# GaodeRender/triangle-splatting

Measured on AMD Instinct MI355X. Metric: fwd+bwd Mpixels/sec @ 1M triangles, 1920x1080; achieved HBM GB/s, higher is better.
Workload: dtype f32

## Files before the change

triangle-splatting_amd/csrc/api.hip:

```cpp
#pragma GCC visibility push(default)
#include "../../include/ts2d.h"
#ifdef TS2D_LAB
#include "ts2d_lab.h"
#endif
#pragma GCC visibility pop
#include "ts2d_api.h"
#include <atomic>
#include <chrono>
#include <cstdarg>
#include <cstdio>
#include <cstring>
#include <mutex>
#include <string>
#include <vector>

namespace
{
thread_local std::string g_err;

struct ProfRow { std::string name; double ms = 0; int64_t launches = 0; };
struct ProfPending { int row; hipEvent_t a, b; };
std::mutex g_prof_mu;
bool g_prof_on = false;
std::string g_prof_only;
std::vector<ProfRow> g_prof_rows;
std::vector<ProfPending> g_prof_pending;
std::vector<hipEvent_t> g_prof_free;

void prof_drain()
{
    for (auto &p : g_prof_pending)
    {
        float ms = 0;
        if (hipEventSynchronize(p.b) == hipSuccess && hipEventElapsedTime(&ms, p.a, p.b) == hipSuccess)
        {
            g_prof_rows[p.row].ms += ms;
            g_prof_rows[p.row].launches += 1;
        }
        g_prof_free.push_back(p.a);
        g_prof_free.push_back(p.b);
    }
    g_prof_pending.clear();
}

#ifdef TS2D_LAB
bool g_lab_all_quadrants = false;
#endif

int validate(const ts2d_camera *cam, const ts2d_geometry *geom, uint32_t flags)
{
    if (!cam || !geom) return ts_fail(TS2D_ERR_INVALID, "null camera/geometry");
    if (cam->width <= 0 || cam->height <= 0) return ts_fail(TS2D_ERR_INVALID, "image size must be positive");
    if (cam->width > 65535 * TS_TILE || cam->height > 65535 * TS_TILE) return ts_fail(TS2D_ERR_INVALID, "image too large");
    if (geom->P < 0) return ts_fail(TS2D_ERR_INVALID, "P must be >= 0");
    if (geom->P > (int)TS_ID_MASK) return ts_fail(TS2D_ERR_CAPACITY, "more than 2^28 - 1 triangles: the instance values keep four bits for the quadrant mask");
    if (geom->C > TS2D_MAX_CHANNELS)
        return ts_fail(TS2D_ERR_INVALID, "feature's num_channels can't be larger than MAX_CHANNELS");
    if (geom->C < 1) return ts_fail(TS2D_ERR_INVALID, "need at least one colour channel");
    if (geom->gamma < 0.0f) return ts_fail(TS2D_ERR_INVALID, "gamma must be larger than 0");
    if (flags & TS2D_FLAG_USE_SHS)
    {
        if (geom->C != 3) return ts_fail(TS2D_ERR_INVALID, "SH mode renders 3 channels");
        if (geom->sh_degree < 0 || geom->sh_degree > 3) return ts_fail(TS2D_ERR_INVALID, "sh_degree must be in 0..3");
        if ((geom->sh_degree + 1) * (geom->sh_degree + 1) > geom->M)
            return ts_fail(TS2D_ERR_INVALID, "shs holds fewer coefficients than sh_degree needs");
        if (geom->P > 0 && !geom->shs) return ts_fail(TS2D_ERR_INVALID, "shs is null");
    }
    else if (geom->P > 0 && !geom->feature) return ts_fail(TS2D_ERR_INVALID, "feature is null");
    if (geom->P > 0 && (!geom->vertex || !geom->opacity)) return ts_fail(TS2D_ERR_INVALID, "vertex/opacity is null");
    if (!cam->viewmatrix || !cam->projmatrix || !cam->campos || !geom->background)
        return ts_fail(TS2D_ERR_INVALID, "camera matrices / background are null");
    return TS2D_OK;
}

PreprocessArgs make_pre(const ts2d_camera *cam, const ts2d_geometry *geom, uint32_t flags)
{
    PreprocessArgs a;
    a.W = cam->width; a.H = cam->height; a.P = geom->P; a.D = geom->sh_degree; a.M = geom->M; a.C = geom->C;
    a.grid_x = (cam->width + TS_TILE - 1) / TS_TILE; a.grid_y = (cam->height + TS_TILE - 1) / TS_TILE;
    a.rich_info = flags & TS2D_FLAG_RICH_INFO; a.use_shs = flags & TS2D_FLAG_USE_SHS;
    a.back_culling = flags & TS2D_FLAG_BACK_CULLING;
    a.tan_fovx = cam->tan_fovx; a.tan_fovy = cam->tan_fovy;
    a.viewmatrix = cam->viewmatrix; a.projmatrix = cam->projmatrix; a.campos = cam->campos;
    a.vertex = geom->vertex; a.shs = geom->shs; a.feature = geom->feature; a.opacity = geom->opacity;
    return a;
}

RenderArgs make_render(const ts2d_camera *cam, const ts2d_geometry *geom, uint32_t flags)
{
    RenderArgs r;
    r.W = cam->width; r.H = cam->height; r.C = geom->C;
    r.grid_x = (cam->width + TS_TILE - 1) / TS_TILE; r.grid_y = (cam->height + TS_TILE - 1) / TS_TILE;
    r.gamma = geom->gamma; r.background_depth = geom->background_depth;
    r.background_depth_dev = geom->background_depth_dev;
    r.background = geom->background;
    r.rich_info = flags & TS2D_FLAG_RICH_INFO;
    return r;
}

inline void cpu_relax()
{
#if defined(__x86_64__) || defined(__i386__)
    __builtin_ia32_pause();
#elif defined(__aarch64__)
    asm volatile("yield" ::: "memory");
#endif
}

struct CapacityHint { int dev, variant, W, H; unsigned long long key; double per_triangle; unsigned long long stamp; };
thread_local unsigned long long t_hint_key = 0;
std::atomic<unsigned long long> g_speculative_overflows{0};
std::mutex g_hint_mu;
std::vector<CapacityHint> g_hints;
unsigned long long g_hint_clock = 0;

void record_instance_count(int variant, int W, int H, int P, unsigned long long n)
{
    int dev = 0;
    if (P <= 0 || hipGetDevice(&dev) != hipSuccess) return;
    const double per = (double)n / (double)P;
    std::lock_guard<std::mutex> lk(g_hint_mu);
    CapacityHint *slot = nullptr;
    for (auto &h : g_hints)
        if (h.dev == dev && h.variant == variant && h.W == W && h.H == H && h.key == t_hint_key) slot = &h;
    if (!slot)
    {
        if (g_hints.size() < 32) { g_hints.push_back({dev, variant, W, H, t_hint_key, 0.0, 0}); slot = &g_hints.back(); }
        else
        {
            slot = &g_hints[0];
            for (auto &h : g_hints)
                if (h.stamp < slot->stamp) slot = &h;
            *slot = {dev, variant, W, H, t_hint_key, 0.0, 0};
        }
    }
    slot->per_triangle = per > 0.97 * slot->per_triangle ? per : 0.97 * slot->per_triangle;
    slot->stamp = ++g_hint_clock;
}

int read_instance_count(const ts2d_camera *cam, const ts2d_geometry *geom, uint32_t flags, const ts2d_state *state, const EarlyCount *early,
                        hipStream_t s, int64_t *num_rendered)
{
    if (int rc = wait_instance_count(geom->P, state, early, s, num_rendered)) return rc;
    record_instance_count((flags & TS2D_FLAG_3D) ? 3 : 2, cam->width, cam->height, geom->P, (unsigned long long)*num_rendered);
    return TS2D_OK;
}

int forward_bin_impl(const ts2d_camera *cam, const ts2d_geometry *geom, uint32_t flags, int32_t *radii, const ts2d_state *state, hipStream_t s,
                     const EarlyCount *early)
{
    const int P = geom->P;
    GeometryStateView g;
    ts_carve_geometry((char *)state->geometry, P, g);
    const PreprocessArgs a = make_pre(cam, geom, flags);
    {
        ProfScope ps("preprocess_fwd", s);
        if (flags & TS2D_FLAG_3D) ts_launch_preprocess3d_fwd(a, radii, g, s);
        else ts_launch_preprocess_fwd(a, radii, g, s);
    }
    TS_CHECK(flags, s, "preprocess_fwd");
    return ts_order_triangles(flags, g, P, early, s);
}

int forward_render_impl(const ts2d_camera *cam, const ts2d_geometry *geom, uint32_t flags, int64_t N, bool count_on_device,
                        const ts2d_state *state, const ts2d_forward_out *out, hipStream_t s)
{
    const bool rich = flags & TS2D_FLAG_RICH_INFO;
    const int P = geom->P, W = cam->width, H = cam->height;
    GeometryStateView g{};
    BinningStateView b{};
    ImageStateView im{};
    if (P > 0) ts_carve_geometry((char *)state->geometry, P, g);
    if (N > 0)
    {
        ts_carve_binning((char *)state->binning, ts_binning_capacity(state->binning_bytes, W, H), W, H, b);
        if (!count_on_device) ts_binning_set_count(b, N);
    }
    ts_carve_image((char *)state->image, W, H, im);
    const RenderArgs r = make_render(cam, geom, flags);
    const int ntiles = r.grid_x * r.grid_y;
    const unsigned long long *n_dev = count_on_device ? ts_instance_count_dev(g, P) : nullptr;

    QuadMaskArgs quad{(flags & TS2D_FLAG_3D) ? 3 : 2, fmaxf(0.0f, 2.0f * geom->gamma), cam->tan_fovx, cam->tan_fovy, W, H, 1.0f / (float)W, 1.0f / (float)H};
#ifdef TS2D_LAB
    if (g_lab_all_quadrants) quad.variant = 0;
#endif
    if (int rc = ts_order_instances(flags, P, r.grid_x, ntiles, g, b, im, rich ? out->contrib_sum : nullptr, rich ? out->contrib_max : nullptr, N, n_dev,
                                    quad, s))
        return rc;
    {
        ProfScope ps("render_fwd", s);
        if (flags & TS2D_FLAG_3D)
            ts_launch_render3d_fwd_group(r, cam->tan_fovx, cam->tan_fovy, g, b, im, out->out_feature, out->depth, out->normal,
                                         out->contrib_sum, out->contrib_max, s);
        else
            ts_launch_render_fwd_group(r, g, b, im, out->out_feature, out->depth, out->normal, out->contrib_sum, out->contrib_max, s);
    }
    TS_CHECK(flags, s, "render_fwd");
    return TS2D_OK;
}

int check_forward_args(const ts2d_camera *cam, const ts2d_geometry *geom, uint32_t flags, int64_t N, const ts2d_state *state,
                       const ts2d_forward_out *out)
{
    if (int rc = validate(cam, geom, flags)) return rc;
    if (!state || !out || !out->out_feature) return ts_fail(TS2D_ERR_INVALID, "null state/output");
    const bool rich = flags & TS2D_FLAG_RICH_INFO;
    if (rich && (!out->depth || !out->normal || (geom->P > 0 && (!out->contrib_sum || !out->contrib_max))))
        return ts_fail(TS2D_ERR_INVALID, "rich_info outputs are null");
    const int P = geom->P, W = cam->width, H = cam->height;
    if (N < 0) return ts_fail(TS2D_ERR_INVALID, "num_rendered < 0");
    if (N > 0x7fffffffll) return ts_fail(TS2D_ERR_CAPACITY, "the instance list addresses at most 2^31 - 1 instances");
    if (!state->image || state->image_bytes < ts2d_image_state_bytes(W, H)) return ts_fail(TS2D_ERR_CAPACITY, "image state buffer too small");
    if (N > 0 && (!state->binning || ts_binning_capacity(state->binning_bytes, W, H) < N))
        return ts_fail(TS2D_ERR_CAPACITY, "binning state buffer too small");
    if (P > 0 && (!state->geometry || state->geometry_bytes < ts2d_geometry_state_bytes(P)))
        return ts_fail(TS2D_ERR_CAPACITY, "geometry state buffer too small");
    return TS2D_OK;
}
}

int ts_fail(int code, const char *fmt, ...)
{
    char buf[512];
    va_list ap;
    va_start(ap, fmt);
    vsnprintf(buf, sizeof(buf), fmt, ap);
    va_end(ap);
    g_err = buf;
    return code;
}

ProfScope::ProfScope(const char *name, hipStream_t stream) : s(stream)
{
    if (!g_prof_on) return;
    std::lock_guard<std::mutex> lk(g_prof_mu);
    if (!g_prof_only.empty() && g_prof_only != name) return;
    for (size_t i = 0; i < g_prof_rows.size(); i++)
        if (g_prof_rows[i].name == name) row = (int)i;
    if (row < 0) { g_prof_rows.push_back({name, 0, 0}); row = (int)g_prof_rows.size() - 1; }
    auto get = [&]() { hipEvent_t e; if (!g_prof_free.empty()) { e = g_prof_free.back(); g_prof_free.pop_back(); } else (void)hipEventCreate(&e); return e; };
    a = get(); b = get();
    (void)hipEventRecord(a, s);
}
ProfScope::~ProfScope()
{
    if (row < 0) return;
    (void)hipEventRecord(b, s);
    std::lock_guard<std::mutex> lk(g_prof_mu);
    g_prof_pending.push_back({row, a, b});
}

bool acquire_early_count(EarlyCount &e)
{
    constexpr int SLOTS = 64, MAXDEV = 16;
    static unsigned long long *ring = [] {
        void *p = nullptr;
        return hipHostMalloc(&p, (size_t)MAXDEV * SLOTS * sizeof(unsigned long long), hipHostMallocPortable | hipHostMallocMapped | hipHostMallocCoherent) == hipSuccess
                   ? (unsigned long long *)p : nullptr;
    }();
    static hipEvent_t events[MAXDEV][SLOTS] = {};
    static std::atomic<unsigned> next{0};
    static std::mutex mu;
    int dev = 0;
    if (!ring || hipGetDevice(&dev) != hipSuccess || dev < 0 || dev >= MAXDEV) return false;
    const unsigned i = next.fetch_add(1) % SLOTS;
    {
        std::lock_guard<std::mutex> lk(mu);
#ifndef TS2D_COUNT_EVENT_FLAGS
#define TS2D_COUNT_EVENT_FLAGS (hipEventDisableTiming | hipEventBlockingSync)
#endif
        if (!events[dev][i] && hipEventCreateWithFlags(&events[dev][i], TS2D_COUNT_EVENT_FLAGS) != hipSuccess) return false;
    }
    e.host = ring + (size_t)dev * SLOTS + i;
    e.ev = events[dev][i];
    __atomic_store_n(e.host, ~0ull, __ATOMIC_RELEASE);
    return true;
}

int wait_instance_count(int P, const ts2d_state *state, const EarlyCount *early, hipStream_t s, int64_t *num_rendered)
{
    unsigned long long n = ~0ull;
    if (early)
    {
        const auto t0 = std::chrono::steady_clock::now();
        for (unsigned spin = 0;; spin++)
        {
            n = __atomic_load_n(early->host, __ATOMIC_ACQUIRE);
            if (n != ~0ull) break;
            cpu_relax();
            if ((spin & 63u) == 63u && std::chrono::steady_clock::now() - t0 > std::chrono::microseconds(250)) break;
        }
        if (n == ~0ull)
        {
            const hipError_t q = hipEventSynchronize(early->ev);
            if (q != hipSuccess) return ts_fail(TS2D_ERR_HIP, "waiting for the instance count: %s", hipGetErrorString(q));
            n = __atomic_load_n(early->host, __ATOMIC_ACQUIRE);
            if (n == ~0ull) return ts_fail(TS2D_ERR_HIP, "the instance count was not published");
        }
    }
    else
    {
        GeometryStateView g;
        ts_carve_geometry((char *)state->geometry, P, g);
        TS_HIP(hipMemcpyAsync(&n, ts_instance_count_dev(g, P), sizeof(n), hipMemcpyDeviceToHost, s));
        TS_HIP(hipStreamSynchronize(s));
    }
    if (n > 0x7fffffffull)
        return ts_fail(TS2D_ERR_CAPACITY, "%llu tile instances exceed the 2^31 - 1 the instance list can address", n);
    *num_rendered = (int64_t)n;
    return TS2D_OK;
}

int ts_order_triangles(uint32_t flags, const GeometryStateView &g, int P, const EarlyCount *early, hipStream_t s)
{
    {
        ProfScope ps("depth_census", s);
        ts_sort_by_depth_begin(g, P, early ? early->host : nullptr, s);
    }
    if (early) TS_HIP(hipEventRecord(early->ev, s));
    { ProfScope ps("depth_sort", s); ts_sort_by_depth_finish(g, P, s); }
    TS_CHECK(flags, s, "depth_sort");
    { ProfScope ps("scan", s); ts_scan_offsets(g, P, s); }
    TS_CHECK(flags, s, "scan");
    return TS2D_OK;
}

int ts_order_instances(uint32_t flags, int P, int grid_x, int ntiles, const GeometryStateView &g, const BinningStateView &b, const ImageStateView &im,
                       float *contrib_sum, float *contrib_max, int64_t N, const unsigned long long *n_dev, const QuadMaskArgs &quad, hipStream_t s)
{
    if (P > 0)
    {
        { ProfScope ps("emit_keys", s); ts_launch_emit_keys(P, grid_x, ntiles, g, b, im, contrib_sum, contrib_max, n_dev ? N : -1, im.status, quad, s); }
        TS_CHECK(flags, s, "emit_keys");
    }
    else ts_launch_zero_words((uint32_t *)im.ranges, 2 * (size_t)ntiles, s);
    if (N > 0)
    {
        { ProfScope ps("tile_sort", s); ts_sort_pairs(b, N, n_dev, ntiles, s); }
        TS_CHECK(flags, s, "tile_sort");
        { ProfScope ps("tile_ranges", s); ts_launch_tile_ranges(N, n_dev, b, im, s); }
        TS_CHECK(flags, s, "tile_ranges");
    }
    return TS2D_OK;
}

extern "C" {

const char *ts2d_version(void) { return "ts2d 0.1 (gfx950)"; }
const char *ts2d_last_error(void) { return g_err.c_str(); }

size_t ts2d_geometry_state_bytes(int32_t P)
{
    GeometryStateView v;
    return ts_carve_geometry(nullptr, P, v);
}
size_t ts2d_binning_state_bytes(int64_t N, int32_t W, int32_t H)
{
    BinningStateView v;
    return ts_carve_binning(nullptr, N, W, H, v);
}
size_t ts2d_image_state_bytes(int32_t W, int32_t H)
{
    ImageStateView v;
    return ts_carve_image(nullptr, W, H, v);
}
size_t ts2d_backward_scratch_bytes(int32_t P) { return (size_t)(P > 0 ? P : 0) * TS_GRAD_FLOATS * sizeof(float) + TS_ALIGN; }
int64_t ts2d_binning_capacity(size_t bytes, int32_t W, int32_t H)
{
    const int64_t c = ts_binning_capacity(bytes, W, H);
    return c < 0 ? 0 : c;
}
int64_t ts2d_instance_capacity_hint(int32_t P, int32_t W, int32_t H, uint32_t flags)
{
    int dev = 0;
    if (P <= 0 || hipGetDevice(&dev) != hipSuccess) return 0;
    const int variant = (flags & TS2D_FLAG_3D) ? 3 : 2;
    std::lock_guard<std::mutex> lk(g_hint_mu);
    for (auto &h : g_hints)
        if (h.dev == dev && h.variant == variant && h.W == W && h.H == H && h.key == t_hint_key)
        {
            h.stamp = ++g_hint_clock;
            const double want = 1.25 * h.per_triangle * (double)P + 4096.0;
            if (want >= 2147483647.0) return 0x7fffffffll;
            int64_t w = (int64_t)want, step = 1;
            while ((step << 4) <= w) step <<= 1;
            w = (w + step - 1) / step * step;
            return w > 0x7fffffffll ? 0x7fffffffll : w;
        }
    return 0;
}

int ts2d_forward_bin(const ts2d_camera *cam, const ts2d_geometry *geom, uint32_t flags, int32_t *radii,
                     const ts2d_state *state, int64_t *num_rendered, void *stream)
{
    if (int rc = validate(cam, geom, flags)) return rc;
    if (!state || !num_rendered) return ts_fail(TS2D_ERR_INVALID, "null state/num_rendered");
    hipStream_t s = (hipStream_t)stream;
    *num_rendered = 0;
    const int P = geom->P;
    if (P == 0) return TS2D_OK;
    if (!radii) return ts_fail(TS2D_ERR_INVALID, "radii is null");
    if (!state->geometry || state->geometry_bytes < ts2d_geometry_state_bytes(P))
        return ts_fail(TS2D_ERR_CAPACITY, "geometry state buffer too small: %zu < %zu", state->geometry_bytes,
                    ts2d_geometry_state_bytes(P));
    EarlyCount early;
    const bool have_early = acquire_early_count(early);
    if (int rc = forward_bin_impl(cam, geom, flags, radii, state, s, have_early ? &early : nullptr)) return rc;
    return read_instance_count(cam, geom, flags, state, have_early ? &early : nullptr, s, num_rendered);
}

int ts2d_forward_render(const ts2d_camera *cam, const ts2d_geometry *geom, uint32_t flags, int64_t N,
                        const ts2d_state *state, const ts2d_forward_out *out, void *stream)
{
    if (int rc = check_forward_args(cam, geom, flags, N, state, out)) return rc;
    return forward_render_impl(cam, geom, flags, N, false, state, out, (hipStream_t)stream);
}

int ts2d_forward(const ts2d_camera *cam, const ts2d_geometry *geom, uint32_t flags, int32_t *radii, const ts2d_state *state,
                 int64_t instance_capacity, const ts2d_forward_out *out, void *stream)
{
    if (int rc = check_forward_args(cam, geom, flags, instance_capacity, state, out)) return rc;
    hipStream_t s = (hipStream_t)stream;
    if (geom->P == 0) return forward_render_impl(cam, geom, flags, 0, false, state, out, s);
    if (!radii) return ts_fail(TS2D_ERR_INVALID, "radii is null");
    if (instance_capacity <= 0) return ts_fail(TS2D_ERR_INVALID, "instance_capacity must be positive");
    if (int rc = forward_bin_impl(cam, geom, flags, radii, state, s, nullptr)) return rc;
    return forward_render_impl(cam, geom, flags, instance_capacity, true, state, out, s);
}

int ts2d_forward_speculative(const ts2d_camera *cam, const ts2d_geometry *geom, uint32_t flags, int32_t *radii, const ts2d_state *state,
                             const ts2d_forward_out *out, int64_t *num_rendered, void *stream)
{
    if (!num_rendered) return ts_fail(TS2D_ERR_INVALID, "null num_rendered");
    *num_rendered = 0;
    if (int rc = check_forward_args(cam, geom, flags, 0, state, out)) return rc;
    hipStream_t s = (hipStream_t)stream;
    const int P = geom->P, W = cam->width, H = cam->height;
    if (P == 0) return forward_render_impl(cam, geom, flags, 0, false, state, out, s);
    if (!radii) return ts_fail(TS2D_ERR_INVALID, "radii is null");
    int64_t cap = state->binning ? ts_binning_capacity(state->binning_bytes, W, H) : 0;
    if (state->binning && cap <= 0) return ts_fail(TS2D_ERR_CAPACITY, "binning state buffer too small for any instance (pass NULL to size it from num_rendered)");
    EarlyCount early;
    const bool have_early = acquire_early_count(early);
    if (int rc = forward_bin_impl(cam, geom, flags, radii, state, s, have_early ? &early : nullptr)) return rc;
    if (cap > 0)
    {
        if (int rc = forward_render_impl(cam, geom, flags, cap, true, state, out, s)) return rc;
    }
    if (int rc = read_instance_count(cam, geom, flags, state, have_early ? &early : nullptr, s, num_rendered)) return rc;
    if (cap > 0 && *num_rendered > cap) g_speculative_overflows.fetch_add(1, std::memory_order_relaxed);
    return TS2D_OK;
}

void ts2d_set_capacity_hint_key(uint64_t key) { t_hint_key = key; }
uint64_t ts2d_speculative_overflow_count(void) { return g_speculative_overflows.load(std::memory_order_relaxed); }

int ts2d_forward_status(const ts2d_state *state, int32_t P, int32_t width, int32_t height, int32_t *overflowed, int64_t *num_rendered,
                        void *stream)
{
    if (!state || !state->image || !overflowed || !num_rendered) return ts_fail(TS2D_ERR_INVALID, "null pointer");
    hipStream_t s = (hipStream_t)stream;
    *overflowed = 0;
    *num_rendered = 0;
    if (P <= 0) return TS2D_OK;
    if (!state->geometry) return ts_fail(TS2D_ERR_INVALID, "null geometry state");
    GeometryStateView g{};
    ImageStateView im{};
    ts_carve_geometry((char *)state->geometry, P, g);
    ts_carve_image((char *)state->image, width, height, im);
    unsigned long long n = 0;
    TS_HIP(hipMemcpyAsync(overflowed, im.status, sizeof(int32_t), hipMemcpyDeviceToHost, s));
    TS_HIP(hipMemcpyAsync(&n, ts_instance_count_dev(g, P), sizeof(n), hipMemcpyDeviceToHost, s));
    TS_HIP(hipStreamSynchronize(s));
    *num_rendered = (int64_t)n;
    return TS2D_OK;
}

int ts2d_backward(const ts2d_camera *cam, const ts2d_geometry *geom, uint32_t flags, int64_t N, const int32_t *radii,
                  const ts2d_state *state, const ts2d_loss_grads *loss, void *scratch, size_t scratch_bytes,
                  const ts2d_backward_out *out, void *stream)
{
    return ts2d_backward_ranged(cam, geom, flags, N, radii, state, loss, scratch, scratch_bytes, out, 1, nullptr, stream);
}

int32_t ts2d_backward_range_rows(int32_t P, int32_t num_ranges)
{
    if (P <= 0 || num_ranges < 1) return 0;
    return ((P + num_ranges - 1) / num_ranges + 63) & ~63;
}

int ts2d_backward_ranged(const ts2d_camera *cam, const ts2d_geometry *geom, uint32_t flags, int64_t N, const int32_t *radii,
                         const ts2d_state *state, const ts2d_loss_grads *loss, void *scratch, size_t scratch_bytes,
                         const ts2d_backward_out *out, int32_t num_ranges, void *const *range_done_events, void *stream)
// ... 16 lines not shown
    if (!scratch || scratch_bytes < ts2d_backward_scratch_bytes(P)) return ts_fail(TS2D_ERR_CAPACITY, "backward scratch too small");
    if (!state->geometry || state->geometry_bytes < ts2d_geometry_state_bytes(P) || !state->image ||
        state->image_bytes < ts2d_image_state_bytes(W, H) ||
        (N > 0 && (!state->binning || ts_binning_capacity(state->binning_bytes, W, H) < N)))
        return ts_fail(TS2D_ERR_CAPACITY, "state buffers too small");
    GeometryStateView g{};
    BinningStateView b{};
    ImageStateView im{};
    ts_carve_geometry((char *)state->geometry, P, g);
    if (N > 0) ts_carve_binning((char *)state->binning, ts_binning_capacity(state->binning_bytes, W, H), W, H, b);
    ts_carve_image((char *)state->image, W, H, im);
    RenderArgs r = make_render(cam, geom, flags);
    if (colour_only) r.rich_info = false;
    float *grad_rec = (float *)ts_align_up((size_t)scratch);

    {
        ProfScope ps("zero_grad_records", s);
        ts_launch_zero_words((uint32_t *)grad_rec, (size_t)TS_GRAD_FLOATS * (size_t)P, s);
    }
    if (N > 0)
    {
        ProfScope ps("render_bwd", s);
        if (flags & TS2D_FLAG_3D)
            ts_launch_render3d_bwd_group(r, cam->tan_fovx, cam->tan_fovy, g, b, im, loss->dL_dout_feature, loss->dL_dout_depth,
                                         loss->dL_dout_normal, grad_rec, s);
        else
            ts_launch_render_bwd_group(r, g, b, im, loss->dL_dout_feature, loss->dL_dout_depth, loss->dL_dout_normal, grad_rec, s);
    }
    TS_CHECK(flags, s, "render_bwd");
    {
        ProfScope ps("preprocess_bwd", s);
        const PreprocessArgs a = make_pre(cam, geom, flags);
        const int per = ((P + num_ranges - 1) / num_ranges + 63) & ~63;
        for (int k = 0; k < num_ranges; k++)
        {
            const int first = k * per, count = first < P ? (P - first < per ? P - first : per) : 0;
            if (count > 0)
            {
                PreprocessArgs ak = a;
                ak.P = count;
                ak.vertex += 9 * (size_t)first;
                if (ak.shs) ak.shs += (size_t)first * a.M * 3;
                if (ak.feature) ak.feature += (size_t)first * a.C;
                ak.opacity += first;
                GeometryStateView gk = g;
                gk.clamped += first;
                if (gk.rec) gk.rec += 4 * (size_t)first;
                float *dshs = (factored || !out->dL_dshs) ? nullptr : out->dL_dshs + (size_t)first * a.M * 3;
                float *dfeat = out->dL_dfeature ? out->dL_dfeature + (size_t)first * a.C : nullptr;
                if (flags & TS2D_FLAG_3D)
                    ts_launch_preprocess3d_bwd(ak, radii + first, gk, grad_rec + TS_GRAD_FLOATS * (size_t)first, out->dL_dvertex + 9 * (size_t)first,
                                               out->dL_dcenter2D + 2 * (size_t)first, dshs, dfeat, out->dL_dopacity + first, s);
                else
                    ts_launch_preprocess_bwd(ak, radii + first, gk, grad_rec + TS_GRAD_FLOATS * (size_t)first, out->dL_dvertex + 9 * (size_t)first,
                                             out->dL_dcenter2D + 2 * (size_t)first, dshs, dfeat, out->dL_dopacity + first, s);
            }
            if (range_done_events && range_done_events[k]) TS_HIP(hipEventRecord((hipEvent_t)range_done_events[k], s));
        }
    }
    TS_CHECK(flags, s, "preprocess_bwd");
    return TS2D_OK;
}

int ts2d_sh_grad_expand(int32_t P, int32_t sh_degree, int32_t M, int32_t num_views, const float *vertex, const float *campos,
                        const float *dL_dcolor, float *dL_dshs, void *stream)
{
    if (P < 0 || num_views < 0) return ts_fail(TS2D_ERR_INVALID, "P / num_views must be >= 0");
    if (sh_degree < 0 || sh_degree > 3) return ts_fail(TS2D_ERR_INVALID, "sh_degree must be in 0..3");
    if ((sh_degree + 1) * (sh_degree + 1) > M) return ts_fail(TS2D_ERR_INVALID, "shs holds fewer coefficients than sh_degree needs");
    if (P == 0) return TS2D_OK;
    if (!vertex || !dL_dshs || (num_views > 0 && (!campos || !dL_dcolor))) return ts_fail(TS2D_ERR_INVALID, "null pointer");
    hipStream_t s = (hipStream_t)stream;
    { ProfScope ps("sh_grad_expand", s); ts_launch_sh_grad_expand(P, sh_degree, M, num_views, vertex, campos, dL_dcolor, dL_dshs, s); }
    TS_CHECK(0u, s, "sh_grad_expand");
    return TS2D_OK;
}

#ifdef TS2D_LAB
int ts2d_debug_read_state(const ts2d_state *state, int32_t P, int64_t N, int32_t W, int32_t H, int32_t field, void *dst,
                          size_t dst_bytes, void *stream)
{
    if (!state || !dst) return ts_fail(TS2D_ERR_INVALID, "null state/dst");
    hipStream_t s = (hipStream_t)stream;
    GeometryStateView g{};
    BinningStateView b{};
    ImageStateView im{};
    if (P > 0 && state->geometry) ts_carve_geometry((char *)state->geometry, P, g);
    if (N > 0 && state->binning) ts_carve_binning((char *)state->binning, ts_binning_capacity(state->binning_bytes, W, H), W, H, b);
    if (state->image) ts_carve_image((char *)state->image, W, H, im);
    const int gx = (W + TS_TILE - 1) / TS_TILE, gy = (H + TS_TILE - 1) / TS_TILE;
    const void *src = nullptr;
    size_t bytes = 0;
    std::vector<float> recs;
    auto need_recs = [&]() -> int {
        recs.resize((size_t)P * TS_REC_FLOATS);
        if (P == 0) return TS2D_OK;
        TS_HIP(hipMemcpyAsync(recs.data(), g.rec, recs.size() * sizeof(float), hipMemcpyDeviceToHost, s));
        TS_HIP(hipStreamSynchronize(s));
        return TS2D_OK;
    };
    auto from_recs = [&](std::initializer_list<int> cols, bool area) -> int {
        if (int rc = need_recs()) return rc;
        const size_t n = area ? 1 : cols.size();
        if (dst_bytes < (size_t)P * n * sizeof(float)) return ts_fail(TS2D_ERR_CAPACITY, "dst too small");
        float *o = (float *)dst;
        for (int i = 0; i < P; i++)
        {
            const float *r = &recs[(size_t)i * TS_REC_FLOATS];
            if (area) o[i] = (r[2] - r[0]) * (r[5] - r[1]) - (r[3] - r[1]) * (r[4] - r[0]);
            else { size_t c = 0; for (int col : cols) o[(size_t)i * n + c++] = r[col]; }
        }
        return TS2D_OK;
    };
    switch (field)
    {
    case 0: return from_recs({0, 1, 2, 3, 4, 5}, false);
    case 1: return from_recs({}, true);
    case 2: return from_recs({10, 11, 12}, false);
    case 3: return from_recs({13, 14, 15}, false);
    case 5: return from_recs({7, 8, 9}, false);
    case 4: src = g.depth; bytes = (size_t)P * 4; break;
    case 6: src = g.clamped; bytes = (size_t)P; break;
    case 7: src = g.offsets; bytes = (size_t)P * 4; break;
    case 8: src = g.tiles_touched; bytes = (size_t)P * 4; break;
    case 9:
    {
        std::vector<uint2> rc((size_t)P);
        if (dst_bytes < (size_t)P * 16) return ts_fail(TS2D_ERR_CAPACITY, "dst too small");
        if (P > 0)
        {
            TS_HIP(hipMemcpyAsync(rc.data(), g.rect, (size_t)P * sizeof(uint2), hipMemcpyDeviceToHost, s));
            TS_HIP(hipStreamSynchronize(s));
        }
        uint32_t *o = (uint32_t *)dst;
        for (int i = 0; i < P; i++)
        {
            o[4 * i] = rc[i].x & 0xffffu; o[4 * i + 1] = rc[i].x >> 16;
            o[4 * i + 2] = rc[i].y & 0xffffu; o[4 * i + 3] = rc[i].y >> 16;
        }
        return TS2D_OK;
    }
    case 10:
    {
        if (dst_bytes < (size_t)N * 8) return ts_fail(TS2D_ERR_CAPACITY, "dst too small");
        std::vector<uint32_t> tile((size_t)N), vals((size_t)N), depth((size_t)P);
        if (N > 0)
        {
            TS_HIP(hipMemcpyAsync(tile.data(), b.tile, (size_t)N * 4, hipMemcpyDeviceToHost, s));
            TS_HIP(hipMemcpyAsync(vals.data(), b.vals, (size_t)N * 4, hipMemcpyDeviceToHost, s));
            TS_HIP(hipMemcpyAsync(depth.data(), g.depth, (size_t)P * 4, hipMemcpyDeviceToHost, s));
            TS_HIP(hipStreamSynchronize(s));
        }
        uint64_t *o = (uint64_t *)dst;
        for (int64_t i = 0; i < N; i++) o[i] = ((uint64_t)tile[i] << 32) | depth[vals[i] & TS_ID_MASK];
        return TS2D_OK;
    }
    case 11: src = b.vals; bytes = (size_t)N * 4; break;
    case 12: src = im.ranges; bytes = (size_t)gx * gy * 8; break;
    case 13: src = im.n_contrib; bytes = (size_t)W * H * 4; break;
    case 14: src = im.final_T; bytes = (size_t)W * H * 4; break;
    case 15: src = b.k[(b.passes & 1) ^ 1]; bytes = (size_t)N * 4; break;
    case 16: src = b.v[(b.passes & 1) ^ 1]; bytes = (size_t)N * 4; break;
    case 17:
    {
        uint32_t top_const = 0;
        if (P > 0)
        {
            TS_HIP(hipMemcpyAsync(&top_const, g.top_const, 4, hipMemcpyDeviceToHost, s));
            TS_HIP(hipStreamSynchronize(s));
        }
        src = top_const ? g.sv[0] : g.sv[1];
        bytes = (size_t)P * 4;
        break;
    }
    case 18: src = g.rec; bytes = (size_t)P * TS_REC_FLOATS * 4; break;
    default: return ts_fail(TS2D_ERR_INVALID, "unknown field %d", field);
    }
    if (dst_bytes < bytes) return ts_fail(TS2D_ERR_CAPACITY, "dst too small");
    if (bytes)
    {
        TS_HIP(hipMemcpyAsync(dst, src, bytes, hipMemcpyDeviceToHost, s));
        TS_HIP(hipStreamSynchronize(s));
    }
    return TS2D_OK;
}

void ts2d_lab_force_ticket_passes(int on) { ts_force_ticket_passes(on != 0); }
void ts2d_lab_force_all_quadrants(int on) { g_lab_all_quadrants = on != 0; }
void ts2d_lab_force_depth_pass4(int on) { ts_force_depth_pass4(on != 0); }
void ts2d_lab_depth_split(int mode, int bucket_cap) { ts_lab_depth_split(mode, bucket_cap); }
#endif

void ts2d_profile_enable(int on)
{
    std::lock_guard<std::mutex> lk(g_prof_mu);
    g_prof_on = on != 0;
}
void ts2d_profile_only(const char *name)
{
    std::lock_guard<std::mutex> lk(g_prof_mu);
    g_prof_only = name ? name : "";
}
void ts2d_profile_reset(void)
{
    std::lock_guard<std::mutex> lk(g_prof_mu);
    prof_drain();
    g_prof_rows.clear();
}
int ts2d_profile_read(int32_t index, char *name, size_t name_bytes, double *total_ms, int64_t *launches)
{
    std::lock_guard<std::mutex> lk(g_prof_mu);
    prof_drain();
    if (index < 0 || (size_t)index >= g_prof_rows.size()) return TS2D_ERR_INVALID;
    const ProfRow &r = g_prof_rows[index];
    if (name && name_bytes) { strncpy(name, r.name.c_str(), name_bytes - 1); name[name_bytes - 1] = 0; }
    if (total_ms) *total_ms = r.ms;
    if (launches) *launches = r.launches;
    return TS2D_OK;
}
}
```

triangle-splatting_amd/csrc/binning.hip:

```cpp
#include "ts2d_common.h"
#include "ts2d_wave.h"
#include "ts2d_support.h"

namespace
{
constexpr int NB = TS_RS_BINS;

__device__ __forceinline__ unsigned long long ballot64(bool p) { return __builtin_amdgcn_ballot_w64(p); }

__device__ __forceinline__ uint32_t wave_inclusive_scan(uint32_t v, int lane)
{
    int x = (int)v;
    x += __builtin_amdgcn_update_dpp(0, x, 0x111, 0xF, 0xF, true);
    x += __builtin_amdgcn_update_dpp(0, x, 0x112, 0xF, 0xF, true);
    x += __builtin_amdgcn_update_dpp(0, x, 0x114, 0xF, 0xF, true);
    x += __builtin_amdgcn_update_dpp(0, x, 0x118, 0xF, 0xF, true);
    x += __builtin_amdgcn_update_dpp(0, x, 0x142, 0xA, 0xF, true);
    x += __builtin_amdgcn_update_dpp(0, x, 0x143, 0xC, 0xF, true);
    return (uint32_t)x;
}
__device__ __forceinline__ unsigned long long wave_sum64(unsigned long long v)
{
    for (int o = 32; o > 0; o >>= 1) v += __shfl_xor(v, o);
    return v;
// ... 492 lines not shown
#pragma unroll
        for (int j = 0; j < KB; j++)
        {
            const int p = t + 256 * j;
            if ((j & 3) == 0) dpack[j >> 2] = 0u;
            if (p < count)
            {
                const uint32_t k = stage_k[p], d = (k >> shift) & mask;
                dpack[j >> 2] |= d << (8 * (j & 3));
                kout[(int64_t)gdelta[d] + p] = k;
            }
        }
        __syncthreads();
#pragma unroll
        for (int b = 0; b < KB; b++)
            if (64 * b + lane < mine) stage_k[rk[b]] = val[b];
        __syncthreads();
#pragma unroll
        for (int j = 0; j < KB; j++)
        {
            const int p = t + 256 * j;
            if (p < count) vout[(int64_t)gdelta[(dpack[j >> 2] >> (8 * (j & 3))) & 0xFFu] + p] = stage_k[p];
        }
        return;
    }
#pragma unroll
    for (int b = 0; b < KB; b++)
        if (64 * b + lane < mine)
        {
            const uint32_t p = wcnt[wave][(key[b] >> shift) & mask] + rk[b];
            stage_k[p] = key[b];
            stage_v[p] = val[b];
        }
    __syncthreads();
    for (int p = t; p < count; p += 256)
    {
        const uint32_t k = stage_k[p];
        const int64_t dst = (int64_t)gdelta[(k >> shift) & mask] + p;
        kout[dst] = k;
        vout[dst] = stage_v[p];
    }
    if (CENSUS && chunk == 0) publish_census(census, r.chunks, t);
}
template <bool IDENTITY_VALUES, int CH, bool DIRECT, bool CENSUS = false>
__global__ void __launch_bounds__(256) rs_scatter_kernel(const uint32_t *__restrict__ kin, const uint32_t *__restrict__ vin,
                                                          uint32_t *__restrict__ kout, uint32_t *__restrict__ vout, int64_t n,
                                                          const unsigned long long *n_dev, int shift, int nbits, RadixScratchView r, const uint32_t *skip_flag,
                                                          const uint32_t *__restrict__ acc, uint32_t *__restrict__ acc_clear, DepthCensus census = DepthCensus{})
{
    rs_scatter_body<IDENTITY_VALUES, CH, DIRECT, CENSUS, false>(kin, vin, kout, vout, n, n_dev, shift, nbits, r, skip_flag, acc, acc_clear, census);
}
template <int CH>
__global__ void __launch_bounds__(256, 5) rs_scatter_two_phase_kernel(const uint32_t *__restrict__ kin, const uint32_t *__restrict__ vin,
                                                                       uint32_t *__restrict__ kout, uint32_t *__restrict__ vout, int64_t n,
                                                                       const unsigned long long *n_dev, int shift, int nbits, RadixScratchView r,
                                                                       const uint32_t *skip_flag, const uint32_t *__restrict__ acc, uint32_t *__restrict__ acc_clear)
{
    rs_scatter_body<false, CH, true, false, true>(kin, vin, kout, vout, n, n_dev, shift, nbits, r, skip_flag, acc, acc_clear, DepthCensus{});
}

#define TS_WITH_CHUNK(chunk, ...)                                    \
    switch (chunk)                                                   \
    {                                                                \
    case TS_RS_CHUNK_SMALL: { constexpr int CH = TS_RS_CHUNK_SMALL; __VA_ARGS__; } break; \
    case TS_RS_CHUNK_MID: { constexpr int CH = TS_RS_CHUNK_MID; __VA_ARGS__; } break;     \
    default: { constexpr int CH = TS_RS_CHUNK; __VA_ARGS__; } break; \
    }
void radix_hist(const uint32_t *kin, int64_t n, const unsigned long long *n_dev, int shift, int nbits, const RadixScratchView &r, hipStream_t s,
                const DepthCensus *census = nullptr, const uint32_t *skip_flag = nullptr)
{
    const dim3 grid((unsigned)r.chunks);
    const uint32_t mask = (1u << nbits) - 1u;
    TS_WITH_CHUNK(r.chunk,
                  if (census) hipLaunchKernelGGL((rs_hist_kernel<true, CH>), grid, dim3(256), 0, s, kin, n, n_dev, shift, mask, r, *census, skip_flag);
                  else hipLaunchKernelGGL((rs_hist_kernel<false, CH>), grid, dim3(256), 0, s, kin, n, n_dev, shift, mask, r, DepthCensus{}, skip_flag))
}
template <int CH>
void radix_scatter_ch(const uint32_t *kin, const uint32_t *vin, uint32_t *kout, uint32_t *vout, int64_t n, const unsigned long long *n_dev, int shift,
                      int nbits, const RadixScratchView &r, hipStream_t s, const uint32_t *skip_flag, const uint32_t *acc, uint32_t *acc_clear)
{
    const dim3 grid((unsigned)r.chunks);
#define TS_SCATTER(ID, D) hipLaunchKernelGGL((rs_scatter_kernel<ID, CH, D>), grid, dim3(256), 0, s, kin, vin, kout, vout, n, n_dev, shift, nbits, r, skip_flag, acc, acc_clear)
    if (acc && vin)
    {
        if constexpr (CH == TS_RS_CHUNK)
            hipLaunchKernelGGL((rs_scatter_two_phase_kernel<CH>), grid, dim3(256), 0, s, kin, vin, kout, vout, n, n_dev, shift, nbits, r, skip_flag, acc, acc_clear);
        else TS_SCATTER(false, true);
    }
    else if (acc) TS_SCATTER(true, true);
    else if (vin) TS_SCATTER(false, false);
    else TS_SCATTER(true, false);
#undef TS_SCATTER
}
void radix_scatter(const uint32_t *kin, const uint32_t *vin, uint32_t *kout, uint32_t *vout, int64_t n, const unsigned long long *n_dev, int shift,
                   int nbits, const RadixScratchView &r, hipStream_t s, const uint32_t *skip_flag = nullptr, const uint32_t *acc = nullptr,
                   uint32_t *acc_clear = nullptr)
{
    TS_WITH_CHUNK(r.chunk, radix_scatter_ch<CH>(kin, vin, kout, vout, n, n_dev, shift, nbits, r, s, skip_flag, acc, acc_clear))
}
void radix_pass(const uint32_t *kin, const uint32_t *vin, uint32_t *kout, uint32_t *vout, int64_t n, const unsigned long long *n_dev, int shift,
                int nbits, const RadixScratchView &r, hipStream_t s, const uint32_t *skip_flag = nullptr)
{
    radix_hist(kin, n, n_dev, shift, nbits, r, s, nullptr, skip_flag);
    radix_scatter(kin, vin, kout, vout, n, n_dev, shift, nbits, r, s, skip_flag);
}
bool g_force_tickets = false;
bool g_force_pass4 = false;
bool radix_direct_ok(const RadixScratchView &r) { return !g_force_tickets && r.slabs <= TS_DIRECT_MAX_SLABS; }
void radix_pass_direct(const uint32_t *kin, const uint32_t *vin, uint32_t *kout, uint32_t *vout, int64_t n, const unsigned long long *n_dev, int shift,
                       int nbits, const RadixScratchView &r, int which, hipStream_t s, const uint32_t *skip_flag = nullptr)
{
    const dim3 grid((unsigned)r.chunks);
    const uint32_t mask = (1u << nbits) - 1u;
    TS_WITH_CHUNK(r.chunk, hipLaunchKernelGGL((rs_hist_direct_kernel<CH>), grid, dim3(256), 0, s, kin, n, n_dev, shift, mask, r, r.slabacc[which], skip_flag))
    radix_scatter(kin, vin, kout, vout, n, n_dev, shift, nbits, r, s, skip_flag, r.slabacc[which], r.slabacc[which ^ 1]);
}

constexpr int SB = 1024;

__global__ void __launch_bounds__(256) gather_blocksum_kernel(int P, GeometryStateView g, bool two_level)
{
    __shared__ unsigned long long wsum[4];
    const int t = threadIdx.x, lane = t & 63, wave = t >> 6;
    const int i0 = blockIdx.x * SB + 4 * t;
    const uint32_t *ids = sorted_ids(g);
    uint32_t v[4];
    unsigned long long sum = 0;
#pragma unroll
    for (int k = 0; k < 4; k++)
    {
        v[k] = (i0 + k < P) ? g.tiles_touched[ids[i0 + k]] : 0u;
        sum += v[k];
    }
    if (i0 + 3 < P) *(uint4 *)(g.tiles_sorted + i0) = make_uint4(v[0], v[1], v[2], v[3]);
    else
        for (int k = 0; k < 4; k++)
            if (i0 + k < P) g.tiles_sorted[i0 + k] = v[k];
    for (int o = 32; o > 0; o >>= 1) sum += __shfl_xor(sum, o);
    if (lane == 0) wsum[wave] = sum;
    __syncthreads();
    if (t == 0)
    {
        const unsigned long long total = wsum[0] + wsum[1] + wsum[2] + wsum[3];
        g.blocksum[blockIdx.x] = total;
        if (two_level && total) __hip_atomic_fetch_add((unsigned long long *)g.supersum + (blockIdx.x >> 6), total, __ATOMIC_RELAXED, __HIP_MEMORY_SCOPE_AGENT);
    }
}

constexpr uint32_t SMALL = 32;

#ifndef TS_EMIT_WAVES
#define TS_EMIT_WAVES 6
#endif
#if TS_EMIT_WAVES > 0
__global__ void __launch_bounds__(256, TS_EMIT_WAVES) scan_emit_kernel(
#else
__global__ void __launch_bounds__(256) scan_emit_kernel(
#endif
int P, int grid_x, int ntiles, GeometryStateView g, BinningStateView b, uint2 *ranges,
                                                         float *contrib_sum, float *contrib_max, long long capacity, int32_t *status, bool two_level,
                                                         QuadMaskArgs qmask)
{
    __shared__ uint32_t wtot[4];
    __shared__ unsigned long long wpart[4];
    const int t = threadIdx.x, lane = t & 63, wave = t >> 6;
    const int i = blockIdx.x * 256 + t;
    for (int k = i; k < ntiles; k += gridDim.x * 256) ranges[k] = make_uint2(0u, 0u);
    if (b.rs.tickets)
    {
        for (int k = i; k < b.rs.slabs + TS_RS_TICKET_EXTRA; k += gridDim.x * 256) b.rs.tickets[k] = 0u;
        for (int k = i; k < b.rs.slabs * NB; k += gridDim.x * 256) b.rs.slabacc[0][k] = 0u;
    }
    if (contrib_sum && i < P)
    {
        contrib_sum[i] = 0.0f;
        contrib_max[i] = 0.0f;
    }
    const bool valid = i < P;
    uint32_t tiles = valid ? g.tiles_sorted[i] : 0u;
    const uint32_t id_ahead = valid ? sorted_ids(g)[i] : 0u;
    const int sblock = blockIdx.x >> 2, quarter = blockIdx.x & 3;
    unsigned long long part = 0;
    if (two_level)
    {
        for (int k = t; k < (sblock >> 6); k += 256) part += g.supersum[k];
        if (t < (sblock & 63)) part += g.blocksum[(sblock & ~63) + t];
    }
    else
        for (int k = t; k < sblock; k += 256) part += g.blocksum[k];
    for (int q = 0; q < quarter; q++)
    {
        const int j = (sblock * 4 + q) * 256 + t;
        part += (j < P) ? g.tiles_sorted[j] : 0u;
    }
    if (capacity >= 0)
    {
        const unsigned long long live = g.blocksum[(P + SB - 1) / SB];
        const bool over = live > (unsigned long long)capacity;
        if (i == 0 && status) *status = over ? 1 : 0;
        if (over) tiles = 0u;
    }
    else if (i == 0 && status) *status = 0;
    const uint32_t inc = wave_inclusive_scan(tiles, lane);
    for (int o = 32; o > 0; o >>= 1) part += __shfl_xor(part, o);
    if (lane == 63) wtot[wave] = inc;
    if (lane == 0) wpart[wave] = part;
    __syncthreads();
    uint32_t before = 0;
    for (int w = 0; w < wave; w++) before += wtot[w];
    const unsigned long long qbase = wpart[0] + wpart[1] + wpart[2] + wpart[3];
    const uint32_t incl = (uint32_t)(qbase + before + inc);
    if (valid) g.offsets[i] = incl;
    const uint32_t id = tiles > 0 ? id_ahead : 0u;
    const uint32_t off = incl - tiles;
    uint2 rect = {0u, 0u};
    float4 rec0 = make_float4(0, 0, 0, 0), rec1 = rec0, rec2 = rec0;
    if (tiles > 0)
    {
        rect = g.rect[id];
        const float4 *rp = g.rec + 4 * (size_t)id;
        rec0 = rp[0];
        rec1 = rp[1];
        if (qmask.variant == 3) rec2 = rp[2];
    }
    const uint32_t minx = rect.x & 0xffffu, miny = rect.x >> 16, maxx = rect.y & 0xffffu, maxy = rect.y >> 16;
    uint32_t *tile_out = b.k[0], *val_out = b.v[0];
    constexpr bool qm = true;
    const float quad_g2 = qmask.g2;
    auto setup_from = [&](const float4 &r0, const float4 &r1, const float4 &r2, uint32_t tminx, uint32_t tminy, uint32_t tmaxx, uint32_t tmaxy) {
        if (qmask.variant == 0) return quad_setup_all();
        if (qmask.variant == 3)
        {
            const float E = quad_g2 == 2.0f ? support_scale<true>(1.0f, quad_g2) : support_scale<false>(1.0f, quad_g2);
            return quad_setup_3d(r0, r1, r2, E, qmask.tan_fovx, qmask.tan_fovy, qmask.W, qmask.H, qmask.inv_W, qmask.inv_H, (float)(tminx * TS_TILE) - 1.0f,
                                 (float)(tminy * TS_TILE) - 1.0f, (float)(tmaxx * TS_TILE), (float)(tmaxy * TS_TILE));
        }
        const float E = quad_g2 == 2.0f ? support_scale<true>(r1.z, quad_g2) : support_scale<false>(r1.z, quad_g2);
        return quad_setup(r0.x, r0.y, r0.z, r0.w, r1.x, r1.y, E);
    };
    auto setup_of = [&](uint32_t tri, uint32_t tminx, uint32_t tminy, uint32_t tmaxx, uint32_t tmaxy) {
        const float4 *rp = g.rec + 4 * (size_t)tri;
        return setup_from(rp[0], rp[1], qmask.variant == 3 ? rp[2] : make_float4(0, 0, 0, 0), tminx, tminy, tmaxx, tmaxy);
    };
    QuadSetup qs{};
    constexpr uint32_t STAGE = 2048;
    __shared__ uint32_t stage_t[STAGE];
    __shared__ __attribute__((aligned(16))) float4 region_b[256 * 4];
    uint32_t *const stage_v = (uint32_t *)region_b;
    const uint32_t run0 = (uint32_t)qbase, run = wtot[0] + wtot[1] + wtot[2] + wtot[3];
    const bool staged = run <= STAGE;
    const bool qstage = qm && staged;
    const uint32_t rw = maxx - minx, rh = maxy - miny;
    if (qm && tiles > 0)
    {
        qs = setup_from(rec0, rec1, rec2, minx, miny, maxx, maxy);
        if (qstage)
        {
            const QuadAffine qa = quad_anchor(qs, id, minx, miny, rw, rh);
            region_b[4 * t] = qa.a; region_b[4 * t + 1] = qa.b; region_b[4 * t + 2] = qa.c; region_b[4 * t + 3] = qa.d;
        }
    }
    if (tiles > 0 && tiles <= SMALL)
    {
        uint32_t o = off;
        if (staged)
        {
            o -= run0;
            for (uint32_t y = miny; y < maxy; y++)
                for (uint32_t x = minx; x < maxx; x++)
                {
                    stage_t[o] = qstage ? ((x - minx) | ((y - miny) << 12) | ((uint32_t)t << 24)) : y * grid_x + x;
                    if (!qstage) stage_v[o] = id;
                    o++;
                }
        }
        else
            for (uint32_t y = miny; y < maxy; y++)
                for (uint32_t x = minx; x < maxx; x++)
                {
                    tile_out[o] = y * grid_x + x;
                    val_out[o] = qm ? id | (quadrant_mask(qs, (float)(x * TS_TILE), (float)(y * TS_TILE)) << TS_ID_BITS) : id;
                    o++;
                }
    }
    unsigned long long big = ballot64(tiles > SMALL);
    while (big)
    {
        const int j = __builtin_ctzll(big);
        big &= big - 1;
        const uint32_t t_minx = __shfl(minx, j), t_miny = __shfl(miny, j), t_maxx = __shfl(maxx, j), t_maxy = __shfl(maxy, j);
        const uint32_t t_tiles = __shfl(tiles, j), t_off = __shfl(off, j), t_id = __shfl(id, j);
        const uint32_t w = t_maxx - t_minx;
        QuadSetup tq{};
        if (qm && !staged) tq = setup_of(t_id, t_minx, t_miny, t_maxx, t_maxy);
        for (uint32_t k = lane; k < t_tiles; k += 64)
        {
            const uint32_t y = t_miny + k / w, x = t_minx + k % w;
            if (staged)
            {
                stage_t[t_off - run0 + k] = qstage ? ((k % w) | ((k / w) << 12) | ((uint32_t)(wave * 64 + j) << 24)) : y * grid_x + x;
                if (!qstage) stage_v[t_off - run0 + k] = t_id;
            }
            else
            {
                tile_out[t_off + k] = y * grid_x + x;
                val_out[t_off + k] = qm ? t_id | (quadrant_mask(tq, (float)(x * TS_TILE), (float)(y * TS_TILE)) << TS_ID_BITS) : t_id;
            }
        }
    }
    if (staged)
    {
        __syncthreads();
        for (uint32_t k = t; k < run; k += 256)
        {
            uint32_t tl = stage_t[k], v;
            if (qstage)
            {
                const uint32_t dx = tl & 0xfffu, dy = (tl >> 12) & 0xfffu, slot = tl >> 24;
                QuadAffine qa;
                qa.a = region_b[4 * slot]; qa.b = region_b[4 * slot + 1]; qa.c = region_b[4 * slot + 2]; qa.d = region_b[4 * slot + 3];
                const uint32_t org = __float_as_uint(qa.d.z), x = (org & 0xffffu) + dx, y = (org >> 16) + dy;
                v = __float_as_uint(qa.d.y) | (quadrant_mask_affine(qa, dx, dy, x, y) << TS_ID_BITS);
                tl = y * grid_x + x;
            }
            else v = stage_v[k];
            tile_out[run0 + k] = tl;
            val_out[run0 + k] = v;
        }
    }
}

__global__ void __launch_bounds__(256) tile_ranges_kernel(int64_t N, const unsigned long long *n_dev, const uint32_t *__restrict__ tile,
                                                           uint2 *__restrict__ ranges)
{
    const int64_t i0 = ((int64_t)blockIdx.x * 256 + threadIdx.x) * 4;
    if (n_dev)
    {
        const unsigned long long live = *n_dev;
        N = (live <= (unsigned long long)N) ? (int64_t)live : 0;
    }
    if (i0 >= N) return;
    uint32_t k[4];
    if (i0 + 3 < N)
    {
        const uint4 q = *(const uint4 *)(tile + i0);
        k[0] = q.x; k[1] = q.y; k[2] = q.z; k[3] = q.w;
    }
    else
        for (int j = 0; j < 4; j++) k[j] = i0 + j < N ? tile[i0 + j] : 0u;
    uint32_t prev = i0 > 0 ? tile[i0 - 1] : 0u;
#pragma unroll
    for (int j = 0; j < 4; j++)
    {
        const int64_t i = i0 + j;
        if (i >= N) break;
        const uint32_t cur = k[j];
        if (i == 0) ranges[cur].x = 0;
        else if (cur != prev)
        {
            ranges[prev].y = (uint32_t)i;
            ranges[cur].x = (uint32_t)i;
        }
        if (i == N - 1) ranges[cur].y = (uint32_t)N;
        prev = cur;
    }
}

__global__ void zero_words_kernel(uint32_t *p, size_t n)
{
    const size_t i = (size_t)blockIdx.x * 256 + threadIdx.x;
    if (i < n) p[i] = 0u;
}
constexpr int TS_DEPTH_SMALL_MAX = 12288;
constexpr int DS_WAVES = 16, DS_KB = TS_DEPTH_SMALL_MAX / (64 * DS_WAVES);
#if !defined(__gfx950__) && defined(__HIP_DEVICE_COMPILE__)
#error "depth_order_small_kernel is sized for gfx950 (160 KB LDS per workgroup)"
#endif
static_assert(2 * TS_DEPTH_SMALL_MAX * 4 + DS_WAVES * NB * 4 + DS_WAVES * 8 + (TS_DEPTH_SMALL_MAX / SB) * 8 + 2 * DS_WAVES * 4 + 16 <= 160 * 1024 - 8 * 1024,
              "depth_order_small_kernel: static LDS must leave 8 KB of the 160 KB for the runtime / alignment");
__global__ void __launch_bounds__(64 * DS_WAVES) depth_order_small_kernel(int P, GeometryStateView g, unsigned long long *host_out)
{
    __shared__ __attribute__((aligned(16))) uint32_t stage_k[TS_DEPTH_SMALL_MAX], stage_v[TS_DEPTH_SMALL_MAX];
    __shared__ uint32_t wcnt[DS_WAVES][NB];
    __shared__ uint32_t wtot[4];
    __shared__ unsigned long long csum[DS_WAVES], bsum[TS_DEPTH_SMALL_MAX / SB];
    __shared__ uint32_t cor[DS_WAVES], cand[DS_WAVES];
    const int t = threadIdx.x, wave = t >> 6, lane = t & 63;
    const int per = ((P + 64 * DS_WAVES - 1) / (64 * DS_WAVES)) * 64;
    const int base = wave * per;
    const int mine = P - base < per ? (P - base > 0 ? P - base : 0) : per;
    const uint32_t *keys = (const uint32_t *)g.depth;
    uint32_t key[DS_KB], val[DS_KB], rk[DS_KB];
    KeyCensus census;
    if (t < TS_DEPTH_SMALL_MAX / SB) bsum[t] = 0ull;
#pragma unroll
    for (int b = 0; b < DS_KB; b++)
    {
        const int i = 64 * b + lane;
        const bool in = i < mine;
        const int src = in ? base + i : 0;
        const uint32_t k = keys[src], tt = g.tiles_touched[src];
        key[b] = in ? k : 0xFFFFFFFFu;
        val[b] = (uint32_t)src;
        census.add(in ? k : 0u, in ? tt : 0u);
    }
    census.wave_fold();
    census.park(csum, cor, cand);
    __syncthreads();
    census = KeyCensus::gather<DS_WAVES>(csum, cor, cand);
    const unsigned long long N = census.tiles;
    const int passes = census.top_byte_constant() ? 3 : 4;
#pragma nounroll
    for (int pass = 0; pass < passes; pass++)
    {
        uint32_t unused;
        lsd_rank_pass<DS_KB, DS_WAVES>(key, rk, 8 * pass, per, mine, wcnt, wtot, unused);
#pragma unroll
        for (int b = 0; b < DS_KB; b++)
            if (64 * b + lane < mine) { stage_k[rk[b]] = key[b]; stage_v[rk[b]] = val[b]; }
        __syncthreads();
#pragma unroll
        for (int b = 0; b < DS_KB; b++)
        {
            key[b] = stage_k[base + 64 * b + lane];
            val[b] = stage_v[base + 64 * b + lane];
        }
    }
#pragma unroll
    for (int b = 0; b < DS_KB; b++)
    {
        if (64 * b >= per) continue;
        const int i = base + 64 * b + lane;
        unsigned long long tiles = 0;
        if (64 * b + lane < mine)
        {
            const uint32_t tt = g.tiles_touched[val[b]];
            g.sk[1][i] = key[b];
            g.sv[1][i] = val[b];
            g.tiles_sorted[i] = tt;
            tiles = tt;
        }
        tiles = wave_sum64(tiles);
        if (lane == 0 && tiles) atomicAdd(&bsum[(base + 64 * b) / SB], tiles);
    }
    __syncthreads();
    const int nblocks = (P + SB - 1) / SB;
    if (t < nblocks) g.blocksum[t] = bsum[t];
    if (t == 0) publish_instance_count(N, (unsigned long long *)g.blocksum + nblocks, g.top_const, false, host_out);
}

#ifndef TS_DEPTH_SPLIT_MAX_VALUE
#define TS_DEPTH_SPLIT_MAX_VALUE 500000
#endif
constexpr int TS_DEPTH_SPLIT_MAX = TS_DEPTH_SPLIT_MAX_VALUE;
constexpr int TS_DEPTH_SPLIT_HARD_MAX = 1600000;
constexpr int DSPL_SAMPLES = 4096, DSPL_SAMPLES_SMALL = 1024, DSPL_SMALL_BELOW = 150000;
constexpr int DB_WAVES = 16, DB_KB = 16, DB_CAP = 64 * DB_WAVES * DB_KB;
#ifndef TS_DB_SMALL_BELOW_VALUE
#define TS_DB_SMALL_BELOW_VALUE 300000
#endif
constexpr int DB_SMALL_WAVES = 4, DB_SMALL_BELOW = TS_DB_SMALL_BELOW_VALUE;
int g_depth_split_mode = 0;
int g_depth_bucket_cap = DB_CAP;

struct DepthSplit
{
    uint32_t *splitters;
    uint32_t *bucket_start;
    unsigned long long *chunk_sum;
    uint8_t *digit;
};
__host__ __device__ inline DepthSplit depth_split_of(const GeometryStateView &g)
{
    DepthSplit d;
    d.splitters = g.offsets;
    d.bucket_start = g.offsets + NB;
    d.chunk_sum = (unsigned long long *)(g.offsets + 1024);
    d.digit = (uint8_t *)g.sv[1];
    return d;
}

__device__ __forceinline__ uint32_t depth_key_adjust(uint32_t key, uint32_t kmin_visible) { return key ? key - kmin_visible + 1u : 0u; }
__device__ __forceinline__ uint32_t depth_key_restore(uint32_t adj, uint32_t kmin_visible) { return adj ? adj - 1u + kmin_visible : 0u; }

template <int SAMPLES>
__global__ void __launch_bounds__(256) depth_split_sample_kernel(int P, GeometryStateView g, DepthSplit ds)
{
    constexpr int DSPL_SAMPLES = SAMPLES, DSPL_PER = SAMPLES / NB;
    __shared__ uint32_t hist[NB], wtot[4], pick[2], rmin[4], rmax[4];
    constexpr int K = DSPL_SAMPLES / 256;
    const int t = threadIdx.x, lane = t & 63, wave = t >> 6;
    const uint32_t *keys = (const uint32_t *)g.depth;
    const int nblocks = (P + SB - 1) / SB;
    for (int i = blockIdx.x * 256 + t; i < nblocks; i += gridDim.x * 256) g.blocksum[i] = 0ull;
    uint32_t smp[K];
#pragma unroll
    for (int k = 0; k < K; k++) smp[k] = keys[(int)(((unsigned long long)(t + 256 * k) * (unsigned long long)P) / DSPL_SAMPLES)];
    uint32_t kmin = 0xFFFFFFFFu, kmax = 0u;
#pragma unroll
    for (int k = 0; k < K; k++) { kmin = min(kmin, smp[k] ? smp[k] : 0xFFFFFFFFu); kmax = max(kmax, smp[k]); }
    for (int o = 32; o > 0; o >>= 1) { kmin = min(kmin, (uint32_t)__shfl_xor((int)kmin, o)); kmax = max(kmax, (uint32_t)__shfl_xor((int)kmax, o)); }
    if (lane == 0) { rmin[wave] = kmin; rmax[wave] = kmax; }
    __syncthreads();
// ... 282 lines not shown
            for (int i = t; i < n; i += 64 * DB_WAVES) atomicAdd(&dstart[(depth_key_adjust(peer_load(kin + i), kmin) >> (8 * pass)) & 0xFFu], 1u);
            __syncthreads();
            {
                const uint32_t start = digit_exclusive_prefix<W>(t < NB ? dstart[t] : 0u, wtot, wave, lane);
                if (t < NB) dstart[t] = start;
                __syncthreads();
            }
            for (int t0 = 0; t0 < n; t0 += tile)
            {
                const int nt = n - t0 < tile ? n - t0 : tile;
                const int tper = ((nt + 64 * DB_WAVES - 1) / (64 * DB_WAVES)) * 64;
                const int tbase = wave * tper;
                const int tmine = nt - tbase < tper ? (nt - tbase > 0 ? nt - tbase : 0) : tper;
#pragma unroll
                for (int b = 0; b < DB_KB; b++)
                {
                    const int i = 64 * b + lane;
                    const bool in = i < tmine;
                    key[b] = in ? depth_key_adjust(peer_load(kin + t0 + tbase + i), kmin) : 0xFFFFFFFFu;
                    val[b] = in ? peer_load(vin + t0 + tbase + i) : 0u;
                }
                uint32_t tile_cnt;
                lsd_rank_pass<DB_KB, W>(key, rk, 8 * pass, tper, tmine, wcnt, wtot, tile_cnt);
#pragma unroll
                for (int b = 0; b < DB_KB; b++)
                    if (64 * b + lane < tmine)
                    {
                        const uint32_t d = (key[b] >> (8 * pass)) & 0xFFu;
                        const uint32_t p = dstart[d] + rk[b] - wcnt[0][d];
                        peer_store(kout + p, depth_key_restore(key[b], kmin));
                        peer_store(vout + p, val[b]);
                    }
                __syncthreads();
                if (t < NB) dstart[t] += tile_cnt;
                __syncthreads();
            }
            asm volatile("s_waitcnt vmcnt(0)" ::: "memory");
            __syncthreads();
        }
        if (src == 0)
            for (int i = t; i < n; i += 64 * DB_WAVES) { peer_store(g.sk[1] + s0 + i, peer_load(g.sk[0] + s0 + i)); peer_store(g.sv[1] + s0 + i, peer_load(g.sv[0] + s0 + i)); }
        asm volatile("s_waitcnt vmcnt(0)" ::: "memory");
        __syncthreads();
        for (int i0 = 64 * wave; i0 < n; i0 += 64 * DB_WAVES)
        {
            const bool in = i0 + lane < n;
            bucket_emit_tiles(g, s0 + i0, s0 + i0 + lane, in, in ? g.tiles_touched[peer_load(g.sv[1] + s0 + i0 + lane)] : 0u, lane);
        }
    }
}
}

#ifndef TS_DEPTH_SMALL_USE_VALUE
#define TS_DEPTH_SMALL_USE_VALUE 9216
#endif
constexpr int TS_DEPTH_SMALL_USE = TS_DEPTH_SMALL_USE_VALUE;
static_assert(TS_DEPTH_SMALL_USE <= TS_DEPTH_SMALL_MAX && TS_DEPTH_SMALL_USE >= 2048, "the split form's scratch needs 1024 + 2 chunks words of `offsets`");
enum class DepthForm { OneLaunch, Split, LsdDirect, LsdTickets };
static DepthForm depth_form(int32_t P, const RadixScratchView &r)
{
    const bool lsd_forced = g_force_tickets || g_force_pass4;
    if (P <= TS_DEPTH_SMALL_USE && !lsd_forced) return DepthForm::OneLaunch;
    if (!radix_direct_ok(r)) return DepthForm::LsdTickets;
    const bool split = P > TS_DEPTH_SMALL_USE && P <= (g_depth_split_mode == 2 ? TS_DEPTH_SPLIT_HARD_MAX : TS_DEPTH_SPLIT_MAX) && g_depth_split_mode != 1;
    return split && !lsd_forced ? DepthForm::Split : DepthForm::LsdDirect;
}
void ts_sort_by_depth_begin(const GeometryStateView &g, int32_t P, unsigned long long *host_out, hipStream_t s)
{
    if (P <= 0) return;
    const DepthForm form = depth_form(P, g.rs);
    if (form == DepthForm::OneLaunch)
    {
        hipLaunchKernelGGL(depth_order_small_kernel, dim3(1), dim3(64 * DS_WAVES), 0, s, P, g, host_out);
        return;
    }
    if (form == DepthForm::Split)
    {
        const DepthSplit ds = depth_split_of(g);
        const dim3 grid((unsigned)g.rs.chunks);
        if (P < DSPL_SMALL_BELOW) hipLaunchKernelGGL(depth_split_sample_kernel<DSPL_SAMPLES_SMALL>, dim3(NB - 1), dim3(256), 0, s, P, g, ds);
        else hipLaunchKernelGGL(depth_split_sample_kernel<DSPL_SAMPLES>, dim3(NB - 1), dim3(256), 0, s, P, g, ds);
        TS_WITH_CHUNK(g.rs.chunk,
                      hipLaunchKernelGGL((depth_split_hist_kernel<CH>), grid, dim3(256), 0, s, (int64_t)P, g, g.rs, g.rs.slabacc[0], ds);
                      hipLaunchKernelGGL((depth_split_scatter_kernel<CH>), grid, dim3(256), 0, s, (int64_t)P, g, g.rs, (const uint32_t *)g.rs.slabacc[0], ds, host_out))
        return;
    }
    DepthCensus c;
    c.tiles_touched = g.tiles_touched;
    c.chunk_sum = (unsigned long long *)g.blocksum;
    c.chunk_or = g.tiles_sorted;
    c.chunk_and = g.offsets;
    c.n_out = (unsigned long long *)g.blocksum + (P + SB - 1) / SB;
    c.host_out = host_out;
    c.top_const = g.top_const;
    c.force_varying = g_force_pass4 ? 0xFF000000u : 0u;
    if (form == DepthForm::LsdTickets)
    {
        radix_hist((const uint32_t *)g.depth, P, nullptr, 0, 8, g.rs, s, &c);
        return;
    }
    const dim3 grid((unsigned)g.rs.chunks);
    const uint32_t *keys = (const uint32_t *)g.depth;
    const unsigned long long *no_count = nullptr;
    const uint32_t *no_vals = nullptr, *no_skip = nullptr;
    TS_WITH_CHUNK(g.rs.chunk,
                  hipLaunchKernelGGL((rs_hist_census_direct_kernel<CH>), grid, dim3(256), 0, s, keys, (int64_t)P, 0xFFu, g.rs, g.rs.slabacc[0], c);
                  hipLaunchKernelGGL((rs_scatter_kernel<true, CH, true, true>), grid, dim3(256), 0, s, keys, no_vals, g.sk[0], g.sv[0], (int64_t)P, no_count, 0, 8,
                                     g.rs, no_skip, (const uint32_t *)g.rs.slabacc[0], g.rs.slabacc[1], c))
}
void ts_sort_by_depth_finish(const GeometryStateView &g, int32_t P, hipStream_t s)
{
    if (P <= 0) return;
    switch (depth_form(P, g.rs))
    {
    case DepthForm::OneLaunch: return;
    case DepthForm::Split:
        if (P < DB_SMALL_BELOW)
            hipLaunchKernelGGL(depth_bucket_sort_kernel<DB_SMALL_WAVES>, dim3(NB), dim3(64 * DB_SMALL_WAVES), 0, s, P, g, depth_split_of(g),
                               min(g_depth_bucket_cap, 64 * DB_SMALL_WAVES * DB_KB));
        else hipLaunchKernelGGL(depth_bucket_sort_kernel<DB_WAVES>, dim3(NB), dim3(64 * DB_WAVES), 0, s, P, g, depth_split_of(g), g_depth_bucket_cap);
        return;
    case DepthForm::LsdTickets:
        radix_scatter((const uint32_t *)g.depth, nullptr, g.sk[0], g.sv[0], P, nullptr, 0, 8, g.rs, s);
        radix_pass(g.sk[0], g.sv[0], g.sk[1], g.sv[1], P, nullptr, 8, 8, g.rs, s);
        radix_pass(g.sk[1], g.sv[1], g.sk[0], g.sv[0], P, nullptr, 16, 8, g.rs, s);
        radix_pass(g.sk[0], g.sv[0], g.sk[1], g.sv[1], P, nullptr, 24, 8, g.rs, s, g.top_const);
        return;
    case DepthForm::LsdDirect:
        radix_pass_direct(g.sk[0], g.sv[0], g.sk[1], g.sv[1], P, nullptr, 8, 8, g.rs, 1, s);
        radix_pass_direct(g.sk[1], g.sv[1], g.sk[0], g.sv[0], P, nullptr, 16, 8, g.rs, 0, s);
        radix_pass_direct(g.sk[0], g.sv[0], g.sk[1], g.sv[1], P, nullptr, 24, 8, g.rs, 1, s, g.top_const);
        return;
    }
}

static bool scan_two_level(int32_t P) { return g_force_tickets || (P + SB - 1) / SB > 2048; }
void ts_scan_offsets(const GeometryStateView &g, int32_t P, hipStream_t s)
{
    if (P <= 0) return;
    switch (depth_form(P, g.rs))
    {
    case DepthForm::OneLaunch:
    case DepthForm::Split: return;
    case DepthForm::LsdDirect:
    case DepthForm::LsdTickets: break;
    }
    hipLaunchKernelGGL(gather_blocksum_kernel, dim3((unsigned)((P + SB - 1) / SB)), dim3(256), 0, s, P, g, scan_two_level(P));
}

void ts_launch_emit_keys(int P, int grid_x, int ntiles, const GeometryStateView &g, const BinningStateView &b, const ImageStateView &im,
                         float *contrib_sum, float *contrib_max, int64_t capacity, int32_t *status, const QuadMaskArgs &qmask, hipStream_t s)
{
    if (P <= 0) return;
    hipLaunchKernelGGL(scan_emit_kernel, dim3((unsigned)(((P + SB - 1) / SB) * 4)), dim3(256), 0, s, P, grid_x, ntiles, g, b, im.ranges, contrib_sum,
                       contrib_max, (long long)capacity, status, scan_two_level(P), qmask);
}
const unsigned long long *ts_instance_count_dev(const GeometryStateView &g, int P) { return (const unsigned long long *)(g.blocksum + (P + SB - 1) / SB); }

void ts_sort_pairs(const BinningStateView &b, int64_t N, const unsigned long long *n_dev, int ntiles, hipStream_t s)
{
    if (N <= 0) return;
    const int bits = ts_tile_bits(ntiles);
    const int per = (bits + b.passes - 1) / b.passes;
    int src = 0;
    for (int p = 0; p < b.passes; p++)
    {
        const int shift = per * p, nbits = min(per, bits - shift);
        if (radix_direct_ok(b.rs)) radix_pass_direct(b.k[src], b.v[src], b.k[src ^ 1], b.v[src ^ 1], N, n_dev, shift, nbits, b.rs, p & 1, s);
        else radix_pass(b.k[src], b.v[src], b.k[src ^ 1], b.v[src ^ 1], N, n_dev, shift, nbits, b.rs, s);
        src ^= 1;
    }
}

void ts_launch_tile_ranges(int64_t N, const unsigned long long *n_dev, const BinningStateView &b, const ImageStateView &im, hipStream_t s)
{
    if (N <= 0) return;
    hipLaunchKernelGGL(tile_ranges_kernel, dim3((unsigned)((N + 1023) / 1024)), dim3(256), 0, s, N, n_dev, b.tile, im.ranges);
}

static int generic_chunk(size_t n) { return ts_instance_chunk(n); }
size_t ts_radix_scratch_bytes(size_t n)
{
    RadixScratchView r{};
    char *p = nullptr;
    ts_carve_radix(p, n, r, generic_chunk(n));
    return (size_t)p + TS_ALIGN;
}
int ts_radix_sort_pairs(uint32_t *const k[2], uint32_t *const v[2], size_t n, int end_bit, void *scratch, hipStream_t s, bool force_tickets)
{
    if (n == 0) return 0;
    RadixScratchView r{};
    char *p = (char *)ts_align_up((size_t)scratch);
    ts_carve_radix(p, n, r, generic_chunk(n));
    hipLaunchKernelGGL(zero_words_kernel, dim3((unsigned)((r.slabs + TS_RS_TICKET_EXTRA + 255) / 256)), dim3(256), 0, s, r.tickets, (size_t)(r.slabs + TS_RS_TICKET_EXTRA));
    const bool direct = !force_tickets && radix_direct_ok(r);
    if (direct) hipLaunchKernelGGL(zero_words_kernel, dim3((unsigned)r.slabs), dim3(256), 0, s, r.slabacc[0], (size_t)(r.slabs * NB));
    const int passes = (end_bit + 7) / 8;
    int src = 0;
    for (int ps = 0; ps < passes; ps++)
    {
        if (direct) radix_pass_direct(k[src], v[src], k[src ^ 1], v[src ^ 1], (int64_t)n, nullptr, 8 * ps, min(8, end_bit - 8 * ps), r, ps & 1, s);
        else radix_pass(k[src], v[src], k[src ^ 1], v[src ^ 1], (int64_t)n, nullptr, 8 * ps, min(8, end_bit - 8 * ps), r, s);
        src ^= 1;
    }
    return src;
}

void ts_force_ticket_passes(bool on) { g_force_tickets = on; }
namespace
{
__global__ void __launch_bounds__(256) zero_words4_kernel(uint4 *p, size_t n4)
{
    const size_t i = (size_t)blockIdx.x * 256 + threadIdx.x;
    if (i < n4) p[i] = make_uint4(0u, 0u, 0u, 0u);
}
}
void ts_launch_zero_words(uint32_t *p, size_t n, hipStream_t s)
{
    if (n == 0) return;
    if (n % 4 == 0 && ((size_t)p & 15) == 0) hipLaunchKernelGGL(zero_words4_kernel, dim3((unsigned)((n / 4 + 255) / 256)), dim3(256), 0, s, (uint4 *)p, n / 4);
    else hipLaunchKernelGGL(zero_words_kernel, dim3((unsigned)((n + 255) / 256)), dim3(256), 0, s, p, n);
}
void ts_force_depth_pass4(bool on) { g_force_pass4 = on; }
void ts_lab_depth_split(int mode, int bucket_cap)
{
    g_depth_split_mode = mode;
    g_depth_bucket_cap = bucket_cap > 0 && bucket_cap < DB_CAP ? bucket_cap : DB_CAP;
}
```

triangle-splatting_amd/csrc/render_group.hip:

```cpp
#include "ts2d_common.h"
#include "ts2d_wave.h"
#include "ts2d_group.h"
#include "ts2d_support.h"

#ifndef TSG_FWD_WAVES
#define TSG_FWD_WAVES 7
#endif
#ifndef TSG_BWD_WAVES
#define TSG_BWD_WAVES 7
#endif
#ifndef TSG_FWD_CAP
#define TSG_FWD_CAP 64
#endif
#ifndef TSG_BWD_CAP
#define TSG_BWD_CAP 64
#endif
#ifndef TSG_TCAP
#define TSG_TCAP 960
#endif
#ifndef TSG_PART
#define TSG_PART 3
#endif
namespace
{
[[maybe_unused]] constexpr int BROW = ROW + 16;

struct BlockCull
{
    float u1x, u1y, u2x, u2y, u3x, u3y, ia;
    bool ov[4];
};

__device__ __forceinline__ void publish_row(float *row, const BlockCull &s, uint32_t id, int jpos, const float4 &r1, const float4 &r2, const float4 &r3)
{
    float4 *q = (float4 *)row;
    q[0] = make_float4(s.u1x, s.u1y, s.u2x, s.u2y);
    q[1] = make_float4(s.u3x, s.u3y, s.ia, r1.z);
    q[2] = make_float4(r1.w, r2.x, r2.y, r2.z);
    q[3] = make_float4(r2.w, r3.x, r3.y, r3.z);
    q[4] = make_float4(r3.w, __uint_as_float(id), __int_as_float(jpos), 0.0f);
}

__device__ __forceinline__ void entry_geometry(BlockCull &s, float v1x, float v1y, float v2x, float v2y, float v3x, float v3y, float OX, float OY)
{
    const float area2 = __fsub_rn(__fmul_rn(v2x - v1x, v3y - v1y), __fmul_rn(v2y - v1y, v3x - v1x));
    s.ia = __builtin_amdgcn_rcpf(area2);
    s.u1x = v1x - OX; s.u1y = v1y - OY; s.u2x = v2x - OX; s.u2y = v2y - OY; s.u3x = v3x - OX; s.u3y = v3y - OY;
}

template <bool RICH>
__device__ __forceinline__ uint32_t republish_row(float *row, const uint32_t *__restrict__ point_list, const float4 *__restrict__ rec, uint32_t pos,
                                                  int jpos, float OX, float OY)
{
    const uint32_t id = point_list[pos] & TS_ID_MASK;
    const float4 *rp = rec + 4 * (size_t)id;
    const float4 r0 = rp[0], r1 = rp[1], r2 = rp[2], r3 = RICH ? rp[3] : make_float4(0, 0, 0, 0);
    BlockCull s;
    entry_geometry(s, r0.x, r0.y, r0.z, r0.w, r1.x, r1.y, OX, OY);
    publish_row(row, s, id, jpos, r1, r2, r3);
    return id;
}

template <bool GAMMA1>
__device__ __forceinline__ BlockCull block_cull(float v1x, float v1y, float v2x, float v2y, float v3x, float v3y, float op, float g2,
                                                float OX, float OY)
{
    BlockCull s;
    entry_geometry(s, v1x, v1y, v2x, v2y, v3x, v3y, OX, OY);
    const float C1 = (s.u2x * s.u3y - s.u2y * s.u3x) * s.ia, A1 = (v2y - v3y) * s.ia, B1 = (v3x - v2x) * s.ia;
    const float C2 = (s.u3x * s.u1y - s.u3y * s.u1x) * s.ia, A2 = (v3y - v1y) * s.ia, B2 = (v1x - v3x) * s.ia;
    const float A3 = -A1 - A2, B3 = -B1 - B2, C3 = 1.0f - C1 - C2;
    const float E = support_scale<GAMMA1>(op, g2);
    const float cx = (s.u1x + s.u2x + s.u3x) * (1.0f / 3.0f), cy = (s.u1y + s.u2y + s.u3y) * (1.0f / 3.0f);
    const float e1x = E * (s.u1x - cx), e2x = E * (s.u2x - cx), e3x = E * (s.u3x - cx);
    const float e1y = E * (s.u1y - cy), e2y = E * (s.u2y - cy), e3y = E * (s.u3y - cy);
    const float pad = 0.05f;
    const float bminx = cx + fminf(fminf(e1x, e2x), e3x) - pad, bmaxx = cx + fmaxf(fmaxf(e1x, e2x), e3x) + pad;
    const float bminy = cy + fminf(fminf(e1y, e2y), e3y) - pad, bmaxy = cy + fmaxf(fmaxf(e1y, e2y), e3y) + pad;
    const bool live = E > 0.0f;
    const bool x0 = live && bminx <= 3.0f && bmaxx >= 0.0f, x1 = live && bminx <= 7.0f && bmaxx >= 4.0f;
    const bool y0 = bminy <= 3.0f && bmaxy >= 0.0f, y1 = bminy <= 7.0f && bmaxy >= 4.0f;
    const float m = (1.0f - E) * (1.0f / 3.0f);
    const float k1 = C1 + fmaxf(0.0f, 3.0f * A1) + fmaxf(0.0f, 3.0f * B1) - m + 1e-6f * (fabsf(C1) + 7.0f * (fabsf(A1) + fabsf(B1)));
    const float k2 = C2 + fmaxf(0.0f, 3.0f * A2) + fmaxf(0.0f, 3.0f * B2) - m + 1e-6f * (fabsf(C2) + 7.0f * (fabsf(A2) + fabsf(B2)));
    const float k3 = C3 + fmaxf(0.0f, 3.0f * A3) + fmaxf(0.0f, 3.0f * B3) - m + 1e-6f * (fabsf(C3) + 7.0f * (fabsf(A3) + fabsf(B3)));
    const float ax1 = 4.0f * A1, ax2 = 4.0f * A2, ax3 = 4.0f * A3, by1 = 4.0f * B1, by2 = 4.0f * B2, by3 = 4.0f * B3;
    s.ov[0] = x0 && y0 && k1 >= 0.0f && k2 >= 0.0f && k3 >= 0.0f;
    s.ov[1] = x1 && y0 && k1 + ax1 >= 0.0f && k2 + ax2 >= 0.0f && k3 + ax3 >= 0.0f;
    s.ov[2] = x0 && y1 && k1 + by1 >= 0.0f && k2 + by2 >= 0.0f && k3 + by3 >= 0.0f;
    s.ov[3] = x1 && y1 && k1 + ax1 + by1 >= 0.0f && k2 + ax2 + by2 >= 0.0f && k3 + ax3 + by3 >= 0.0f;
    return s;
}

__device__ __forceinline__ void write_dummy_row(float *row, int lane)
{
    if (lane < ROW)
    {
        float v = 0.0f;
        if (lane == 0 || lane == 1 || lane == 3 || lane == 4) v = 1000.0f;
        if (lane == 2 || lane == 5) v = 1001.0f;
        if (lane == 6) v = 1.0f;
        if (lane == 18) v = __int_as_float(0x7fffffff);
        row[lane] = v;
    }
}

struct Bary { float p1x, p1y, p2x, p2y, p3x, p3y, a1, a2, a3, mn, ecc; };
__device__ __forceinline__ Bary barycentrics(const float4 &q0, const float4 &q1, float fx, float fy)
{
    Bary b;
    b.p1x = q0.x - fx; b.p1y = q0.y - fy; b.p2x = q0.z - fx; b.p2y = q0.w - fy; b.p3x = q1.x - fx; b.p3y = q1.y - fy;
    b.a1 = (b.p2x * b.p3y - b.p2y * b.p3x) * q1.z;
    b.a2 = (b.p3x * b.p1y - b.p3y * b.p1x) * q1.z;
    b.a3 = 1.0f - b.a1 - b.a2;
    b.mn = fminf(fminf(b.a1, b.a2), b.a3);
    b.ecc = fmaf(-3.0f, b.mn, 1.0f);
    return b;
}
#ifdef TS2D_STATS
__device__ unsigned long long g_stats_group[12];
#define TSG_STAT(i, v) stat_acc[i] += (unsigned long long)(v)
#else
#define TSG_STAT(i, v)
#endif

#if TSG_PART & 1
template <bool RICH, bool GAMMA1>
__global__ void __launch_bounds__(256, TSG_FWD_WAVES) render_fwd_group_kernel(RenderArgs a, const uint2 *__restrict__ ranges,
                                                                const uint32_t *__restrict__ point_list, const float4 *__restrict__ rec,
                                                                float *__restrict__ final_T, uint32_t *__restrict__ n_contrib,
                                                                float *__restrict__ out_feature, float *__restrict__ out_depth,
                                                                float *__restrict__ out_normal, float *__restrict__ contrib_sum,
                                                                float *__restrict__ contrib_max)
{
    __shared__ __attribute__((aligned(16))) float cst_all[4][(NR + 1) * ROW];
    __shared__ __attribute__((aligned(16))) uint32_t list_all[4][4 * NR / 2];
    constexpr int TCAP = TSG_TCAP;
    __shared__ unsigned long long tsum[RICH ? TCAP : 1];
    __shared__ int tmax[RICH ? TCAP : 1];

    const int tile = tile_of_block(blockIdx.x, a.grid_x, a.grid_y);
    if (tile < 0) return;
    const int wave = threadIdx.x >> 6;
    const GroupPixel p = group_pixel(a, tile, wave);
    const int lane = p.lane;
    const float fx = (float)p.lx, fy = (float)p.ly, OX = (float)p.X0, OY = (float)p.Y0;
    const uint2 range = ranges[tile];
    const int len = (int)(range.y - range.x);
    if (RICH) tile_stats_clear<TCAP>(tsum, tmax, len);
    const float g2 = 2.0f * a.gamma;
    float *cst = cst_all[wave] + ROW;
    uint32_t *list = list_all[wave];
    write_dummy_row(cst - ROW, lane);
    const char *lds0 = (const char *)cst_all;
    const uint32_t row0 = table_row0(wave, ROW), dummy = row0 - ROW * 4;
    const int stat_step = window_stat_step(lane);
    FwdPixel P = fwd_pixel(p.inside, len);

#ifdef TS2D_STATS
    unsigned long long stat_acc[12] = {0, 0, 0, 0, 0, 1, 0, 0, 0, 0, 0, 0};
#endif
    uint32_t id = 0;
    int pos = 0, cursor = 0;
    for (;;)
    {
        const unsigned long long alive = ballot(!P.done);
        if (alive == 0) break;
        int nq = 0;
        stream_refill<false, TSG_FWD_CAP>(id, pos, nq, point_list + range.x, cursor, len, TS_ID_BITS + wave, lane);
        if (nq == 0) break;
        const bool valid = lane < nq;
        const int ent = pos;
        float4 r0 = make_float4(0, 0, 0, 0), r1 = r0, r2 = r0, r3 = r0;
        gather_record<RICH>(rec, id, valid, r0, r1, r2, r3);
        const BlockCull s = block_cull<GAMMA1>(r0.x, r0.y, r0.z, r0.w, r1.x, r1.y, r1.z, g2, OX, OY);
        unsigned long long M[4];
        const unsigned long long any = fwd_block_masks(M, alive, valid, s.ov);
        TSG_STAT(0, __popcll(ballot(valid)));
        if (any == 0) continue;
        TSG_STAT(1, __popcll(M[0]) + __popcll(M[1]) + __popcll(M[2]) + __popcll(M[3]));
        TSG_STAT(6, 1);
        TSG_STAT(7, __popcll(any));
        const Compaction cp = compact_rows(any, lane);
        bool mine = in_pass(cp, false);
        if (mine) publish_row(cst + cp.r * ROW, s, id, ent, r1, r2, r3);
        for (int h = 0;;)
        {
            const int steps = build_lists(list, M, pass_mask(cp, mine), row0, cp.r, ROW, dummy, lane);
            const u16a *mylist = (const u16a *)list + p.grp * NR;
            TSG_STAT(2, steps);
            TSG_STAT(3, (steps + 7) / 8);
            TSG_STAT(8, __popcll(list_conflicts(list, dummy, lane)));
            TSG_STAT(9, 1);
            TSG_STAT(10, h > 0 ? 1 : 0);

            for (int t0 = 0; t0 < steps; t0 += 8)
            {
                float c[8];
                const uint4 packed = *(const uint4 *)(mylist + t0);
#pragma unroll
                for (int st = 0; st < 8; st++)
                {
                    c[st] = 0.0f;
                    if (t0 + st < steps)
                    {
                        const float *row = window_row(lds0, packed, st);
                        const float4 q0 = *(const float4 *)(row), q1 = *(const float4 *)(row + 4);
                        const Bary b = barycentrics(q0, q1, fx, fy);
                        const float4 q2 = *(const float4 *)(row + 8);
                        float4 q3 = make_float4(0, 0, 0, 0);
                        float vd3 = 0.0f;
                        int jpos;
                        if (RICH)
                        {
                            q3 = *(const float4 *)(row + 12);
                            const float4 q4 = *(const float4 *)(row + 16);
                            vd3 = q4.x;
                            jpos = __float_as_int(q4.z);
                        }
                        else jpos = __float_as_int(row[18]);
                        const float pw = GAMMA1 ? b.ecc * b.ecc : pow_nonneg(b.ecc, g2);
                        const float alpha = fminf(0.99f, q1.w * __builtin_amdgcn_exp2f(pw * -0.7213475204444817f));
                        const bool hit = !P.done && ecc_in_range(b.ecc) && alpha >= 1.0f / 255.0f;
                        TSG_STAT(4, __popcll(ballot(hit)));
                        const float d = q3.z * b.a1 + q3.w * b.a2 + vd3 * b.a3;
                        const float contrib = fwd_blend<RICH>(P, hit, alpha, q2.x, q2.y, q2.z, q2.w, q3.x, q3.y, d, jpos);
                        if (RICH) c[st] = contrib;
                    }
                }
                if (RICH) window_stats<TCAP>(c, lane, stat_step, lds0, mylist, t0, 18, tsum, tmax, point_list + range.x, contrib_sum, contrib_max);
            }
            if (++h * NR >= cp.nact) break;
            mine = in_pass(cp, true);
            if (mine) republish_row<RICH>(cst + cp.r * ROW, point_list, rec, range.x + pos, ent, OX, OY);
        }
    }

#ifdef TS2D_STATS
    if (lane == 0)
        for (int i = 0; i < 12; i++) atomicAdd(&g_stats_group[i], stat_acc[i]);
#endif
    fwd_store_pixel<RICH>(a, p, P, final_T, n_contrib, out_feature, out_depth, out_normal);
    if (RICH) tile_stats_leave<TCAP>(tsum, tmax, len, point_list + range.x, contrib_sum, contrib_max);
}

#endif

#if TSG_PART & 2
template <bool RICH, bool GAMMA1>
__global__ void __launch_bounds__(64, TSG_BWD_WAVES) render_bwd_group_kernel(RenderArgs a, const uint2 *__restrict__ ranges,
                                                             const uint32_t *__restrict__ point_list, const float4 *__restrict__ rec,
                                                             const float *__restrict__ final_T, const uint32_t *__restrict__ n_contrib,
                                                             const float *__restrict__ dL_dout_feature,
                                                             const float *__restrict__ dL_dout_depth,
                                                             const float *__restrict__ dL_dout_normal, float *__restrict__ grad_rec)
{
    __shared__ __attribute__((aligned(16))) float rows_all[(NR + 1) * BROW];
    __shared__ __attribute__((aligned(16))) uint32_t list[4 * NR / 2];

    int quad;
    const int tile = tile_of_quadrant_block(blockIdx.x, a.grid_x, a.grid_y, quad);
    if (tile < 0) return;
    const GroupPixel p = group_pixel(a, tile, quad);
    const int lane = p.lane, grp = p.grp, sub = p.sub;
    const float fx = (float)p.lx, fy = (float)p.ly, OX = (float)p.X0, OY = (float)p.Y0;
    const uint2 range = ranges[tile];
    const float g2 = 2.0f * a.gamma;
    float *rows = rows_all + BROW;
    write_dummy_row(rows - BROW, lane);
    char *lds0 = (char *)rows_all;
    const uint32_t row0 = table_row0(0, BROW), dummy = row0 - BROW * 4;
    const uint32_t accoff = ROW * 4 + 4 * sub;

    const BwdPixel P = bwd_pixel<RICH>(a, p, final_T, n_contrib, dL_dout_feature, dL_dout_depth, dL_dout_normal);
    float T = P.T, B = P.B;
    const int last = P.last;
    const float dpr = P.dpr, dpg = P.dpg, dpb = P.dpb, dnx = P.dnx, dny = P.dny, dnz = P.dnz, dd = P.dd;
    const int quarter = sub >> 2;
    const float kq0 = quarter == 0 ? dpr : (quarter == 1 ? dpg : (quarter == 2 ? dpb : dnx));
    const float kq1 = quarter == 0 ? dpb : (quarter == 1 ? dnx : (quarter == 2 ? dpr : dpg));
    const float kq2 = quarter == 0 ? dpg : (quarter == 1 ? dpr : (quarter == 2 ? dnx : dpb));
    const float kq3 = quarter == 0 ? dnx : (quarter == 1 ? dpb : (quarter == 2 ? dpg : dpr));
    const float kp4 = (sub & 8) ? dnz : dny, kp5 = (sub & 8) ? dny : dnz;
    const int rcol = (int)((0xF15ADC39E0486B27ull >> (4 * sub)) & 15ull);
    int glast[4];
    const int maxlast = block_lasts(last, glast);
    if (maxlast <= 0) return;

    uint32_t id = 0;
    int pos = 0, cursor = maxlast;
    for (;;)
    {
        int nq = 0;
        stream_refill<true, TSG_BWD_CAP>(id, pos, nq, point_list + range.x, cursor, maxlast, TS_ID_BITS + quad, lane);
        if (nq == 0) break;
        const bool valid = lane < nq;
        const int ent = pos;
        float4 r0 = make_float4(0, 0, 0, 0), r1 = r0, r2 = r0, r3 = r0;
        gather_record<RICH>(rec, id, valid, r0, r1, r2, r3);
        const BlockCull s = block_cull<GAMMA1>(r0.x, r0.y, r0.z, r0.w, r1.x, r1.y, r1.z, g2, OX, OY);
        unsigned long long M[4];
        const unsigned long long any = bwd_block_masks(M, valid, s.ov, pos, glast);
        if (any == 0) continue;
        const Compaction cp = compact_rows(any, lane);
        bool mine = in_pass(cp, false);
        if (mine) publish_row(rows + cp.r * BROW, s, id, ent, r1, r2, r3);
        for (int h = (cp.nact - 1) / NR;;)
        {
            const unsigned long long mm = pass_mask(cp, mine);
            if (mine) zero_sums(rows + cp.r * BROW + ROW);
            const int steps = build_lists(list, M, mm, row0, cp.r, BROW, dummy, lane);
            const u16a *mylist = (const u16a *)list + grp * NR;
            const unsigned long long conflict = list_conflicts(list, dummy, lane);
            uint32_t ra_next = mylist[0];
            for (int t0 = 0; t0 < steps; t0++)
            {
                {
                    const uint32_t ra = ra_next;
                    ra_next = mylist[min(t0 + 1, NR - 1)];
                    const float *row = (const float *)(lds0 + ra);
                    float *acc = (float *)(lds0 + ra + accoff);
                    const bool shared_row = (conflict >> t0) & 1;
                    const float q0acc = *acc;
                    const float4 q0 = *(const float4 *)(row), q1 = *(const float4 *)(row + 4);
                    const Bary b = barycentrics(q0, q1, fx, fy);
                    const float4 q2 = *(const float4 *)(row + 8);
                    float4 q3 = make_float4(0, 0, 0, 0);
                    float vd3 = 0.0f;
                    int jpos;
                    if (RICH)
                    {
                        q3 = *(const float4 *)(row + 12);
                        const float4 q4 = *(const float4 *)(row + 16);
                        vd3 = q4.x;
                        jpos = __float_as_int(q4.z);
                    }
                    else jpos = __float_as_int(row[18]);
                    const float pw = GAMMA1 ? b.ecc * b.ecc : pow_nonneg(b.ecc, g2);
                    const float G = __builtin_amdgcn_exp2f(pw * -0.7213475204444817f);
                    const float opG = q1.w * G;
                    const float alpha = fminf(0.99f, opG);
                    const bool hit = (jpos < last) && ecc_in_range(b.ecc) && alpha >= 1.0f / 255.0f;
                    const float al = hit ? alpha : 0.0f;
                    const float oma = 1.0f - al;
                    T = T * __builtin_amdgcn_rcpf(oma);
                    const float contrib = al * T;
                    float X = fmaf(dpb, q2.z, fmaf(dpg, q2.y, dpr * q2.x));
                    float w = 0.0f;
                    if (RICH)
                    {
                        X = fmaf(dnz, q3.y, fmaf(dny, q3.x, fmaf(dnx, q2.w, X)));
                        const float depth = fmaf(vd3, b.a3, fmaf(q3.w, b.a2, q3.z * b.a1));
                        X = fmaf(dd, depth, X);
                        w = dd * contrib;
                    }
                    const float dL_dcontrib = X - B;
                    B = fmaf(al, X, oma * B);
                    const float dL_dalpha = dL_dcontrib * T;
                    const float zr = GAMMA1 ? 1.5f * g2 * (dL_dalpha * alpha) * b.ecc
                                            : 1.5f * g2 * (dL_dalpha * alpha) * pw * __builtin_amdgcn_rcpf(b.ecc + 1e-8f);
                    const float z = (hit && opG < 0.99f) ? zr : 0.0f;
                    const bool k1 = b.a1 == b.mn;
                    const bool k2 = !k1 && b.a2 == b.mn;
                    const float z1 = k1 ? z : 0.0f, z2 = k2 ? z : 0.0f, z3 = z - z1 - z2;
                    const float da1 = fmaf(w, q3.z, z1), da2 = fmaf(w, q3.w, z2), da3 = fmaf(w, vd3, z3);
                    const float sdot = fmaf(da3, b.a3, fmaf(da2, b.a2, da1 * b.a1));
                    const float e1 = da1 - sdot, e2 = da2 - sdot, e3 = da3 - sdot;
                    float v[16];
                    v[0] = kq0 * contrib; v[1] = kq1 * contrib; v[2] = kq2 * contrib; v[3] = kq3 * contrib;
                    v[4] = kp4 * contrib; v[5] = kp5 * contrib;
                    v[6] = e3 * b.p2y - e2 * b.p3y;
                    v[7] = e2 * b.p3x - e3 * b.p2x;
                    v[8] = e1 * b.p3y - e3 * b.p1y;
                    v[9] = e3 * b.p1x - e1 * b.p3x;
                    v[10] = e2 * b.p1y - e1 * b.p2y;
                    v[11] = e1 * b.p2x - e2 * b.p1x;
                    v[12] = hit ? dL_dalpha * G : 0.0f;
                    v[13] = w * b.a1; v[14] = w * b.a2; v[15] = w * b.a3;
                    const float red = row_reduce16c(v, 0xCCCCCCCCCCCCCCCCull, 0xAAAAAAAAAAAAAAAAull);
                    row_add(acc, q0acc, red, shared_row, grp);
                }
            }

            {
                const int n = __popcll(mm);
#pragma unroll 1
                for (int e0 = 0; e0 < n; e0 += 4)
                {
                    const int e = e0 + grp;
                    if (e < n)
                    {
                        const uint32_t eid = __float_as_uint(rows[e * BROW + 17]);
                        float val = rows[e * BROW + ROW + sub];
                        if (rcol < 6) val *= rows[e * BROW + 6];
                        if (RICH || rcol < 10) unsafeAtomicAdd(grad_rec + TS_GRAD_FLOATS * (size_t)eid + rcol, val);
                    }
                }
            }
            if (--h < 0) break;
            mine = in_pass(cp, true);
            if (mine) republish_row<RICH>(rows + cp.r * BROW, point_list, rec, range.x + pos, ent, OX, OY);
        }
    }
}
#endif
}

#if TSG_PART & 1
void ts_launch_render_fwd_group(const RenderArgs &a, const GeometryStateView &g, const BinningStateView &b, const ImageStateView &im,
                                float *out_feature, float *out_depth, float *out_normal, float *contrib_sum, float *contrib_max,
                                hipStream_t s)
{
    if (a.grid_x * a.grid_y == 0) return;
    TS_LAUNCH_BLEND(render_fwd_group_kernel, a, ts_tile_units(a.grid_x, a.grid_y), 256, s, a, im.ranges, b.vals, g.rec, im.final_T, im.n_contrib,
                    out_feature, out_depth, out_normal, contrib_sum, contrib_max);
}

#endif

#if defined(TS2D_STATS) && (TSG_PART & 1)
extern "C" __attribute__((visibility("default"))) int ts2d_stats_read_group(unsigned long long *out, int reset)
{
    hipError_t e = hipMemcpyFromSymbol(out, HIP_SYMBOL(g_stats_group), sizeof(unsigned long long) * 12);
    if (e == hipSuccess && reset)
    {
        unsigned long long z[12] = {0};
        e = hipMemcpyToSymbol(HIP_SYMBOL(g_stats_group), z, sizeof(z));
    }
    return e == hipSuccess ? 0 : 2;
}
#endif

#if TSG_PART & 2
void ts_launch_render_bwd_group(const RenderArgs &a, const GeometryStateView &g, const BinningStateView &b, const ImageStateView &im,
                                const float *dL_dout_feature, const float *dL_dout_depth, const float *dL_dout_normal, float *grad_rec,
                                hipStream_t s)
{
    if (a.grid_x * a.grid_y == 0) return;
    TS_LAUNCH_BLEND(render_bwd_group_kernel, a, ts_quadrant_units(a.grid_x, a.grid_y), 64, s, a, im.ranges, b.vals, g.rec, im.final_T, im.n_contrib,
                    dL_dout_feature, dL_dout_depth, dL_dout_normal, grad_rec);
}
#endif
```

triangle-splatting_amd/csrc/ts2d_common.h:

```cpp
#pragma once
#include <hip/hip_runtime.h>
#include <stddef.h>
#include <stdint.h>

#define TS_TILE 16
#define TS_ALIGN 256

#define TS_REC_FLOATS 16

#define TS_ID_BITS 28
#define TS_ID_MASK 0x0FFFFFFFu
#define TS_GRAD_FLOATS 16

#ifndef TS_RS_CHUNK
#define TS_RS_CHUNK 4096
#endif
#define TS_RS_CHUNK_MID 2048
#define TS_RS_CHUNK_SMALL 1024
#define TS_RS_SMALL_BELOW 2500000
static inline int ts_instance_chunk(size_t n) { return n <= (size_t)TS_RS_SMALL_BELOW ? TS_RS_CHUNK_SMALL : TS_RS_CHUNK; }
static inline int ts_depth_chunk(size_t n) { return n <= (size_t)TS_RS_SMALL_BELOW ? TS_RS_CHUNK_SMALL : TS_RS_CHUNK_MID; }
#define TS_RS_BINS 256
#define TS_RS_TICKET_EXTRA 8
struct RadixScratchView
{
    uint32_t *table;
    uint32_t *slabtot;
    uint32_t *binbase;
    uint32_t *tickets;
    uint32_t *slabacc[2];
    int chunks, slabs;
    int chunk;
};

struct GeometryStateView
{
    float4 *rec;
    float *depth;
    uint32_t *tiles_touched;
    uint2 *rect;
    uint8_t *clamped;
    uint32_t *sk[2], *sv[2];
    uint32_t *depth_sorted;
    uint32_t *perm;
    uint32_t *top_const;
    uint32_t *tiles_sorted;
    uint32_t *offsets;
    uint64_t *blocksum;
    uint64_t *supersum;
    RadixScratchView rs;
};

struct BinningStateView
{
    uint32_t *k[2], *v[2];
    uint32_t *tile;
    uint32_t *vals;
    int passes;
    RadixScratchView rs;
};

struct ImageStateView
{
    uint2 *ranges;
    uint32_t *n_contrib;
    float *final_T;
    int32_t *status;
};

static inline size_t ts_align_up(size_t v) { return (v + TS_ALIGN - 1) & ~(size_t)(TS_ALIGN - 1); }

template <typename T>
static inline void ts_carve(char *&p, T *&out, size_t count)
{
    p = (char *)ts_align_up((size_t)p);
    out = (T *)p;
    p += count * sizeof(T);
}

static inline void ts_carve_radix(char *&p, size_t n, RadixScratchView &r, int chunk = TS_RS_CHUNK, int reserve_chunk = 0)
{
    r.chunk = chunk;
    r.chunks = (int)((n + chunk - 1) / chunk);
    r.slabs = (r.chunks + 63) / 64;
    const int rc = reserve_chunk > 0 ? reserve_chunk : chunk;
    const size_t chunks = (n + rc - 1) / rc, slabs = (chunks + 63) / 64;
    ts_carve(p, r.table, chunks * TS_RS_BINS);
    ts_carve(p, r.slabtot, slabs * TS_RS_BINS);
    ts_carve(p, r.binbase, (size_t)TS_RS_BINS);
    ts_carve(p, r.tickets, slabs + TS_RS_TICKET_EXTRA);
    ts_carve(p, r.slabacc[0], slabs * TS_RS_BINS);
    ts_carve(p, r.slabacc[1], slabs * TS_RS_BINS);
}

static inline size_t ts_carve_geometry(char *base, int32_t P, GeometryStateView &v)
{
    char *p = base;
    size_t n = (size_t)(P > 0 ? P : 0);
    ts_carve(p, v.rec, n * 4);
    ts_carve(p, v.depth, n);
    ts_carve(p, v.tiles_touched, n);
    ts_carve(p, v.rect, n);
    ts_carve(p, v.clamped, n);
    ts_carve(p, v.sk[0], n);
    ts_carve(p, v.sk[1], n);
    ts_carve(p, v.sv[0], n);
    ts_carve(p, v.sv[1], n);
    v.depth_sorted = v.sk[1];
    v.perm = v.sv[1];
    ts_carve(p, v.tiles_sorted, n);
    ts_carve(p, v.offsets, n);
    ts_carve(p, v.blocksum, (n + 1023) / 1024 + 2);
    ts_carve(p, v.supersum, ((n + 1023) / 1024 + 63) / 64 + 1);
    ts_carve_radix(p, n, v.rs, ts_depth_chunk(n));
    v.top_const = v.rs.tickets + v.rs.slabs + 4;
    return (size_t)(p - base) + TS_ALIGN;
}

static inline int ts_higher_msb(uint32_t n)
{
    uint32_t msb = sizeof(n) * 4, step = msb;
    while (step > 1)
    {
        step /= 2;
        if (n >> msb) msb += step;
        else msb -= step;
    }
    if (n >> msb) msb++;
    return (int)msb;
}

static inline int ts_tile_bits(int ntiles) { return ts_higher_msb((uint32_t)(ntiles > 1 ? ntiles - 1 : 1)); }

static inline size_t ts_carve_binning(char *base, int64_t N, int32_t W, int32_t H, BinningStateView &v)
{
    char *p = base;
    size_t n = (size_t)(N > 0 ? N : 0);
    int gx = (W + TS_TILE - 1) / TS_TILE, gy = (H + TS_TILE - 1) / TS_TILE;
    ts_carve(p, v.k[0], n);
    ts_carve(p, v.k[1], n);
    ts_carve(p, v.v[0], n);
    ts_carve(p, v.v[1], n);
    v.passes = (ts_tile_bits(gx * gy) + 7) / 8;
    v.tile = v.k[v.passes & 1];
    v.vals = v.v[v.passes & 1];
    ts_carve_radix(p, n, v.rs, ts_instance_chunk(n), TS_RS_CHUNK_SMALL);
    return (size_t)(p - base) + TS_ALIGN;
}

static inline int64_t ts_binning_capacity(size_t bytes, int32_t W, int32_t H)
{
    BinningStateView v;
    if (bytes < ts_carve_binning(nullptr, 0, W, H, v)) return -1;
    int64_t lo = 0, hi = (int64_t)(bytes / 16) + 1;
    if (hi > 0x7fffffffll) hi = 0x7fffffffll;
    while (lo < hi)
    {
        const int64_t mid = lo + (hi - lo + 1) / 2;
        if (ts_carve_binning(nullptr, mid, W, H, v) <= bytes) lo = mid;
        else hi = mid - 1;
    }
    return lo;
}

static inline void ts_binning_set_count(BinningStateView &v, int64_t n)
{
    v.rs.chunks = (int)((n + v.rs.chunk - 1) / v.rs.chunk);
    v.rs.slabs = (v.rs.chunks + 63) / 64;
}

static inline size_t ts_carve_image(char *base, int32_t W, int32_t H, ImageStateView &v)
{
    char *p = base;
    int gx = (W + TS_TILE - 1) / TS_TILE, gy = (H + TS_TILE - 1) / TS_TILE;
    ts_carve(p, v.ranges, (size_t)gx * gy);
    ts_carve(p, v.n_contrib, (size_t)W * H);
    ts_carve(p, v.final_T, (size_t)W * H);
    ts_carve(p, v.status, (size_t)4);
    return (size_t)(p - base) + TS_ALIGN;
}

struct PreprocessArgs
{
    int W, H, P, D, M, C;
    int grid_x, grid_y;
    bool rich_info, use_shs, back_culling;
    float tan_fovx, tan_fovy;
    const float *viewmatrix, *projmatrix, *campos;
    const float *vertex, *shs, *feature, *opacity;
};

void ts_launch_preprocess_fwd(const PreprocessArgs &a, int32_t *radii, const GeometryStateView &g, hipStream_t s);
void ts_sort_by_depth_begin(const GeometryStateView &g, int32_t P, unsigned long long *host_out, hipStream_t s);
void ts_sort_by_depth_finish(const GeometryStateView &g, int32_t P, hipStream_t s);
void ts_scan_offsets(const GeometryStateView &g, int32_t P, hipStream_t s);
struct QuadMaskArgs
{
    int variant;
    float g2;
    float tan_fovx, tan_fovy;
    int W, H;
    float inv_W, inv_H;
};
void ts_launch_zero_words(uint32_t *p, size_t n, hipStream_t s);
void ts_launch_emit_keys(int P, int grid_x, int ntiles, const GeometryStateView &g, const BinningStateView &b, const ImageStateView &im,
                         float *contrib_sum, float *contrib_max, int64_t capacity, int32_t *status, const QuadMaskArgs &qm, hipStream_t s);
const unsigned long long *ts_instance_count_dev(const GeometryStateView &g, int P);
void ts_sort_pairs(const BinningStateView &b, int64_t N, const unsigned long long *n_dev, int ntiles, hipStream_t s);
void ts_launch_tile_ranges(int64_t N, const unsigned long long *n_dev, const BinningStateView &b, const ImageStateView &im, hipStream_t s);
size_t ts_quantile_scratch_bytes();
void ts_quantile_threshold(const uint32_t *keys, size_t n, float q, void *scratch, float *thr, hipStream_t s);
void ts_quantile_passes(const uint32_t *keys, size_t n, float q, void *scratch, int first_pass, hipStream_t s);
size_t ts_quantile_state_words();
size_t ts_radix_scratch_bytes(size_t n);
int ts_radix_sort_pairs(uint32_t *const k[2], uint32_t *const v[2], size_t n, int end_bit, void *scratch, hipStream_t s, bool force_tickets = false);
void ts_force_ticket_passes(bool on);
void ts_force_depth_pass4(bool on);
void ts_lab_depth_split(int mode, int bucket_cap);

struct RenderArgs
{
    int W, H, C, grid_x, grid_y;
    float gamma, background_depth;
    const float *background;
    const float *background_depth_dev;
    bool rich_info;
};
void ts_launch_render_fwd_group(const RenderArgs &a, const GeometryStateView &g, const BinningStateView &b,
                                const ImageStateView &im, float *out_feature, float *out_depth, float *out_normal,
                                float *contrib_sum, float *contrib_max, hipStream_t s);
void ts_launch_render_bwd_group(const RenderArgs &a, const GeometryStateView &g, const BinningStateView &b,
                                const ImageStateView &im, const float *dL_dout_feature, const float *dL_dout_depth,
                                const float *dL_dout_normal, float *grad_rec, hipStream_t s);
void ts_launch_preprocess_bwd(const PreprocessArgs &a, const int32_t *radii, const GeometryStateView &g,
                              const float *grad_rec, float *dL_dvertex, float *dL_dcenter2D, float *dL_dshs,
                              float *dL_dfeature, float *dL_dopacity, hipStream_t s);

void ts_launch_preprocess3d_fwd(const PreprocessArgs &a, int32_t *radii, const GeometryStateView &g, hipStream_t s);
void ts_launch_preprocess3d_bwd(const PreprocessArgs &a, const int32_t *radii, const GeometryStateView &g,
                                const float *grad_rec, float *dL_dvertex, float *dL_dcenter2D, float *dL_dshs,
                                float *dL_dfeature, float *dL_dopacity, hipStream_t s);

void ts_launch_render3d_fwd_group(const RenderArgs &a, float tan_fovx, float tan_fovy, const GeometryStateView &g,
                                  const BinningStateView &b, const ImageStateView &im, float *out_feature, float *out_depth,
                                  float *out_normal, float *contrib_sum, float *contrib_max, hipStream_t s);
void ts_launch_render3d_bwd_group(const RenderArgs &a, float tan_fovx, float tan_fovy, const GeometryStateView &g,
                                  const BinningStateView &b, const ImageStateView &im, const float *dL_dout_feature,
                                  const float *dL_dout_depth, const float *dL_dout_normal, float *grad_rec, hipStream_t s);

struct MeshArgs
{
    int W, H, V, F, grid_x, grid_y;
    float tan_fovx, tan_fovy, znear;
    const float *viewmatrix;
    const float *vertices;
    const int32_t *faces;
};
void ts_launch_mesh_preprocess(const MeshArgs &a, const GeometryStateView &g, hipStream_t s);
void ts_launch_mesh_resolve(const MeshArgs &a, const GeometryStateView &g, const BinningStateView &b, const ImageStateView &im,
                            const float *faces_color, const float *background, float *render, float *mask, float *depth, int32_t *face_idx,
                            unsigned long long *wave_visits, hipStream_t s);
void ts_launch_mesh_census(int W, int H, int F, const int32_t *face_idx, const float *target, const float *pixel_mask, unsigned long long *census,
                           hipStream_t s);

void ts_launch_sh_grad_expand(int P, int D, int M, int V, const float *vertex, const float *campos, const float *dL_dcolor,
                              float *dL_dshs, hipStream_t s);

size_t ts_loss_workspace_bytes(int C, int H, int W);
hipError_t ts_loss_forward(const float *image, const float *gt, int C, int H, int W, float w_l1, float w_ssim, bool need_grad,
                           void *workspace, float *out, hipStream_t s);
hipError_t ts_loss_backward(const float *image, const float *gt, int C, int H, int W, float w_l1, float w_ssim, const void *workspace,
                            const float *grad_out, float *dL_dimage, hipStream_t s);

size_t ts_aux_loss_workspace_bytes(int C, int H, int W, double scale);
hipError_t ts_dog_mask(const float *gt, int C, int H, int W, double sigma1, int ksize1, double sigma2, int ksize2, int invert, double scale, void *workspace,
                       float *mask, hipStream_t s);
hipError_t ts_smoothness_mask(const float *gt, int C, int H, int W, double scale, float quantile, void *workspace, float *mask, hipStream_t s);
hipError_t ts_masked_l1_forward(const float *img, const float *gt, const float *mask, int C, int H, int W, void *workspace, float *out, hipStream_t s);
hipError_t ts_masked_l1_backward(const float *img, const float *gt, const float *mask, int C, int H, int W, const float *grad_out, float *dimg, hipStream_t s);
hipError_t ts_scharr_smoothness_forward(const float *img, const float *mask, int C, int H, int W, void *workspace, float *out, hipStream_t s);
hipError_t ts_scharr_smoothness_backward(const float *img, const float *mask, int C, int H, int W, void *workspace, const float *grad_out, float *dimg,
                                         hipStream_t s);
hipError_t ts_downsample_forward(const float *in, int C, int H, int W, int h, int w, float *out, hipStream_t s);
hipError_t ts_downsample_backward(const float *gout, int C, int H, int W, int h, int w, float *gin, hipStream_t s);
hipError_t ts_downsample_forward_planes(int n, const float *const *src, int H, int W, int h, int w, float *const *dst, hipStream_t s);
hipError_t ts_downsample_backward_planes(int n, const float *const *gout, int H, int W, int h, int w, float *const *gin, hipStream_t s);
size_t ts_depth_normal_workspace_bytes(int H, int W, double scale);
hipError_t ts_depth_normal_forward(const float *depth, const float *normal, int H, int W, float tan_fovx, float tan_fovy, double scale, float quantile,
                                   void *workspace, float *out, hipStream_t s);
hipError_t ts_depth_normal_backward(const float *depth, const float *normal, int H, int W, float tan_fovx, float tan_fovy, double scale,
                                    const void *workspace, const float *grad_out, float *dL_ddepth, float *dL_dnormal, hipStream_t s);

size_t ts_reg_workspace_bytes();
size_t ts_reg_prepared_bytes(int P);
hipError_t ts_reg_prepare(int P, const uint32_t *nearest, void *prepared, hipStream_t s);
hipError_t ts_reg_forward(int P, const float *vertex, const float *opacity, const uint32_t *nearest, float w_s, float w_o, int omode, float w_v,
                          void *workspace, float *out, hipStream_t s);
hipError_t ts_reg_backward(int P, const float *vertex, const float *opacity, const uint32_t *nearest, const void *prepared, float w_s, float w_o,
                           int omode, float w_v, const float *grad_out, float *dvertex, float *dopacity, hipStream_t s);
hipError_t ts_color_affine_forward(const float *x, int H, int W, const float *Wm, const float *b, float *y, hipStream_t s);
hipError_t ts_color_affine_backward(const float *x, int H, int W, const float *Wm, const float *b, const float *gy, void *workspace, float *gx,
                                    float *dW, float *db, hipStream_t s);

size_t ts_knn_workspace_bytes(int P);
hipError_t ts_knn_mean_dist3(int P, const float *points, float *mean_dist2, void *ws, hipStream_t s);
hipError_t ts_knn_nearest_other(int P, int group, const float *points, uint32_t *nearest, void *ws, hipStream_t s);

struct tso_adam_slice;
struct tso_sh_factored_step;
hipError_t ts_optim_adam_step(const tso_adam_slice *slices, int n, double beta1, double beta2, double eps, hipStream_t s);
hipError_t ts_optim_adam_step_sh_factored(const tso_sh_factored_step &a, double beta1, double beta2, double eps, hipStream_t s);

hipError_t ts_model_training_statistic(int P, int V, const int32_t *radii, const float *c2d_grad, const float *csum, const float *cmax,
                                       float *g_accum, float *g_denom, float *max_radii, float *s_csum, float *s_cmax, float *c_denom,
                                       hipStream_t s);
size_t ts_model_select_scratch_bytes(int P);
hipError_t ts_model_select_rows(int P, const uint8_t *mask, int match, uint32_t *pos, uint32_t *scratch, uint32_t *count_host, hipStream_t s);
hipError_t ts_model_scatter_rows(int64_t rows, int row_words, const uint32_t *pos, const void *src, void *dst, int64_t dst_row0, hipStream_t s);
hipError_t ts_model_gather_rows(int64_t rows, int row_words, const uint32_t *idx, const void *src, void *dst, int64_t dst_row0, hipStream_t s);
hipError_t ts_model_grow_classify(int P, const float *vertex, float *g_accum, float *g_denom, float min_view_count, float grad_threshold,
                                  float split_scale_threshold, uint8_t *code, hipStream_t s);
hipError_t ts_model_split_vertex(int n_split, const uint32_t *parents, const float *vertex, float *child1, float *child2, hipStream_t s);
hipError_t ts_model_update_mask(int P, int mode, const float *opacity, const float *vertex, const float *max_radii, float a, float b, uint8_t *mask,
                                hipStream_t s);
hipError_t ts_model_clip(int P, int mode, const uint8_t *mask, float value, float *param, float *exp_avg, float *exp_avg_sq, hipStream_t s);
hipError_t ts_model_opacity_reset(int P, float reset_value, float *opacity, float *exp_avg, float *exp_avg_sq, hipStream_t s);
hipError_t ts_model_max_distance(int n_vertices, const float *vertex, const float *campos, float *out, hipStream_t s);
hipError_t ts_model_state_digest(int n, const void *const *segments, const uint64_t *num_words, uint64_t *digests, hipStream_t s);
```

triangle-splatting_amd/csrc/ts2d_group.h:

```cpp
#pragma once
#include "ts2d_common.h"
#include "ts2d_wave.h"

namespace
{
constexpr int NR = 32;
typedef unsigned short __attribute__((may_alias)) u16a;
constexpr int ROW = 20;

__device__ __forceinline__ unsigned long long ballot(bool p) { return __builtin_amdgcn_ballot_w64(p); }
__device__ __forceinline__ int lane_rank(unsigned long long m)
{
    return (int)__builtin_amdgcn_mbcnt_hi((uint32_t)(m >> 32), __builtin_amdgcn_mbcnt_lo((uint32_t)m, 0u));
}

__device__ __forceinline__ bool ecc_in_range(float ecc) { return __float_as_uint(ecc) <= 0x41200000u; }

template <bool DESC, int CAP = 64>
__device__ __forceinline__ void stream_refill(uint32_t &id, int &pos, int &n, const uint32_t *__restrict__ list, int &cursor, int end, int qbit, int lane)
{
    while (n < CAP && (DESC ? cursor > 0 : cursor < end))
    {
        const int k = DESC ? cursor - 1 - lane : cursor + lane;
        const bool valid = DESC ? k >= 0 : k < end;
        const uint32_t v = valid ? list[k] : 0u;
        const bool want = valid && ((v >> qbit) & 1u);
        unsigned long long mt = ballot(want);
        int adv = 64;
        const int room = CAP - n;
        bool taken = want;
        if (__popcll(mt) > room)
        {
            taken = want && lane_rank(mt) < room;
            mt = ballot(taken);
            adv = 64 - __builtin_clzll(mt);
        }
        cursor += DESC ? -adv : adv;
        if (mt == 0) continue;
        const int cnt = __popcll(mt), rk = lane_rank(mt);
        const int dest = (taken ? n + rk : n + cnt + (lane - rk)) & 63;
        const uint32_t pid = (uint32_t)__builtin_amdgcn_ds_permute(dest << 2, (int)(v & TS_ID_MASK));
        const int ppos = __builtin_amdgcn_ds_permute(dest << 2, k);
        const bool fresh = lane >= n && lane < n + cnt;
        id = fresh ? pid : id;
        pos = fresh ? ppos : pos;
        n += cnt;
    }
}

__device__ __forceinline__ void row_reduce8_sum_max(const float (&c)[8], unsigned long long mask_b1, float &sum, float &mx)
{
    float s0, s1, s2, s3, m0, m1, m2, m3;
#define TSG8_L1(OP, T, X, Y)                                                              \
    OP " " T ", " Y ", " Y " row_ror:8 row_mask:0xf bank_mask:0xc\n"                      \
    OP " " T ", " X ", " X " row_ror:8 row_mask:0xf bank_mask:0x3\n"
#define TSG8_L2(OP, X, Y)                                                                 \
    OP " " Y ", " Y ", " Y " row_half_mirror row_mask:0xf bank_mask:0xa\n"                \
    OP " " Y ", " X ", " X " row_half_mirror row_mask:0xf bank_mask:0x5\n"
#define TSG8_QP(OP, X, QP) OP " " X ", " X ", " X " quad_perm:" QP " row_mask:0xf bank_mask:0xf\n"
    asm volatile("s_nop 1\n"
                 TSG8_L1("v_add_f32_dpp", "%0", "%8", "%9") TSG8_L1("v_add_f32_dpp", "%1", "%10", "%11")
                 TSG8_L1("v_add_f32_dpp", "%2", "%12", "%13") TSG8_L1("v_add_f32_dpp", "%3", "%14", "%15")
                 TSG8_L1("v_max_f32_dpp", "%4", "%8", "%9") TSG8_L1("v_max_f32_dpp", "%5", "%10", "%11")
                 TSG8_L1("v_max_f32_dpp", "%6", "%12", "%13") TSG8_L1("v_max_f32_dpp", "%7", "%14", "%15")
                 TSG8_L2("v_add_f32_dpp", "%0", "%1") TSG8_L2("v_max_f32_dpp", "%4", "%5")
                 TSG8_L2("v_add_f32_dpp", "%2", "%3") TSG8_L2("v_max_f32_dpp", "%6", "%7")
                 TSG8_QP("v_add_f32_dpp", "%1", "[2,3,0,1]") TSG8_QP("v_max_f32_dpp", "%5", "[2,3,0,1]")
                 TSG8_QP("v_add_f32_dpp", "%3", "[2,3,0,1]") TSG8_QP("v_max_f32_dpp", "%7", "[2,3,0,1]")
                 "v_cndmask_b32_e64 %3, %1, %3, %16\n"
                 "v_cndmask_b32_e64 %7, %5, %7, %16\n"
                 "s_nop 0\n"
                 TSG8_QP("v_add_f32_dpp", "%3", "[1,0,3,2]") TSG8_QP("v_max_f32_dpp", "%7", "[1,0,3,2]")
                 "s_nop 1\n"
                 : "=&v"(s0), "=&v"(s1), "=&v"(s2), "=&v"(s3), "=&v"(m0), "=&v"(m1), "=&v"(m2), "=&v"(m3)
                 : "v"(c[0]), "v"(c[1]), "v"(c[2]), "v"(c[3]), "v"(c[4]), "v"(c[5]), "v"(c[6]), "v"(c[7]), "s"(mask_b1));
#undef TSG8_L1
#undef TSG8_L2
#undef TSG8_QP
    sum = s3;
    mx = m3;
}

__device__ __forceinline__ float row_reduce16(float (&v)[16], unsigned long long mask_b1, unsigned long long mask_b0)
{
#define TSG_L1(X, Y)                                                                    \
    "v_add_f32_dpp " Y ", " Y ", " Y " row_ror:8 row_mask:0xf bank_mask:0xc\n"         \
    "v_add_f32_dpp " Y ", " X ", " X " row_ror:8 row_mask:0xf bank_mask:0x3\n"
#define TSG_L2(X, Y)                                                                    \
    "v_add_f32_dpp " Y ", " Y ", " Y " row_half_mirror row_mask:0xf bank_mask:0xa\n"   \
    "v_add_f32_dpp " Y ", " X ", " X " row_half_mirror row_mask:0xf bank_mask:0x5\n"
#define TSG_L3(X, Y, QP, M)                                                             \
    "v_add_f32_dpp " X ", " X ", " X " quad_perm:" QP " row_mask:0xf bank_mask:0xf\n"  \
    "v_add_f32_dpp " Y ", " Y ", " Y " quad_perm:" QP " row_mask:0xf bank_mask:0xf\n"  \
    "v_cndmask_b32_e64 " Y ", " X ", " Y ", " M "\n"
    asm volatile("s_nop 1\n"
                 TSG_L1("%0", "%1") TSG_L1("%2", "%3") TSG_L1("%4", "%5") TSG_L1("%6", "%7")
                 TSG_L1("%8", "%9") TSG_L1("%10", "%11") TSG_L1("%12", "%13") TSG_L1("%14", "%15")
                 TSG_L2("%1", "%3") TSG_L2("%5", "%7") TSG_L2("%9", "%11") TSG_L2("%13", "%15")
                 TSG_L3("%3", "%7", "[2,3,0,1]", "%16") TSG_L3("%11", "%15", "[2,3,0,1]", "%16")
                 "v_add_f32_dpp %7, %7, %7 quad_perm:[1,0,3,2] row_mask:0xf bank_mask:0xf\n"
                 "s_nop 0\n"
                 "v_add_f32_dpp %15, %15, %15 quad_perm:[1,0,3,2] row_mask:0xf bank_mask:0xf\n"
                 "v_cndmask_b32_e64 %15, %7, %15, %17\n"
                 "s_nop 1\n"
                 : "+v"(v[0]), "+v"(v[1]), "+v"(v[2]), "+v"(v[3]), "+v"(v[4]), "+v"(v[5]), "+v"(v[6]), "+v"(v[7]), "+v"(v[8]),
                   "+v"(v[9]), "+v"(v[10]), "+v"(v[11]), "+v"(v[12]), "+v"(v[13]), "+v"(v[14]), "+v"(v[15])
                 : "s"(mask_b1), "s"(mask_b0));
#undef TSG_L1
#undef TSG_L2
#undef TSG_L3
    return v[15];
}
__device__ __forceinline__ float row_reduce16c(float (&v)[16], unsigned long long mask_b1, unsigned long long mask_b0)
{
#define TSG_L1(X, Y)                                                                    \
    "v_add_f32_dpp " Y ", " Y ", " Y " row_ror:8 row_mask:0xf bank_mask:0xc\n"         \
    "v_add_f32_dpp " Y ", " X ", " X " row_ror:8 row_mask:0xf bank_mask:0x3\n"
#define TSG_L1C(X, Y) "v_add_f32_dpp " Y ", " Y ", " X " row_ror:8 row_mask:0xf bank_mask:0xf\n"
#define TSG_L2(X, Y)                                                                    \
    "v_add_f32_dpp " Y ", " Y ", " Y " row_half_mirror row_mask:0xf bank_mask:0xa\n"   \
    "v_add_f32_dpp " Y ", " X ", " X " row_half_mirror row_mask:0xf bank_mask:0x5\n"
#define TSG_L3(X, Y, QP, M)                                                             \
    "v_add_f32_dpp " X ", " X ", " X " quad_perm:" QP " row_mask:0xf bank_mask:0xf\n"  \
    "v_add_f32_dpp " Y ", " Y ", " Y " quad_perm:" QP " row_mask:0xf bank_mask:0xf\n"  \
    "v_cndmask_b32_e64 " Y ", " X ", " Y ", " M "\n"
    asm volatile("s_nop 1\n"
                 TSG_L1C("%0", "%1") TSG_L1C("%2", "%3") TSG_L1C("%4", "%5") TSG_L1("%6", "%7")
                 TSG_L1("%8", "%9") TSG_L1("%10", "%11") TSG_L1("%12", "%13") TSG_L1("%14", "%15")
                 "v_add_f32_dpp %3, %3, %1 row_half_mirror row_mask:0xf bank_mask:0xf\n"
                 TSG_L2("%5", "%7") TSG_L2("%9", "%11") TSG_L2("%13", "%15")
                 TSG_L3("%3", "%7", "[2,3,0,1]", "%16") TSG_L3("%11", "%15", "[2,3,0,1]", "%16")
                 "v_add_f32_dpp %7, %7, %7 quad_perm:[1,0,3,2] row_mask:0xf bank_mask:0xf\n"
                 "s_nop 0\n"
                 "v_add_f32_dpp %15, %15, %15 quad_perm:[1,0,3,2] row_mask:0xf bank_mask:0xf\n"
                 "v_cndmask_b32_e64 %15, %7, %15, %17\n"
                 "s_nop 1\n"
                 : "+v"(v[0]), "+v"(v[1]), "+v"(v[2]), "+v"(v[3]), "+v"(v[4]), "+v"(v[5]), "+v"(v[6]), "+v"(v[7]), "+v"(v[8]),
                   "+v"(v[9]), "+v"(v[10]), "+v"(v[11]), "+v"(v[12]), "+v"(v[13]), "+v"(v[14]), "+v"(v[15])
                 : "s"(mask_b1), "s"(mask_b0));
#undef TSG_L1
#undef TSG_L1C
#undef TSG_L2
#undef TSG_L3
    return v[15];
}
constexpr int bitrev4(int c) { return ((c & 1) << 3) | ((c & 2) << 1) | ((c & 4) >> 1) | ((c & 8) >> 3); }


__device__ __forceinline__ unsigned long long to_fixed48(float x)
{
    const float y = x * 0x1p48f;
    const uint32_t hi = (uint32_t)(y * 0x1p-32f);
    const float rem = fmaf(-(float)hi, 0x1p32f, y);
    return ((unsigned long long)hi << 32) | (unsigned long long)(uint32_t)rem;
}
__device__ __forceinline__ void global_stats_add(uint32_t tid, float sm, float mx, float *contrib_sum, float *contrib_max)
{
    unsafeAtomicAdd(contrib_sum + tid, sm);
    if (mx > contrib_max[tid]) atomicMax((int *)contrib_max + tid, __float_as_int(mx));
}
template <int TCAP>
__device__ __forceinline__ void tile_stats_add(unsigned long long *tsum, int *tmax, int k, float sm, float mx, const uint32_t *tile_list,
                                               float *contrib_sum, float *contrib_max)
{
    if (k < TCAP)
    {
        __hip_atomic_fetch_add(tsum + k, to_fixed48(sm), __ATOMIC_RELAXED, __HIP_MEMORY_SCOPE_WORKGROUP);
        __hip_atomic_fetch_max(tmax + k, __float_as_int(mx), __ATOMIC_RELAXED, __HIP_MEMORY_SCOPE_WORKGROUP);
    }
    else global_stats_add(tile_list[k] & TS_ID_MASK, sm, mx, contrib_sum, contrib_max);
}
__device__ __forceinline__ void tile_stats_flush(unsigned long long fx48, int mxbits, uint32_t tid, float *contrib_sum, float *contrib_max)
{
    global_stats_add(tid, (float)((double)fx48 * 0x1p-48), __int_as_float(mxbits), contrib_sum, contrib_max);
}

struct GroupPixel
{
    int lane, grp, sub;
    int X0, Y0, lx, ly, px, py;
    bool inside;
};
__device__ __forceinline__ GroupPixel group_pixel(const RenderArgs &a, int tile, int quad)
{
    GroupPixel p;
    const int tx = tile % a.grid_x, ty = tile / a.grid_x;
    p.lane = threadIdx.x & 63;
    p.grp = p.lane >> 4; p.sub = p.lane & 15;
    p.X0 = tx * TS_TILE + (quad & 1) * 8; p.Y0 = ty * TS_TILE + (quad >> 1) * 8;
    p.lx = ((p.grp & 1) << 2) + (p.sub & 3); p.ly = ((p.grp >> 1) << 2) + (p.sub >> 2);
    p.px = p.X0 + p.lx; p.py = p.Y0 + p.ly;
    p.inside = p.px < a.W && p.py < a.H;
    return p;
}
// ... 244 lines not shown
```

triangle-splatting_amd/csrc/ts2d_lab.h:

```cpp
#ifndef TS2D_LAB_H
#define TS2D_LAB_H

#include "../../include/ts2d.h"

#ifdef __cplusplus
extern "C" {
#endif

int ts2d_debug_read_state(const ts2d_state *state, int32_t P, int64_t num_rendered, int32_t width, int32_t height,
                          int32_t field, void *dst, size_t dst_bytes, void *stream);

int ts2d_test_sort_pairs(const uint32_t *keys_in, const uint32_t *vals_in, uint32_t *keys_out, uint32_t *vals_out, size_t n,
                         int32_t end_bit, int32_t which, void *stream);
int ts2d_test_inclusive_scan_rocprim(const uint32_t *in, uint32_t *out, size_t n, void *stream);

void ts2d_lab_force_ticket_passes(int on);
void ts2d_lab_force_depth_pass4(int on);
size_t ts2d_test_quantile_scratch_bytes(void);
int ts2d_test_quantile(const uint32_t *keys, size_t n, float q, void *scratch, float *out, void *stream);
void ts2d_lab_depth_split(int mode, int bucket_cap);
void ts2d_lab_force_all_quadrants(int on);

#ifdef __cplusplus
}
#endif
#endif
```

triangle-splatting_amd/csrc/ts2d_support.h:

```cpp
#pragma once
#include "ts2d_wave.h"

#include "ts2d_common.h"

namespace
{
template <bool GAMMA1>
__device__ __forceinline__ float support_scale(float op, float g2)
{
    const float t = 255.0f * op;
    float E = -1.0f;
    if (t >= 1.0f)
    {
        const float L = 2.0f * 0.6931471805599453f * __builtin_amdgcn_logf(t);
        if (GAMMA1) E = __builtin_amdgcn_sqrtf(L);
        else E = (g2 < 1e-6f) ? 10.0f : pow_nonneg(L, 1.0f / g2);
        E = fminf(E * 1.0005f + 0.002f, 10.01f);
    }
    return E;
}

struct QuadSetup
{
    float v1x, v1y, v2x, v2y, v3x, v3y, ia;
    float A1, B1, A2, B2, A3, B3;
    float P1, P2, P3;
    float bminx, bmaxx, bminy, bmaxy;
    bool live;
};
__device__ __forceinline__ QuadSetup quad_setup(float v1x, float v1y, float v2x, float v2y, float v3x, float v3y, float E, float pad_px = 0.0f)
{
    QuadSetup q;
    q.v1x = v1x; q.v1y = v1y; q.v2x = v2x; q.v2y = v2y; q.v3x = v3x; q.v3y = v3y;
    const float area2 = __fsub_rn(__fmul_rn(v2x - v1x, v3y - v1y), __fmul_rn(v2y - v1y, v3x - v1x));
    q.ia = __builtin_amdgcn_rcpf(area2);
    q.A1 = (v2y - v3y) * q.ia; q.B1 = (v3x - v2x) * q.ia;
    q.A2 = (v3y - v1y) * q.ia; q.B2 = (v1x - v3x) * q.ia;
    q.A3 = -q.A1 - q.A2; q.B3 = -q.B1 - q.B2;
    const float m = (1.0f - E) * (1.0f / 3.0f);
    const float slope_margin = 2e-6f * 15.0f + pad_px;
    q.P1 = fmaxf(0.0f, 7.0f * q.A1) + fmaxf(0.0f, 7.0f * q.B1) - m + slope_margin * (fabsf(q.A1) + fabsf(q.B1));
    q.P2 = fmaxf(0.0f, 7.0f * q.A2) + fmaxf(0.0f, 7.0f * q.B2) - m + slope_margin * (fabsf(q.A2) + fabsf(q.B2));
    q.P3 = fmaxf(0.0f, 7.0f * q.A3) + fmaxf(0.0f, 7.0f * q.B3) - m + slope_margin * (fabsf(q.A3) + fabsf(q.B3));
    const float cx = (v1x + v2x + v3x) * (1.0f / 3.0f), cy = (v1y + v2y + v3y) * (1.0f / 3.0f);
    const float e1x = E * (v1x - cx), e2x = E * (v2x - cx), e3x = E * (v3x - cx);
    const float e1y = E * (v1y - cy), e2y = E * (v2y - cy), e3y = E * (v3y - cy);
    const float padx = 0.05f + pad_px + 4e-7f * fabsf(cx), pady = 0.05f + pad_px + 4e-7f * fabsf(cy);
    q.bminx = cx + fminf(fminf(e1x, e2x), e3x) - padx; q.bmaxx = cx + fmaxf(fmaxf(e1x, e2x), e3x) + padx;
    q.bminy = cy + fminf(fminf(e1y, e2y), e3y) - pady; q.bmaxy = cy + fmaxf(fmaxf(e1y, e2y), e3y) + pady;
    q.live = E > 0.0f;
    return q;
}
__device__ __forceinline__ QuadSetup quad_setup_all()
{
    QuadSetup q{};
    q.P1 = q.P2 = q.P3 = 1e30f;
    q.bminx = q.bminy = -3e38f;
    q.bmaxx = q.bmaxy = 3e38f;
    q.live = true;
    return q;
}
constexpr float PAD3D = 0.02f;
__device__ __forceinline__ QuadSetup quad_setup_3d(const float4 &r0, const float4 &r1, const float4 &r2, float E, float tan_fovx, float tan_fovy, int W, int H,
                                                   float inv_W, float inv_H, float px0, float py0, float px1, float py1)
{
    {
        const float nx = r2.y, ny = r2.z, nz = r2.w;
        const float sx = tan_fovx * inv_W, sy = tan_fovy * inv_H;
        const float rx0 = sx * (2.0f * px0 - (float)W + 1.0f), rx1 = sx * (2.0f * px1 - (float)W + 1.0f);
        const float ry0 = sy * (2.0f * py0 - (float)H + 1.0f), ry1 = sy * (2.0f * py1 - (float)H + 1.0f);
        const float d00 = rx0 * nx + ry0 * ny + nz, d10 = rx1 * nx + ry0 * ny + nz, d01 = rx0 * nx + ry1 * ny + nz, d11 = rx1 * nx + ry1 * ny + nz;
        const float lo = fminf(fminf(d00, d10), fminf(d01, d11)), hi = fmaxf(fmaxf(d00, d10), fmaxf(d01, d11));
        const float big = fmaxf(fabsf(lo), fabsf(hi));
        if (!(lo > 1e-3f * big || hi < -1e-3f * big)) return quad_setup_all();
    }
    const float v1x = r0.x, v1y = r0.y, v1z = r0.z, v2x = r0.w, v2y = r1.x, v2z = r1.y, v3x = r1.z, v3y = r1.w, v3z = r2.x;
    const float cx = (v1x + v2x + v3x) * (1.0f / 3.0f), cy = (v1y + v2y + v3y) * (1.0f / 3.0f), cz = (v1z + v2z + v3z) * (1.0f / 3.0f);
    const float w1z = cz + E * (v1z - cz), w2z = cz + E * (v2z - cz), w3z = cz + E * (v3z - cz);
    const float zmin = 0.05f * cz;
    if (!(E > 0.0f && cz > 0.0f && w1z >= zmin && w2z >= zmin && w3z >= zmin)) return quad_setup_all();
    const float kx = 0.5f * (float)W * __builtin_amdgcn_rcpf(tan_fovx), ky = 0.5f * (float)H * __builtin_amdgcn_rcpf(tan_fovy);
    const float ox = 0.5f * (float)W - 0.5f, oy = 0.5f * (float)H - 0.5f;
    const float i1 = __builtin_amdgcn_rcpf(w1z), i2 = __builtin_amdgcn_rcpf(w2z), i3 = __builtin_amdgcn_rcpf(w3z);
    const float s1x = (cx + E * (v1x - cx)) * i1 * kx + ox, s1y = (cy + E * (v1y - cy)) * i1 * ky + oy;
    const float s2x = (cx + E * (v2x - cx)) * i2 * kx + ox, s2y = (cy + E * (v2y - cy)) * i2 * ky + oy;
    const float s3x = (cx + E * (v3x - cx)) * i3 * kx + ox, s3y = (cy + E * (v3y - cy)) * i3 * ky + oy;
    const float area2 = (s2x - s1x) * (s3y - s1y) - (s2y - s1y) * (s3x - s1x);
    const float span = fmaxf(fmaxf(fabsf(s2x - s1x), fabsf(s3x - s1x)), fmaxf(fabsf(s2y - s1y), fabsf(s3y - s1y)));
    if (!(fabsf(area2) > 1e-3f * span) || !(span < 1e7f)) return quad_setup_all();
    return quad_setup(s1x, s1y, s2x, s2y, s3x, s3y, 1.0f, PAD3D);
}
__device__ __forceinline__ uint32_t quadrant_mask(const QuadSetup &q, float TX, float TY)
{
    const float u1x = q.v1x - TX, u1y = q.v1y - TY, u2x = q.v2x - TX, u2y = q.v2y - TY, u3x = q.v3x - TX, u3y = q.v3y - TY;
    const float t1a = u2x * u3y, t1b = u2y * u3x, t2a = u3x * u1y, t2b = u3y * u1x, aia = fabsf(q.ia);
    const float C1 = (t1a - t1b) * q.ia, C2 = (t2a - t2b) * q.ia;
    const float C3 = 1.0f - C1 - C2;
    const float r1 = 4e-7f * (fabsf(t1a) + fabsf(t1b)) * aia, r2 = 4e-7f * (fabsf(t2a) + fabsf(t2b)) * aia;
    const float k1 = C1 + q.P1 + r1, k2 = C2 + q.P2 + r2, k3 = C3 + q.P3 + (r1 + r2 + 4e-7f);
    const float ax1 = 8.0f * q.A1, ax2 = 8.0f * q.A2, ax3 = 8.0f * q.A3, by1 = 8.0f * q.B1, by2 = 8.0f * q.B2, by3 = 8.0f * q.B3;
    const bool x0 = q.live && q.bminx <= TX + 7.0f && q.bmaxx >= TX, x1 = q.live && q.bminx <= TX + 15.0f && q.bmaxx >= TX + 8.0f;
    const bool y0 = q.bminy <= TY + 7.0f && q.bmaxy >= TY, y1 = q.bminy <= TY + 15.0f && q.bmaxy >= TY + 8.0f;
    uint32_t m = 0;
    m |= (x0 && y0 && k1 >= 0.0f && k2 >= 0.0f && k3 >= 0.0f) ? 1u : 0u;
    m |= (x1 && y0 && k1 + ax1 >= 0.0f && k2 + ax2 >= 0.0f && k3 + ax3 >= 0.0f) ? 2u : 0u;
    m |= (x0 && y1 && k1 + by1 >= 0.0f && k2 + by2 >= 0.0f && k3 + by3 >= 0.0f) ? 4u : 0u;
    m |= (x1 && y1 && k1 + ax1 + by1 >= 0.0f && k2 + ax2 + by2 >= 0.0f && k3 + ax3 + by3 >= 0.0f) ? 8u : 0u;
    return m;
}

struct QuadAffine { float4 a, b, c, d; };
__device__ __forceinline__ QuadAffine quad_anchor(const QuadSetup &q, uint32_t id, uint32_t minx, uint32_t miny, uint32_t w, uint32_t h)
{
    const float TX = (float)(minx * TS_TILE), TY = (float)(miny * TS_TILE), Wpx = (float)((w - 1u) * TS_TILE), Hpx = (float)((h - 1u) * TS_TILE);
    const float u1x = q.v1x - TX, u1y = q.v1y - TY, u2x = q.v2x - TX, u2y = q.v2y - TY, u3x = q.v3x - TX, u3y = q.v3y - TY;
    const float aia = fabsf(q.ia);
    const float C1 = (u2x * u3y - u2y * u3x) * q.ia, C2 = (u3x * u1y - u3y * u1x) * q.ia;
    const float C3 = 1.0f - C1 - C2;
    const float U1x = fmaxf(fabsf(u1x), fabsf(u1x - Wpx)), U1y = fmaxf(fabsf(u1y), fabsf(u1y - Hpx));
    const float U2x = fmaxf(fabsf(u2x), fabsf(u2x - Wpx)), U2y = fmaxf(fabsf(u2y), fabsf(u2y - Hpx));
    const float U3x = fmaxf(fabsf(u3x), fabsf(u3x - Wpx)), U3y = fmaxf(fabsf(u3y), fabsf(u3y - Hpx));
    const float r1 = 4e-7f * (U2x * U3y + U2y * U3x) * aia, r2 = 4e-7f * (U3x * U1y + U3y * U1x) * aia;
    const float s1 = 6e-7f * (fabsf(q.A1) * Wpx + fabsf(q.B1) * Hpx) + 2.5e-7f * fabsf(C1);
    const float s2 = 6e-7f * (fabsf(q.A2) * Wpx + fabsf(q.B2) * Hpx) + 2.5e-7f * fabsf(C2);
    const float s3 = 6e-7f * (fabsf(q.A3) * Wpx + fabsf(q.B3) * Hpx) + 2.5e-7f * fabsf(C3);
    QuadAffine o;
    o.a = make_float4(C1 + q.P1 + r1 + s1, C2 + q.P2 + r2 + s2, C3 + q.P3 + (r1 + r2 + 4e-7f) + s3, q.A1);
    o.b = make_float4(q.A2, q.A3, q.B1, q.B2);
    o.c = make_float4(q.B3, q.live ? q.bminx : 3e38f, q.live ? q.bmaxx : -3e38f, q.bminy);
    o.d = make_float4(q.bmaxy, __uint_as_float(id), __uint_as_float(minx | (miny << 16)), 0.0f);
    return o;
}
__device__ __forceinline__ uint32_t quadrant_mask_affine(const QuadAffine &o, uint32_t dx, uint32_t dy, uint32_t x, uint32_t y)
{
    const float fx = (float)(dx * TS_TILE), fy = (float)(dy * TS_TILE), TX = (float)(x * TS_TILE), TY = (float)(y * TS_TILE);
    const float A1 = o.a.w, A2 = o.b.x, A3 = o.b.y, B1 = o.b.z, B2 = o.b.w, B3 = o.c.x;
    const float k1 = fmaf(B1, fy, fmaf(A1, fx, o.a.x)), k2 = fmaf(B2, fy, fmaf(A2, fx, o.a.y)), k3 = fmaf(B3, fy, fmaf(A3, fx, o.a.z));
    const float ax1 = 8.0f * A1, ax2 = 8.0f * A2, ax3 = 8.0f * A3, by1 = 8.0f * B1, by2 = 8.0f * B2, by3 = 8.0f * B3;
    const float bminx = o.c.y, bmaxx = o.c.z, bminy = o.c.w, bmaxy = o.d.x;
    const bool x0 = bminx <= TX + 7.0f && bmaxx >= TX, x1 = bminx <= TX + 15.0f && bmaxx >= TX + 8.0f;
    const bool y0 = bminy <= TY + 7.0f && bmaxy >= TY, y1 = bminy <= TY + 15.0f && bmaxy >= TY + 8.0f;
    uint32_t m = 0;
    m |= (x0 && y0 && k1 >= 0.0f && k2 >= 0.0f && k3 >= 0.0f) ? 1u : 0u;
    m |= (x1 && y0 && k1 + ax1 >= 0.0f && k2 + ax2 >= 0.0f && k3 + ax3 >= 0.0f) ? 2u : 0u;
    m |= (x0 && y1 && k1 + by1 >= 0.0f && k2 + by2 >= 0.0f && k3 + by3 >= 0.0f) ? 4u : 0u;
    m |= (x1 && y1 && k1 + ax1 + by1 >= 0.0f && k2 + ax2 + by2 >= 0.0f && k3 + ax3 + by3 >= 0.0f) ? 8u : 0u;
    return m;
}
}
```

triangle-splatting_amd/diff_triangle_rasterization_2D/_abi.py:

```python
import ctypes as C

_vp = C.c_void_p


class _Camera(C.Structure):
    _fields_ = [("width", C.c_int32), ("height", C.c_int32), ("tan_fovx", C.c_float), ("tan_fovy", C.c_float),
                ("viewmatrix", _vp), ("projmatrix", _vp), ("campos", _vp)]


class _Geometry(C.Structure):
    _fields_ = [("P", C.c_int32), ("sh_degree", C.c_int32), ("M", C.c_int32), ("C", C.c_int32),
                ("gamma", C.c_float), ("scale_modifier", C.c_float), ("background_depth", C.c_float),
                ("background", _vp), ("vertex", _vp), ("shs", _vp), ("feature", _vp), ("opacity", _vp), ("background_depth_dev", _vp)]


class _ForwardOut(C.Structure):
    _fields_ = [("out_feature", _vp), ("depth", _vp), ("normal", _vp), ("contrib_sum", _vp), ("contrib_max", _vp)]


class _LossGrads(C.Structure):
    _fields_ = [("dL_dout_feature", _vp), ("dL_dout_depth", _vp), ("dL_dout_normal", _vp)]


class _BackwardOut(C.Structure):
    _fields_ = [("dL_dvertex", _vp), ("dL_dcenter2D", _vp), ("dL_dshs", _vp), ("dL_dfeature", _vp),
                ("dL_dopacity", _vp)]


class _State(C.Structure):
    _fields_ = [("geometry", _vp), ("geometry_bytes", C.c_size_t), ("binning", _vp), ("binning_bytes", C.c_size_t),
                ("image", _vp), ("image_bytes", C.c_size_t)]


class _Slice(C.Structure):
    _fields_ = [("param", _vp), ("grad", _vp), ("exp_avg", _vp), ("exp_avg_sq", _vp), ("count", C.c_int64), ("step_size", C.c_float),
                ("bias2_sqrt", C.c_float), ("grad_scale", C.c_float), ("step_size_tail", C.c_float), ("index0", C.c_int64),
                ("period", C.c_int32), ("split", C.c_int32)]


class _RowSlice(C.Structure):
    _fields_ = [("param", _vp), ("grad", _vp), ("exp_avg", _vp), ("exp_avg_sq", _vp), ("floats_per_row", C.c_int32), ("step_size", C.c_float),
                ("bias2_sqrt", C.c_float), ("grad_scale", C.c_float)]


SH_ROW_SLICES = 2


class _ShFactoredStep(C.Structure):
    _fields_ = [("P", C.c_int32), ("M", C.c_int32), ("sh_degree", C.c_int32), ("V", C.c_int32), ("vertex", _vp), ("campos", _vp), ("dL_dcolor", _vp),
                ("param_dc", _vp), ("exp_avg_dc", _vp), ("exp_avg_sq_dc", _vp), ("param_rest", _vp), ("exp_avg_rest", _vp), ("exp_avg_sq_rest", _vp),
                ("dc_stride", C.c_int64), ("rest_stride", C.c_int64), ("step_size_dc", C.c_float), ("bias2_sqrt_dc", C.c_float),
                ("step_size_rest", C.c_float), ("bias2_sqrt_rest", C.c_float), ("grad_scale", C.c_float), ("num_rows", C.c_int32),
                ("rows", _RowSlice * SH_ROW_SLICES)]


SIGNATURES = {
    "ts2d_version": (C.c_char_p, []),
    "ts2d_last_error": (C.c_char_p, []),
    "ts2d_geometry_state_bytes": (C.c_size_t, [C.c_int32]),
    "ts2d_binning_state_bytes": (C.c_size_t, [C.c_int64, C.c_int32, C.c_int32]),
    "ts2d_image_state_bytes": (C.c_size_t, [C.c_int32, C.c_int32]),
    "ts2d_backward_scratch_bytes": (C.c_size_t, [C.c_int32]),
    "ts2d_binning_capacity": (C.c_int64, [C.c_size_t, C.c_int32, C.c_int32]),
    "ts2d_forward_bin": (C.c_int, [C.POINTER(_Camera), C.POINTER(_Geometry), C.c_uint32, _vp, C.POINTER(_State), C.POINTER(C.c_int64), _vp]),
    "ts2d_forward_render": (C.c_int, [C.POINTER(_Camera), C.POINTER(_Geometry), C.c_uint32, C.c_int64, C.POINTER(_State), C.POINTER(_ForwardOut),
                                      _vp]),
    "ts2d_backward": (C.c_int, [C.POINTER(_Camera), C.POINTER(_Geometry), C.c_uint32, C.c_int64, _vp, C.POINTER(_State), C.POINTER(_LossGrads), _vp,
                                C.c_size_t, C.POINTER(_BackwardOut), _vp]),
    "ts2d_backward_ranged": (C.c_int, [C.POINTER(_Camera), C.POINTER(_Geometry), C.c_uint32, C.c_int64, _vp, C.POINTER(_State),
                                       C.POINTER(_LossGrads), _vp, C.c_size_t, C.POINTER(_BackwardOut), C.c_int32, C.POINTER(_vp), _vp]),
    "ts2d_backward_range_rows": (C.c_int32, [C.c_int32, C.c_int32]),
    "ts2d_forward": (C.c_int, [C.POINTER(_Camera), C.POINTER(_Geometry), C.c_uint32, _vp, C.POINTER(_State), C.c_int64, C.POINTER(_ForwardOut), _vp]),
    "ts2d_forward_speculative": (C.c_int, [C.POINTER(_Camera), C.POINTER(_Geometry), C.c_uint32, _vp, C.POINTER(_State), C.POINTER(_ForwardOut),
                                           C.POINTER(C.c_int64), _vp]),
    "ts2d_instance_capacity_hint": (C.c_int64, [C.c_int32, C.c_int32, C.c_int32, C.c_uint32]),
    "ts2d_set_capacity_hint_key": (None, [C.c_uint64]),
    "ts2d_speculative_overflow_count": (C.c_uint64, []),
    "ts2d_forward_status": (C.c_int, [C.POINTER(_State), C.c_int32, C.c_int32, C.c_int32, C.POINTER(C.c_int32), C.POINTER(C.c_int64), _vp]),
    "ts2d_sh_grad_expand": (C.c_int, [C.c_int32, C.c_int32, C.c_int32, C.c_int32, _vp, _vp, _vp, _vp, _vp]),
    "ts2d_profile_enable": (None, [C.c_int]),
    "ts2d_profile_only": (None, [C.c_char_p]),
    "ts2d_profile_reset": (None, []),
    "ts2d_profile_read": (C.c_int, [C.c_int32, C.c_char_p, C.c_size_t, C.POINTER(C.c_double), C.POINTER(C.c_int64)]),
    "tsl_workspace_bytes": (C.c_size_t, [C.c_int32, C.c_int32, C.c_int32]),
    "tsl_photometric_forward": (C.c_int, [_vp, _vp, C.c_int32, C.c_int32, C.c_int32, C.c_float, C.c_float, C.c_int32, _vp, C.c_size_t, _vp, _vp]),
    "tsl_photometric_backward": (C.c_int, [_vp, _vp, C.c_int32, C.c_int32, C.c_int32, C.c_float, C.c_float, _vp, C.c_size_t, _vp, _vp, _vp]),
    "tsl_depth_normal_workspace_bytes": (C.c_size_t, [C.c_int32, C.c_int32, C.c_double]),
    "tsl_depth_normal_forward": (C.c_int, [_vp, _vp, C.c_int32, C.c_int32, C.c_float, C.c_float, C.c_double, C.c_float, _vp, C.c_size_t, _vp, _vp]),
    "tsl_depth_normal_backward": (C.c_int, [_vp, _vp, C.c_int32, C.c_int32, C.c_float, C.c_float, C.c_double, _vp, C.c_size_t, _vp, _vp, _vp, _vp]),
    "tsl_aux_loss_workspace_bytes": (C.c_size_t, [C.c_int32, C.c_int32, C.c_int32, C.c_double]),
    "tsl_dog_mask": (C.c_int, [_vp, C.c_int32, C.c_int32, C.c_int32, C.c_double, C.c_int32, C.c_double, C.c_int32, C.c_int32, C.c_double, _vp,
                               C.c_size_t, _vp, _vp]),
    "tsl_smoothness_mask": (C.c_int, [_vp, C.c_int32, C.c_int32, C.c_int32, C.c_double, C.c_float, _vp, C.c_size_t, _vp, _vp]),
    "tsl_masked_l1_forward": (C.c_int, [_vp, _vp, _vp, C.c_int32, C.c_int32, C.c_int32, _vp, C.c_size_t, _vp, _vp]),
    "tsl_masked_l1_backward": (C.c_int, [_vp, _vp, _vp, C.c_int32, C.c_int32, C.c_int32, _vp, _vp, _vp]),
    "tsl_scharr_smoothness_forward": (C.c_int, [_vp, _vp, C.c_int32, C.c_int32, C.c_int32, _vp, C.c_size_t, _vp, _vp]),
    "tsl_scharr_smoothness_backward": (C.c_int, [_vp, _vp, C.c_int32, C.c_int32, C.c_int32, _vp, C.c_size_t, _vp, _vp, _vp]),
    "tsl_downsample_forward": (C.c_int, [_vp, C.c_int32, C.c_int32, C.c_int32, C.c_int32, C.c_int32, _vp, _vp]),
    "tsl_downsample_backward": (C.c_int, [_vp, C.c_int32, C.c_int32, C.c_int32, C.c_int32, C.c_int32, _vp, _vp]),
    "tsl_downsample_forward_planes": (C.c_int, [C.c_int32, C.POINTER(_vp), C.c_int32, C.c_int32, C.c_int32, C.c_int32, C.POINTER(_vp), _vp]),
    "tsl_downsample_backward_planes": (C.c_int, [C.c_int32, C.POINTER(_vp), C.c_int32, C.c_int32, C.c_int32, C.c_int32, C.POINTER(_vp), _vp]),
    "tsl_reg_workspace_bytes": (C.c_size_t, []),
    "tsl_reg_prepared_bytes": (C.c_size_t, [C.c_int32]),
    "tsl_reg_prepare": (C.c_int, [C.c_int32, _vp, _vp, C.c_size_t, _vp]),
    "tsl_reg_forward": (C.c_int, [C.c_int32, _vp, _vp, _vp, C.c_float, C.c_float, C.c_int32, C.c_float, _vp, C.c_size_t, _vp, _vp]),
    "tsl_reg_backward": (C.c_int, [C.c_int32, _vp, _vp, _vp, _vp, C.c_size_t, C.c_float, C.c_float, C.c_int32, C.c_float, _vp, _vp, _vp, _vp]),
    "tsl_color_affine_forward": (C.c_int, [_vp, C.c_int32, C.c_int32, _vp, _vp, _vp, _vp]),
    "tsl_color_affine_backward": (C.c_int, [_vp, C.c_int32, C.c_int32, _vp, _vp, _vp, _vp, C.c_size_t, _vp, _vp, _vp, _vp]),
    "tsk_workspace_bytes": (C.c_size_t, [C.c_int32]),
    "tsk_mean_dist3": (C.c_int, [C.c_int32, _vp, _vp, _vp, C.c_size_t, _vp]),
    "tsk_nearest_other": (C.c_int, [C.c_int32, C.c_int32, _vp, _vp, _vp, C.c_size_t, _vp]),
    "tsm_training_statistic": (C.c_int, [C.c_int32, C.c_int32, _vp, _vp, _vp, _vp, _vp, _vp, _vp, _vp, _vp, _vp, _vp]),
    "tsm_select_scratch_bytes": (C.c_size_t, [C.c_int32]),
    "tsm_select_rows": (C.c_int, [C.c_int32, _vp, C.c_int32, _vp, _vp, C.c_size_t, C.POINTER(C.c_uint32), _vp]),
    "tsm_scatter_rows": (C.c_int, [C.c_int64, C.c_int32, _vp, _vp, _vp, C.c_int64, _vp]),
    "tsm_gather_rows": (C.c_int, [C.c_int64, C.c_int32, _vp, _vp, _vp, C.c_int64, _vp]),
    "tsm_grow_classify": (C.c_int, [C.c_int32, _vp, _vp, _vp, C.c_float, C.c_float, C.c_float, _vp, _vp]),
    "tsm_split_vertex": (C.c_int, [C.c_int32, _vp, _vp, _vp, _vp, _vp]),
    "tsm_update_mask": (C.c_int, [C.c_int32, C.c_int32, _vp, _vp, _vp, C.c_float, C.c_float, _vp, _vp]),
    "tsm_clip": (C.c_int, [C.c_int32, C.c_int32, _vp, C.c_float, _vp, _vp, _vp, _vp]),
    "tsm_opacity_reset": (C.c_int, [C.c_int32, C.c_float, _vp, _vp, _vp, _vp]),
    "tsm_max_vertex_distance": (C.c_int, [C.c_int32, _vp, _vp, _vp, _vp]),
    "tsm_state_digest": (C.c_int, [C.c_int32, C.POINTER(_vp), C.POINTER(C.c_uint64), _vp, _vp]),
    "tso_adam_step": (C.c_int, [C.POINTER(_Slice), C.c_int32, C.c_double, C.c_double, C.c_double, _vp]),
    "tso_adam_step_sh_factored": (C.c_int, [C.POINTER(_ShFactoredStep), C.c_double, C.c_double, C.c_double, _vp]),
    "ts2d_mesh_geometry_state_bytes": (C.c_size_t, [C.c_int32]),
    "ts2d_mesh_bin": (C.c_int, [C.POINTER(_Camera), C.c_float, C.c_int32, _vp, C.c_int32, _vp, C.POINTER(_State), C.POINTER(C.c_int64), _vp]),
    "ts2d_mesh_render": (C.c_int, [C.POINTER(_Camera), C.c_int32, _vp, _vp, C.c_int64, C.POINTER(_State), _vp, _vp, _vp, _vp, _vp]),
    "ts2d_mesh_render_counted": (C.c_int, [C.POINTER(_Camera), C.c_int32, _vp, _vp, C.c_int64, C.POINTER(_State), _vp, _vp, _vp, _vp, _vp, _vp]),
    "ts2d_mesh_census_add": (C.c_int, [C.c_int32, C.c_int32, C.c_int32, _vp, _vp, _vp, _vp, _vp]),
    "ts2d_weld_workspace_bytes": (C.c_size_t, [C.c_int32, C.c_int32]),
    "ts2d_weld_labels": (C.c_int, [C.c_int32, _vp, C.c_float, _vp, _vp, C.c_size_t, _vp]),
    "ts2d_weld_labels_counted": (C.c_int, [C.c_int32, _vp, C.c_float, _vp, _vp, _vp, C.c_size_t, _vp]),
    "ts2d_weld_face_components": (C.c_int, [C.c_int32, C.c_int32, _vp, _vp, _vp, _vp, C.c_size_t, _vp]),
    "ts2d_weld_compact": (C.c_int, [C.c_int32, _vp, _vp, C.c_int32, _vp, _vp, _vp, _vp, C.c_size_t, _vp]),
    "ts2d_weld_remap_faces": (C.c_int, [C.c_int32, C.c_int32, _vp, _vp, _vp, _vp, _vp]),
    "ts2d_weld_edge_census": (C.c_int, [C.c_int32, C.c_int32, _vp, _vp, _vp, _vp, C.c_size_t, _vp]),
}

LAB_SIGNATURES = {
    "ts2d_debug_read_state": (C.c_int, [C.POINTER(_State), C.c_int32, C.c_int64, C.c_int32, C.c_int32, C.c_int32, _vp, C.c_size_t, _vp]),
    "ts2d_test_sort_pairs": (C.c_int, [_vp, _vp, _vp, _vp, C.c_size_t, C.c_int32, C.c_int32, _vp]),
    "ts2d_test_inclusive_scan_rocprim": (C.c_int, [_vp, _vp, C.c_size_t, _vp]),
    "ts2d_lab_force_ticket_passes": (None, [C.c_int]),
    "ts2d_lab_force_depth_pass4": (None, [C.c_int]),
    "ts2d_test_quantile_scratch_bytes": (C.c_size_t, []),
    "ts2d_test_quantile": (C.c_int, [_vp, C.c_size_t, C.c_float, _vp, _vp, _vp]),
    "ts2d_lab_depth_split": (None, [C.c_int, C.c_int]),
    "ts2d_lab_force_all_quadrants": (None, [C.c_int]),
}

GEOM_SIGNATURES = {
    "tsg_last_error": (C.c_char_p, []),
    "tsg_cross_workspace_bytes": (C.c_size_t, [C.c_int32, C.c_int32]),
    "tsg_nearest_cross": (C.c_int, [C.c_int32, _vp, C.c_int32, _vp, _vp, _vp, _vp, _vp, C.c_size_t, _vp]),
    "tsg_sample_workspace_bytes": (C.c_size_t, [C.c_int32]),
    "tsg_face_areas": (C.c_int, [C.c_int32, C.c_int32, _vp, _vp, _vp, _vp, _vp]),
    "tsg_sample_surface": (C.c_int, [C.c_int32, C.c_int32, _vp, _vp, _vp, C.c_int32, C.c_uint64, _vp, _vp, _vp, C.c_size_t, _vp]),
}


def bind_geom(lib):
    missing = [name for name in GEOM_SIGNATURES if not hasattr(lib, name)]
    if missing:
        raise ImportError(f"{getattr(lib, '_name', lib)} does not export {', '.join(missing)}: rebuild it with `python triangle-splatting_amd/build.py`")
    for name, (restype, argtypes) in GEOM_SIGNATURES.items():
        fn = getattr(lib, name)
        fn.restype, fn.argtypes = restype, argtypes
    return lib


def bind(lib):
    missing = [name for name in SIGNATURES if not hasattr(lib, name)]
    if missing:
        raise ImportError(f"{getattr(lib, '_name', lib)} does not export {', '.join(missing)}: rebuild it with `python triangle-splatting_amd/build.py`")
    for table in (SIGNATURES, LAB_SIGNATURES):
        for name, (restype, argtypes) in table.items():
            if table is SIGNATURES or hasattr(lib, name):
                fn = getattr(lib, name)
                fn.restype, fn.argtypes = restype, argtypes
    return lib
```

Measured before the change: 1335.

## Precompute per-tile 4x4 block masks during binning and pack into sort keys

The emit-keys kernel now computes, for each triangle-tile instance, a 16-bit mask of which 4x4 pixel blocks the triangle may cover. It stores that mask in the upper bits of the tile key, and tile_ranges masks those bits off. The forward and backward render kernels read the mask from the keys during refill instead of recomputing the per-block cull from the triangle record, which removes ALU work and lets entries that touch no relevant blocks be skipped earlier. The cost is extra key reads and more binning work, and the sort may now run over wider keys. The path is limited to 2D mode and to tile counts that fit the key bits.

```diff
diff --git a/triangle-splatting_amd/csrc/api.hip b/triangle-splatting_amd/csrc/api.hip
--- a/triangle-splatting_amd/csrc/api.hip
+++ b/triangle-splatting_amd/csrc/api.hip
@@ -45,7 +45,14 @@
 
 #ifdef TS2D_LAB
 bool g_lab_all_quadrants = false;
+bool g_lab_kernel_cull = false;
 #endif
+
+bool block_masks_in_keys(const ts2d_camera *cam, uint32_t flags)
+{
+    const int gx = (cam->width + TS_TILE - 1) / TS_TILE, gy = (cam->height + TS_TILE - 1) / TS_TILE;
+    return !(flags & TS2D_FLAG_3D) && (int64_t)gx * gy <= TS_BLOCKMASK_MAX_TILES;
+}
 
 int validate(const ts2d_camera *cam, const ts2d_geometry *geom, uint32_t flags)
 {
@@ -95,6 +102,10 @@
     r.background_depth_dev = geom->background_depth_dev;
     r.background = geom->background;
     r.rich_info = flags & TS2D_FLAG_RICH_INFO;
+    r.block_masks = block_masks_in_keys(cam, flags);
+#ifdef TS2D_LAB
+    if (g_lab_kernel_cull) r.block_masks = false;
+#endif
     return r;
 }
 
@@ -181,7 +192,8 @@
     const int ntiles = r.grid_x * r.grid_y;
     const unsigned long long *n_dev = count_on_device ? ts_instance_count_dev(g, P) : nullptr;
 
-    QuadMaskArgs quad{(flags & TS2D_FLAG_3D) ? 3 : 2, fmaxf(0.0f, 2.0f * geom->gamma), cam->tan_fovx, cam->tan_fovy, W, H, 1.0f / (float)W, 1.0f / (float)H};
+    QuadMaskArgs quad{(flags & TS2D_FLAG_3D) ? 3 : 2, fmaxf(0.0f, 2.0f * geom->gamma), cam->tan_fovx, cam->tan_fovy, W, H, 1.0f / (float)W, 1.0f / (float)H,
+                      block_masks_in_keys(cam, flags) ? 1 : 0};
 #ifdef TS2D_LAB
     if (g_lab_all_quadrants) quad.variant = 0;
 #endif
@@ -339,7 +351,7 @@
     {
         { ProfScope ps("tile_sort", s); ts_sort_pairs(b, N, n_dev, ntiles, s); }
         TS_CHECK(flags, s, "tile_sort");
-        { ProfScope ps("tile_ranges", s); ts_launch_tile_ranges(N, n_dev, b, im, s); }
+        { ProfScope ps("tile_ranges", s); ts_launch_tile_ranges(N, n_dev, ntiles, b, im, s); }
         TS_CHECK(flags, s, "tile_ranges");
     }
     return TS2D_OK;
@@ -662,7 +674,8 @@
             TS_HIP(hipStreamSynchronize(s));
         }
         uint64_t *o = (uint64_t *)dst;
-        for (int64_t i = 0; i < N; i++) o[i] = ((uint64_t)tile[i] << 32) | depth[vals[i] & TS_ID_MASK];
+        const uint32_t keymask = ts_tile_keymask(gx * gy);
+        for (int64_t i = 0; i < N; i++) o[i] = ((uint64_t)(tile[i] & keymask) << 32) | depth[vals[i] & TS_ID_MASK];
         return TS2D_OK;
     }
     case 11: src = b.vals; bytes = (size_t)N * 4; break;
@@ -697,6 +710,7 @@
 
 void ts2d_lab_force_ticket_passes(int on) { ts_force_ticket_passes(on != 0); }
 void ts2d_lab_force_all_quadrants(int on) { g_lab_all_quadrants = on != 0; }
+void ts2d_lab_force_kernel_cull(int on) { g_lab_kernel_cull = on != 0; }
 void ts2d_lab_force_depth_pass4(int on) { ts_force_depth_pass4(on != 0); }
 void ts2d_lab_depth_split(int mode, int bucket_cap) { ts_lab_depth_split(mode, bucket_cap); }
 #endif
diff --git a/triangle-splatting_amd/csrc/binning.hip b/triangle-splatting_amd/csrc/binning.hip
--- a/triangle-splatting_amd/csrc/binning.hip
+++ b/triangle-splatting_amd/csrc/binning.hip
@@ -668,6 +668,7 @@
 #ifndef TS_EMIT_WAVES
 #define TS_EMIT_WAVES 6
 #endif
+template <bool BM>
 #if TS_EMIT_WAVES > 0
 __global__ void __launch_bounds__(256, TS_EMIT_WAVES) scan_emit_kernel(
 #else
@@ -742,6 +743,7 @@
     const uint32_t minx = rect.x & 0xffffu, miny = rect.x >> 16, maxx = rect.y & 0xffffu, maxy = rect.y >> 16;
     uint32_t *tile_out = b.k[0], *val_out = b.v[0];
     constexpr bool qm = true;
+    constexpr bool bm = BM;
     const float quad_g2 = qmask.g2;
     auto setup_from = [&](const float4 &r0, const float4 &r1, const float4 &r2, uint32_t tminx, uint32_t tminy, uint32_t tmaxx, uint32_t tmaxy) {
         if (qmask.variant == 0) return quad_setup_all();
@@ -752,7 +754,7 @@
                                  (float)(tminy * TS_TILE) - 1.0f, (float)(tmaxx * TS_TILE), (float)(tmaxy * TS_TILE));
         }
         const float E = quad_g2 == 2.0f ? support_scale<true>(r1.z, quad_g2) : support_scale<false>(r1.z, quad_g2);
-        return quad_setup(r0.x, r0.y, r0.z, r0.w, r1.x, r1.y, E);
+        return quad_setup<bm ? 3 : 7>(r0.x, r0.y, r0.z, r0.w, r1.x, r1.y, E);
     };
     auto setup_of = [&](uint32_t tri, uint32_t tminx, uint32_t tminy, uint32_t tmaxx, uint32_t tmaxy) {
         const float4 *rp = g.rec + 4 * (size_t)tri;
@@ -794,8 +796,17 @@
             for (uint32_t y = miny; y < maxy; y++)
                 for (uint32_t x = minx; x < maxx; x++)
                 {
-                    tile_out[o] = y * grid_x + x;
-                    val_out[o] = qm ? id | (quadrant_mask(qs, (float)(x * TS_TILE), (float)(y * TS_TILE)) << TS_ID_BITS) : id;
+                    if (bm)
+                    {
+                        const uint32_t m16 = block_mask(qs, (float)(x * TS_TILE), (float)(y * TS_TILE));
+                        tile_out[o] = (y * grid_x + x) | (m16 << 16);
+                        val_out[o] = id | (quadrants_of_blocks(m16) << TS_ID_BITS);
+                    }
+                    else
+                    {
+                        tile_out[o] = y * grid_x + x;
+                        val_out[o] = qm ? id | (quadrant_mask(qs, (float)(x * TS_TILE), (float)(y * TS_TILE)) << TS_ID_BITS) : id;
+                    }
                     o++;
                 }
     }
@@ -819,8 +830,17 @@
             }
             else
             {
-                tile_out[t_off + k] = y * grid_x + x;
-                val_out[t_off + k] = qm ? t_id | (quadrant_mask(tq, (float)(x * TS_TILE), (float)(y * TS_TILE)) << TS_ID_BITS) : t_id;
+                if (bm)
+                {
+                    const uint32_t m16 = block_mask(tq, (float)(x * TS_TILE), (float)(y * TS_TILE));
+                    tile_out[t_off + k] = (y * grid_x + x) | (m16 << 16);
+                    val_out[t_off + k] = t_id | (quadrants_of_blocks(m16) << TS_ID_BITS);
+                }
+                else
+                {
+                    tile_out[t_off + k] = y * grid_x + x;
+                    val_out[t_off + k] = qm ? t_id | (quadrant_mask(tq, (float)(x * TS_TILE), (float)(y * TS_TILE)) << TS_ID_BITS) : t_id;
+                }
             }
         }
     }
@@ -836,8 +856,17 @@
                 QuadAffine qa;
                 qa.a = region_b[4 * slot]; qa.b = region_b[4 * slot + 1]; qa.c = region_b[4 * slot + 2]; qa.d = region_b[4 * slot + 3];
                 const uint32_t org = __float_as_uint(qa.d.z), x = (org & 0xffffu) + dx, y = (org >> 16) + dy;
-                v = __float_as_uint(qa.d.y) | (quadrant_mask_affine(qa, dx, dy, x, y) << TS_ID_BITS);
-                tl = y * grid_x + x;
+                if (bm)
+                {
+                    const uint32_t m16 = block_mask_affine(qa, dx, dy, x, y);
+                    v = __float_as_uint(qa.d.y) | (quadrants_of_blocks(m16) << TS_ID_BITS);
+                    tl = (y * grid_x + x) | (m16 << 16);
+                }
+                else
+                {
+                    v = __float_as_uint(qa.d.y) | (quadrant_mask_affine(qa, dx, dy, x, y) << TS_ID_BITS);
+                    tl = y * grid_x + x;
+                }
             }
             else v = stage_v[k];
             tile_out[run0 + k] = tl;
@@ -847,7 +876,7 @@
 }
 
 __global__ void __launch_bounds__(256) tile_ranges_kernel(int64_t N, const unsigned long long *n_dev, const uint32_t *__restrict__ tile,
-                                                           uint2 *__restrict__ ranges)
+                                                           uint2 *__restrict__ ranges, uint32_t keymask)
 {
     const int64_t i0 = ((int64_t)blockIdx.x * 256 + threadIdx.x) * 4;
     if (n_dev)
@@ -860,11 +889,11 @@
     if (i0 + 3 < N)
     {
         const uint4 q = *(const uint4 *)(tile + i0);
-        k[0] = q.x; k[1] = q.y; k[2] = q.z; k[3] = q.w;
+        k[0] = q.x & keymask; k[1] = q.y & keymask; k[2] = q.z & keymask; k[3] = q.w & keymask;
     }
     else
-        for (int j = 0; j < 4; j++) k[j] = i0 + j < N ? tile[i0 + j] : 0u;
-    uint32_t prev = i0 > 0 ? tile[i0 - 1] : 0u;
+        for (int j = 0; j < 4; j++) k[j] = i0 + j < N ? tile[i0 + j] & keymask : 0u;
+    uint32_t prev = i0 > 0 ? tile[i0 - 1] & keymask : 0u;
 #pragma unroll
     for (int j = 0; j < 4; j++)
     {
@@ -1453,8 +1482,13 @@
                          float *contrib_sum, float *contrib_max, int64_t capacity, int32_t *status, const QuadMaskArgs &qmask, hipStream_t s)
 {
     if (P <= 0) return;
-    hipLaunchKernelGGL(scan_emit_kernel, dim3((unsigned)(((P + SB - 1) / SB) * 4)), dim3(256), 0, s, P, grid_x, ntiles, g, b, im.ranges, contrib_sum,
-                       contrib_max, (long long)capacity, status, scan_two_level(P), qmask);
+    const dim3 grid((unsigned)(((P + SB - 1) / SB) * 4));
+    if (qmask.blocks)
+        hipLaunchKernelGGL(scan_emit_kernel<true>, grid, dim3(256), 0, s, P, grid_x, ntiles, g, b, im.ranges, contrib_sum, contrib_max, (long long)capacity,
+                           status, scan_two_level(P), qmask);
+    else
+        hipLaunchKernelGGL(scan_emit_kernel<false>, grid, dim3(256), 0, s, P, grid_x, ntiles, g, b, im.ranges, contrib_sum, contrib_max, (long long)capacity,
+                           status, scan_two_level(P), qmask);
 }
 const unsigned long long *ts_instance_count_dev(const GeometryStateView &g, int P) { return (const unsigned long long *)(g.blocksum + (P + SB - 1) / SB); }
 
@@ -1473,10 +1507,10 @@
     }
 }
 
-void ts_launch_tile_ranges(int64_t N, const unsigned long long *n_dev, const BinningStateView &b, const ImageStateView &im, hipStream_t s)
+void ts_launch_tile_ranges(int64_t N, const unsigned long long *n_dev, int ntiles, const BinningStateView &b, const ImageStateView &im, hipStream_t s)
 {
     if (N <= 0) return;
-    hipLaunchKernelGGL(tile_ranges_kernel, dim3((unsigned)((N + 1023) / 1024)), dim3(256), 0, s, N, n_dev, b.tile, im.ranges);
+    hipLaunchKernelGGL(tile_ranges_kernel, dim3((unsigned)((N + 1023) / 1024)), dim3(256), 0, s, N, n_dev, b.tile, im.ranges, ts_tile_keymask(ntiles));
 }
 
 static int generic_chunk(size_t n) { return ts_instance_chunk(n); }
diff --git a/triangle-splatting_amd/csrc/render_group.hip b/triangle-splatting_amd/csrc/render_group.hip
--- a/triangle-splatting_amd/csrc/render_group.hip
+++ b/triangle-splatting_amd/csrc/render_group.hip
@@ -92,6 +92,17 @@
     return s;
 }
 
+template <bool GAMMA1, bool CULL>
+__device__ __forceinline__ BlockCull entry_blocks(const float4 &r0, const float4 &r1, uint32_t id_nibble, float g2, float OX, float OY)
+{
+    if (CULL) return block_cull<GAMMA1>(r0.x, r0.y, r0.z, r0.w, r1.x, r1.y, r1.z, g2, OX, OY);
+    BlockCull s;
+    entry_geometry(s, r0.x, r0.y, r0.z, r0.w, r1.x, r1.y, OX, OY);
+#pragma unroll
+    for (int g = 0; g < 4; g++) s.ov[g] = (id_nibble >> (TS_ID_BITS + g)) & 1u;
+    return s;
+}
+
 __device__ __forceinline__ void write_dummy_row(float *row, int lane)
 {
     if (lane < ROW)
@@ -125,9 +136,10 @@
 #endif
 
 #if TSG_PART & 1
-template <bool RICH, bool GAMMA1>
+template <bool RICH, bool GAMMA1, bool CULL>
 __global__ void __launch_bounds__(256, TSG_FWD_WAVES) render_fwd_group_kernel(RenderArgs a, const uint2 *__restrict__ ranges,
-                                                                const uint32_t *__restrict__ point_list, const float4 *__restrict__ rec,
+                                                                const uint32_t *__restrict__ point_list, const uint32_t *__restrict__ keys,
+                                                                const float4 *__restrict__ rec,
                                                                 float *__restrict__ final_T, uint32_t *__restrict__ n_contrib,
                                                                 float *__restrict__ out_feature, float *__restrict__ out_depth,
                                                                 float *__restrict__ out_normal, float *__restrict__ contrib_sum,
@@ -167,13 +179,15 @@
         const unsigned long long alive = ballot(!P.done);
         if (alive == 0) break;
         int nq = 0;
-        stream_refill<false, TSG_FWD_CAP>(id, pos, nq, point_list + range.x, cursor, len, TS_ID_BITS + wave, lane);
+        stream_refill<false, TSG_FWD_CAP, !CULL>(id, pos, nq, point_list + range.x, cursor, len, CULL ? TS_ID_BITS + wave : 16 + 4 * wave, lane,
+                                                 keys + range.x);
         if (nq == 0) break;
         const bool valid = lane < nq;
         const int ent = pos;
+        const uint32_t tid = CULL ? id : id & TS_ID_MASK;
         float4 r0 = make_float4(0, 0, 0, 0), r1 = r0, r2 = r0, r3 = r0;
-        gather_record<RICH>(rec, id, valid, r0, r1, r2, r3);
-        const BlockCull s = block_cull<GAMMA1>(r0.x, r0.y, r0.z, r0.w, r1.x, r1.y, r1.z, g2, OX, OY);
+        gather_record<RICH>(rec, tid, valid, r0, r1, r2, r3);
+        const BlockCull s = entry_blocks<GAMMA1, CULL>(r0, r1, id, g2, OX, OY);
         unsigned long long M[4];
         const unsigned long long any = fwd_block_masks(M, alive, valid, s.ov);
         TSG_STAT(0, __popcll(ballot(valid)));
@@ -183,7 +197,7 @@
         TSG_STAT(7, __popcll(any));
         const Compaction cp = compact_rows(any, lane);
         bool mine = in_pass(cp, false);
-        if (mine) publish_row(cst + cp.r * ROW, s, id, ent, r1, r2, r3);
+        if (mine) publish_row(cst + cp.r * ROW, s, tid, ent, r1, r2, r3);
         for (int h = 0;;)
         {
             const int steps = build_lists(list, M, pass_mask(cp, mine), row0, cp.r, ROW, dummy, lane);
@@ -247,9 +261,10 @@
 #endif
 
 #if TSG_PART & 2
-template <bool RICH, bool GAMMA1>
+template <bool RICH, bool GAMMA1, bool CULL>
 __global__ void __launch_bounds__(64, TSG_BWD_WAVES) render_bwd_group_kernel(RenderArgs a, const uint2 *__restrict__ ranges,
-                                                             const uint32_t *__restrict__ point_list, const float4 *__restrict__ rec,
+                                                             const uint32_t *__restrict__ point_list, const uint32_t *__restrict__ keys,
+                                                             const float4 *__restrict__ rec,
                                                              const float *__restrict__ final_T, const uint32_t *__restrict__ n_contrib,
                                                              const float *__restrict__ dL_dout_feature,
                                                              const float *__restrict__ dL_dout_depth,
@@ -292,19 +307,21 @@
     for (;;)
     {
         int nq = 0;
-        stream_refill<true, TSG_BWD_CAP>(id, pos, nq, point_list + range.x, cursor, maxlast, TS_ID_BITS + quad, lane);
+        stream_refill<true, TSG_BWD_CAP, !CULL>(id, pos, nq, point_list + range.x, cursor, maxlast, CULL ? TS_ID_BITS + quad : 16 + 4 * quad, lane,
+                                                keys + range.x);
         if (nq == 0) break;
         const bool valid = lane < nq;
         const int ent = pos;
+        const uint32_t tid = CULL ? id : id & TS_ID_MASK;
         float4 r0 = make_float4(0, 0, 0, 0), r1 = r0, r2 = r0, r3 = r0;
-        gather_record<RICH>(rec, id, valid, r0, r1, r2, r3);
-        const BlockCull s = block_cull<GAMMA1>(r0.x, r0.y, r0.z, r0.w, r1.x, r1.y, r1.z, g2, OX, OY);
+        gather_record<RICH>(rec, tid, valid, r0, r1, r2, r3);
+        const BlockCull s = entry_blocks<GAMMA1, CULL>(r0, r1, id, g2, OX, OY);
         unsigned long long M[4];
         const unsigned long long any = bwd_block_masks(M, valid, s.ov, pos, glast);
         if (any == 0) continue;
         const Compaction cp = compact_rows(any, lane);
         bool mine = in_pass(cp, false);
-        if (mine) publish_row(rows + cp.r * BROW, s, id, ent, r1, r2, r3);
+        if (mine) publish_row(rows + cp.r * BROW, s, tid, ent, r1, r2, r3);
         for (int h = (cp.nact - 1) / NR;;)
         {
             const unsigned long long mm = pass_mask(cp, mine);
@@ -406,14 +423,30 @@
 #endif
 }
 
+#define TS_BLEND2D_RG(KERNEL, R, G1, A, GRID, BLOCK, STREAM, ...)                                                                  \
+    do                                                                                                                            \
+    {                                                                                                                             \
+        if ((A).block_masks) hipLaunchKernelGGL((KERNEL<R, G1, false>), dim3(GRID), dim3(BLOCK), 0, STREAM, __VA_ARGS__);          \
+        else hipLaunchKernelGGL((KERNEL<R, G1, true>), dim3(GRID), dim3(BLOCK), 0, STREAM, __VA_ARGS__);                          \
+    } while (0)
+#define TS_LAUNCH_BLEND2D(KERNEL, A, GRID, BLOCK, STREAM, ...)                                                                    \
+    do                                                                                                                            \
+    {                                                                                                                             \
+        const bool g1 = ((A).gamma == 1.0f);                                                                                      \
+        if ((A).rich_info && g1) TS_BLEND2D_RG(KERNEL, true, true, A, GRID, BLOCK, STREAM, __VA_ARGS__);                          \
+        else if ((A).rich_info) TS_BLEND2D_RG(KERNEL, true, false, A, GRID, BLOCK, STREAM, __VA_ARGS__);                          \
+        else if (g1) TS_BLEND2D_RG(KERNEL, false, true, A, GRID, BLOCK, STREAM, __VA_ARGS__);                                     \
+        else TS_BLEND2D_RG(KERNEL, false, false, A, GRID, BLOCK, STREAM, __VA_ARGS__);                                            \
+    } while (0)
+
 #if TSG_PART & 1
 void ts_launch_render_fwd_group(const RenderArgs &a, const GeometryStateView &g, const BinningStateView &b, const ImageStateView &im,
                                 float *out_feature, float *out_depth, float *out_normal, float *contrib_sum, float *contrib_max,
                                 hipStream_t s)
 {
     if (a.grid_x * a.grid_y == 0) return;
-    TS_LAUNCH_BLEND(render_fwd_group_kernel, a, ts_tile_units(a.grid_x, a.grid_y), 256, s, a, im.ranges, b.vals, g.rec, im.final_T, im.n_contrib,
-                    out_feature, out_depth, out_normal, contrib_sum, contrib_max);
+    TS_LAUNCH_BLEND2D(render_fwd_group_kernel, a, ts_tile_units(a.grid_x, a.grid_y), 256, s, a, im.ranges, b.vals, b.tile, g.rec, im.final_T, im.n_contrib,
+                      out_feature, out_depth, out_normal, contrib_sum, contrib_max);
 }
 
 #endif
@@ -437,7 +470,7 @@
                                 hipStream_t s)
 {
     if (a.grid_x * a.grid_y == 0) return;
-    TS_LAUNCH_BLEND(render_bwd_group_kernel, a, ts_quadrant_units(a.grid_x, a.grid_y), 64, s, a, im.ranges, b.vals, g.rec, im.final_T, im.n_contrib,
-                    dL_dout_feature, dL_dout_depth, dL_dout_normal, grad_rec);
-}
-#endif
+    TS_LAUNCH_BLEND2D(render_bwd_group_kernel, a, ts_quadrant_units(a.grid_x, a.grid_y), 64, s, a, im.ranges, b.vals, b.tile, g.rec, im.final_T, im.n_contrib,
+                      dL_dout_feature, dL_dout_depth, dL_dout_normal, grad_rec);
+}
+#endif
diff --git a/triangle-splatting_amd/csrc/ts2d_common.h b/triangle-splatting_amd/csrc/ts2d_common.h
--- a/triangle-splatting_amd/csrc/ts2d_common.h
+++ b/triangle-splatting_amd/csrc/ts2d_common.h
@@ -131,6 +131,8 @@
 }
 
 static inline int ts_tile_bits(int ntiles) { return ts_higher_msb((uint32_t)(ntiles > 1 ? ntiles - 1 : 1)); }
+#define TS_BLOCKMASK_MAX_TILES 65535
+static inline uint32_t ts_tile_keymask(int ntiles) { return ntiles <= TS_BLOCKMASK_MAX_TILES ? 0xFFFFu : 0xFFFFFFFFu; }
 
 static inline size_t ts_carve_binning(char *base, int64_t N, int32_t W, int32_t H, BinningStateView &v)
 {
@@ -201,13 +203,14 @@
     float tan_fovx, tan_fovy;
     int W, H;
     float inv_W, inv_H;
+    int blocks;
 };
 void ts_launch_zero_words(uint32_t *p, size_t n, hipStream_t s);
 void ts_launch_emit_keys(int P, int grid_x, int ntiles, const GeometryStateView &g, const BinningStateView &b, const ImageStateView &im,
                          float *contrib_sum, float *contrib_max, int64_t capacity, int32_t *status, const QuadMaskArgs &qm, hipStream_t s);
 const unsigned long long *ts_instance_count_dev(const GeometryStateView &g, int P);
 void ts_sort_pairs(const BinningStateView &b, int64_t N, const unsigned long long *n_dev, int ntiles, hipStream_t s);
-void ts_launch_tile_ranges(int64_t N, const unsigned long long *n_dev, const BinningStateView &b, const ImageStateView &im, hipStream_t s);
+void ts_launch_tile_ranges(int64_t N, const unsigned long long *n_dev, int ntiles, const BinningStateView &b, const ImageStateView &im, hipStream_t s);
 size_t ts_quantile_scratch_bytes();
 void ts_quantile_threshold(const uint32_t *keys, size_t n, float q, void *scratch, float *thr, hipStream_t s);
 void ts_quantile_passes(const uint32_t *keys, size_t n, float q, void *scratch, int first_pass, hipStream_t s);
@@ -225,6 +228,7 @@
     const float *background;
     const float *background_depth_dev;
     bool rich_info;
+    bool block_masks;
 };
 void ts_launch_render_fwd_group(const RenderArgs &a, const GeometryStateView &g, const BinningStateView &b,
                                 const ImageStateView &im, float *out_feature, float *out_depth, float *out_normal,
diff --git a/triangle-splatting_amd/csrc/ts2d_group.h b/triangle-splatting_amd/csrc/ts2d_group.h
--- a/triangle-splatting_amd/csrc/ts2d_group.h
+++ b/triangle-splatting_amd/csrc/ts2d_group.h
@@ -16,15 +16,22 @@
 
 __device__ __forceinline__ bool ecc_in_range(float ecc) { return __float_as_uint(ecc) <= 0x41200000u; }
 
-template <bool DESC, int CAP = 64>
-__device__ __forceinline__ void stream_refill(uint32_t &id, int &pos, int &n, const uint32_t *__restrict__ list, int &cursor, int end, int qbit, int lane)
+template <bool DESC, int CAP = 64, bool NIB = false>
+__device__ __forceinline__ void stream_refill(uint32_t &id, int &pos, int &n, const uint32_t *__restrict__ list, int &cursor, int end, int qbit, int lane,
+                                              const uint32_t *__restrict__ keys = nullptr)
 {
     while (n < CAP && (DESC ? cursor > 0 : cursor < end))
     {
         const int k = DESC ? cursor - 1 - lane : cursor + lane;
         const bool valid = DESC ? k >= 0 : k < end;
-        const uint32_t v = valid ? list[k] : 0u;
-        const bool want = valid && ((v >> qbit) & 1u);
+        uint32_t v = 0u, key = 0u;
+        if (valid)
+        {
+            v = list[k];
+            if (NIB) key = keys[k];
+        }
+        const uint32_t nib = NIB ? (key << (TS_ID_BITS - qbit)) & ~TS_ID_MASK : 0u;
+        const bool want = NIB ? nib != 0u : valid && ((v >> qbit) & 1u);
         unsigned long long mt = ballot(want);
         int adv = 64;
         const int room = CAP - n;
@@ -39,7 +46,7 @@
         if (mt == 0) continue;
         const int cnt = __popcll(mt), rk = lane_rank(mt);
         const int dest = (taken ? n + rk : n + cnt + (lane - rk)) & 63;
-        const uint32_t pid = (uint32_t)__builtin_amdgcn_ds_permute(dest << 2, (int)(v & TS_ID_MASK));
+        const uint32_t pid = (uint32_t)__builtin_amdgcn_ds_permute(dest << 2, (int)((v & TS_ID_MASK) | nib));
         const int ppos = __builtin_amdgcn_ds_permute(dest << 2, k);
         const bool fresh = lane >= n && lane < n + cnt;
         id = fresh ? pid : id;
diff --git a/triangle-splatting_amd/csrc/ts2d_lab.h b/triangle-splatting_amd/csrc/ts2d_lab.h
--- a/triangle-splatting_amd/csrc/ts2d_lab.h
+++ b/triangle-splatting_amd/csrc/ts2d_lab.h
@@ -20,6 +20,7 @@
 int ts2d_test_quantile(const uint32_t *keys, size_t n, float q, void *scratch, float *out, void *stream);
 void ts2d_lab_depth_split(int mode, int bucket_cap);
 void ts2d_lab_force_all_quadrants(int on);
+void ts2d_lab_force_kernel_cull(int on);
 
 #ifdef __cplusplus
 }
diff --git a/triangle-splatting_amd/csrc/ts2d_support.h b/triangle-splatting_amd/csrc/ts2d_support.h
--- a/triangle-splatting_amd/csrc/ts2d_support.h
+++ b/triangle-splatting_amd/csrc/ts2d_support.h
@@ -28,8 +28,10 @@
     float bminx, bmaxx, bminy, bmaxy;
     bool live;
 };
+template <int BOX = 7>
 __device__ __forceinline__ QuadSetup quad_setup(float v1x, float v1y, float v2x, float v2y, float v3x, float v3y, float E, float pad_px = 0.0f)
 {
+    constexpr float box = (float)BOX;
     QuadSetup q;
     q.v1x = v1x; q.v1y = v1y; q.v2x = v2x; q.v2y = v2y; q.v3x = v3x; q.v3y = v3y;
     const float area2 = __fsub_rn(__fmul_rn(v2x - v1x, v3y - v1y), __fmul_rn(v2y - v1y, v3x - v1x));
@@ -39,9 +41,9 @@
     q.A3 = -q.A1 - q.A2; q.B3 = -q.B1 - q.B2;
     const float m = (1.0f - E) * (1.0f / 3.0f);
     const float slope_margin = 2e-6f * 15.0f + pad_px;
-    q.P1 = fmaxf(0.0f, 7.0f * q.A1) + fmaxf(0.0f, 7.0f * q.B1) - m + slope_margin * (fabsf(q.A1) + fabsf(q.B1));
-    q.P2 = fmaxf(0.0f, 7.0f * q.A2) + fmaxf(0.0f, 7.0f * q.B2) - m + slope_margin * (fabsf(q.A2) + fabsf(q.B2));
-    q.P3 = fmaxf(0.0f, 7.0f * q.A3) + fmaxf(0.0f, 7.0f * q.B3) - m + slope_margin * (fabsf(q.A3) + fabsf(q.B3));
+    q.P1 = fmaxf(0.0f, box * q.A1) + fmaxf(0.0f, box * q.B1) - m + slope_margin * (fabsf(q.A1) + fabsf(q.B1));
+    q.P2 = fmaxf(0.0f, box * q.A2) + fmaxf(0.0f, box * q.B2) - m + slope_margin * (fabsf(q.A2) + fabsf(q.B2));
+    q.P3 = fmaxf(0.0f, box * q.A3) + fmaxf(0.0f, box * q.B3) - m + slope_margin * (fabsf(q.A3) + fabsf(q.B3));
     const float cx = (v1x + v2x + v3x) * (1.0f / 3.0f), cy = (v1y + v2y + v3y) * (1.0f / 3.0f);
     const float e1x = E * (v1x - cx), e2x = E * (v2x - cx), e3x = E * (v3x - cx);
     const float e1y = E * (v1y - cy), e2y = E * (v2y - cy), e3y = E * (v3y - cy);
@@ -109,6 +111,47 @@
     return m;
 }
 
+__device__ __forceinline__ uint32_t block_edge_bits(float k, float A, float B)
+{
+    const float x0 = k, x1 = fmaf(4.0f, A, k), x2 = fmaf(8.0f, A, k), x3 = fmaf(12.0f, A, k);
+    const float y1 = -4.0f * B, y2 = -8.0f * B, y3 = -12.0f * B;
+    const uint32_t c0 = (x0 >= 0.0f ? 0x01u : 0u) | (x1 >= 0.0f ? 0x02u : 0u) | (x2 >= 0.0f ? 0x10u : 0u) | (x3 >= 0.0f ? 0x20u : 0u);
+    const uint32_t c1 = (x0 >= y1 ? 0x01u : 0u) | (x1 >= y1 ? 0x02u : 0u) | (x2 >= y1 ? 0x10u : 0u) | (x3 >= y1 ? 0x20u : 0u);
+    const uint32_t c2 = (x0 >= y2 ? 0x01u : 0u) | (x1 >= y2 ? 0x02u : 0u) | (x2 >= y2 ? 0x10u : 0u) | (x3 >= y2 ? 0x20u : 0u);
+    const uint32_t c3 = (x0 >= y3 ? 0x01u : 0u) | (x1 >= y3 ? 0x02u : 0u) | (x2 >= y3 ? 0x10u : 0u) | (x3 >= y3 ? 0x20u : 0u);
+    return c0 | (c1 << 2) | (c2 << 8) | (c3 << 10);
+}
+__device__ __forceinline__ uint32_t block_bits(float k1, float k2, float k3, float A1, float A2, float A3, float B1, float B2, float B3, float bminx,
+                                               float bmaxx, float bminy, float bmaxy, float TX, float TY)
+{
+    uint32_t cols = 0, rows = 0;
+#pragma unroll
+    for (int i = 0; i < 4; i++)
+    {
+        cols |= (bminx <= TX + (float)(4 * i + 3) && bmaxx >= TX + (float)(4 * i)) ? 1u << ((i >> 1) * 4 + (i & 1)) : 0u;
+        rows |= (bminy <= TY + (float)(4 * i + 3) && bmaxy >= TY + (float)(4 * i)) ? 1u << ((i >> 1) * 8 + (i & 1) * 2) : 0u;
+    }
+    uint32_t m = (cols * 0x0505u) & (rows * 0x0033u);
+    if (m) m &= block_edge_bits(k1, A1, B1);
+    if (m) m &= block_edge_bits(k2, A2, B2);
+    if (m) m &= block_edge_bits(k3, A3, B3);
+    return m;
+}
+__device__ __forceinline__ uint32_t block_mask(const QuadSetup &q, float TX, float TY)
+{
+    const float u1x = q.v1x - TX, u1y = q.v1y - TY, u2x = q.v2x - TX, u2y = q.v2y - TY, u3x = q.v3x - TX, u3y = q.v3y - TY;
+    const float t1a = u2x * u3y, t1b = u2y * u3x, t2a = u3x * u1y, t2b = u3y * u1x, aia = fabsf(q.ia);
+    const float C1 = (t1a - t1b) * q.ia, C2 = (t2a - t2b) * q.ia;
+    const float C3 = 1.0f - C1 - C2;
+    const float r1 = 4e-7f * (fabsf(t1a) + fabsf(t1b)) * aia, r2 = 4e-7f * (fabsf(t2a) + fabsf(t2b)) * aia;
+    const float k1 = C1 + q.P1 + r1, k2 = C2 + q.P2 + r2, k3 = C3 + q.P3 + (r1 + r2 + 4e-7f);
+    return block_bits(k1, k2, k3, q.A1, q.A2, q.A3, q.B1, q.B2, q.B3, q.live ? q.bminx : 3e38f, q.live ? q.bmaxx : -3e38f, q.bminy, q.bmaxy, TX, TY);
+}
+__device__ __forceinline__ uint32_t quadrants_of_blocks(uint32_t m)
+{
+    return ((m & 0x000Fu) ? 1u : 0u) | ((m & 0x00F0u) ? 2u : 0u) | ((m & 0x0F00u) ? 4u : 0u) | ((m & 0xF000u) ? 8u : 0u);
+}
+
 struct QuadAffine { float4 a, b, c, d; };
 __device__ __forceinline__ QuadAffine quad_anchor(const QuadSetup &q, uint32_t id, uint32_t minx, uint32_t miny, uint32_t w, uint32_t h)
 {
@@ -147,4 +190,11 @@
     m |= (x1 && y1 && k1 + ax1 + by1 >= 0.0f && k2 + ax2 + by2 >= 0.0f && k3 + ax3 + by3 >= 0.0f) ? 8u : 0u;
     return m;
 }
-}
+__device__ __forceinline__ uint32_t block_mask_affine(const QuadAffine &o, uint32_t dx, uint32_t dy, uint32_t x, uint32_t y)
+{
+    const float fx = (float)(dx * TS_TILE), fy = (float)(dy * TS_TILE), TX = (float)(x * TS_TILE), TY = (float)(y * TS_TILE);
+    const float A1 = o.a.w, A2 = o.b.x, A3 = o.b.y, B1 = o.b.z, B2 = o.b.w, B3 = o.c.x;
+    const float k1 = fmaf(B1, fy, fmaf(A1, fx, o.a.x)), k2 = fmaf(B2, fy, fmaf(A2, fx, o.a.y)), k3 = fmaf(B3, fy, fmaf(A3, fx, o.a.z));
+    return block_bits(k1, k2, k3, A1, A2, A3, B1, B2, B3, o.c.y, o.c.z, o.c.w, o.d.x, TX, TY);
+}
+}
diff --git a/triangle-splatting_amd/diff_triangle_rasterization_2D/_abi.py b/triangle-splatting_amd/diff_triangle_rasterization_2D/_abi.py
--- a/triangle-splatting_amd/diff_triangle_rasterization_2D/_abi.py
+++ b/triangle-splatting_amd/diff_triangle_rasterization_2D/_abi.py
@@ -148,6 +148,7 @@
     "ts2d_test_quantile": (C.c_int, [_vp, C.c_size_t, C.c_float, _vp, _vp, _vp]),
     "ts2d_lab_depth_split": (None, [C.c_int, C.c_int]),
     "ts2d_lab_force_all_quadrants": (None, [C.c_int]),
+    "ts2d_lab_force_kernel_cull": (None, [C.c_int]),
 }
 
 GEOM_SIGNATURES = {
```

After: 1353, median of 6. 1.01x the previous value.
